# Ipsedo/MARLClassification

Hardware: AMD Instinct MI355X
Metric: agent-env-steps/sec (higher is better)
Workload: dtype f32; 1 GPU; RESISC45 256x256x3, 16 agents, 16 steps, f=12, README dims (configs[2]); full train iteration: rollout + A2C loss + BPTT backward + Adam; batch_per_gpu=256, global_batch=256, parallelism=dp1, rng=library (Philox4x32-10), launch=eager

## Files before the change

marlclassification_amd/csrc/common.h:

```cpp
#pragma once

#include <hip/hip_runtime.h>
#include <stdint.h>
#include <stdio.h>

#include "../../include/marl_hip.h"
#include "split.h"

namespace marl {

constexpr int kWave = 64;

inline int p4(int x) { return (x + 3) & ~3; }
inline int64_t cdiv(int64_t a, int64_t b) { return (a + b - 1) / b; }

void set_error(const char* fmt, ...);

int tune_get(const char* key, int dflt);
int tune_set(const char* key, int value);

__device__ __forceinline__ float rcp_fast(float x) { return __builtin_amdgcn_rcpf(x); }
__device__ __forceinline__ float sigmoid_acc(float x) { return rcp_fast(1.0f + __expf(-x)); }
__device__ __forceinline__ float tanh_fast(float x) { return 1.0f - 2.0f * rcp_fast(1.0f + __expf(2.0f * x)); }
__device__ __forceinline__ float silu_fast(float y) { return y * sigmoid_acc(y); }
__device__ __forceinline__ float silu_grad_fast(float y) {
    const float s = sigmoid_acc(y);
    return s * (1.0f + y * (1.0f - s));
}

__device__ __forceinline__ float wave_sum(float v) {
    int x = __float_as_int(v);
#define MARL_DPP_ADD(ctrl, rmask)                         \
    x = __float_as_int(__int_as_float(x) +                \
                       __int_as_float(__builtin_amdgcn_update_dpp(0, x, ctrl, rmask, 0xf, false)))
    MARL_DPP_ADD(0x111, 0xf);
    MARL_DPP_ADD(0x112, 0xf);
    MARL_DPP_ADD(0x114, 0xf);
    MARL_DPP_ADD(0x118, 0xf);
    MARL_DPP_ADD(0x142, 0xa);
    MARL_DPP_ADD(0x143, 0xc);
#undef MARL_DPP_ADD
    return __int_as_float(__builtin_amdgcn_readlane(x, 63));
}

#define MARL_HIP_CHECK(expr)                                                        \
    do {                                                                            \
        hipError_t e_ = (expr);                                                     \
        if (e_ != hipSuccess) {                                                     \
            marl::set_error("%s failed: %s (%s:%d)", #expr, hipGetErrorString(e_),  \
                            __FILE__, __LINE__);                                    \
            return MARL_EHIP;                                                       \
        }                                                                           \
    } while (0)

#define MARL_LAUNCH_CHECK() MARL_HIP_CHECK(hipGetLastError())

#define MARL_TRY(expr)             \
    do {                           \
        int rc_ = (expr);          \
        if (rc_ != MARL_OK) return rc_; \
    } while (0)

struct GemmSeg {
    const float* a;
    const float* b;
    int lda, ldb, k;
    const void* b3;
    int kt3;
};

struct GemmB {
    const float* b;
    int ld, k;
    const void* b3;
    int kt3;
    GemmB from_row(int row0) const {
        return GemmB{b + (size_t)row0 * ld, ld, k,
                     b3 ? static_cast<const char*>(b3) + (size_t)row0 * kt3 * 192 : nullptr, kt3};
    }
};
inline GemmB gemm_b(const float* b, int ld, int k) { return GemmB{b, ld, k, nullptr, 0}; }

struct GemmProb {
    GemmSeg seg[2];
    int nseg;
    int m, n;
    float* c;
    int ldc;
    const float* bias;
    int accumulate;
    const float* c_prev;
    float* h_next;
    float* c_next;
    float* gates;
    int ld_state, ld_gates;
};

constexpr int kMaxGemmBatch = 4;
struct GemmBatch {
    GemmProb p[kMaxGemmBatch];
    int count;
    int gx, gy;
    int xcd_map;
    int single_buf;
#ifdef MARL_KERNEL_TS
    long long* ts;
#endif
};

__device__ __forceinline__ void xcd_tile(unsigned gx, unsigned gy, unsigned gz, unsigned& bx,
                                         unsigned& by, unsigned& bz) {
    const unsigned T = gx * gy * gz, L = blockIdx.x;
    const unsigned per = T >> 3, rem = T & 7, xcd = L & 7, slot = L >> 3;
    const unsigned q = (xcd < rem ? xcd * (per + 1) : rem * (per + 1) + (xcd - rem) * per) + slot;
    bz = q / (gx * gy);
    const unsigned r = q - bz * gx * gy;
    bx = r / gy;
    by = r - bx * gy;
}
int xcd_map_enabled();

GemmProb gemm_prob(const float* a, int lda, const GemmB& b, float* c, int ldc, int m, int n,
                   const float* bias = nullptr, int accumulate = 0);
void gemm_add_seg(GemmProb& p, const float* a, int lda, const GemmB& b);

int launch_gemm_nt(const GemmBatch& batch, hipStream_t st);
int launch_gemm_lstm(const GemmBatch& batch, hipStream_t st);

int split_mode();
size_t split_image_floats(int rows, int k);
struct SplitDesc {
    const float* src;
    void* dst;
    int rows, k, ld, kt;
};
constexpr int kMaxSplitDesc = 64;
struct SplitBatch {
    SplitDesc d[kMaxSplitDesc];
    int count;
};
int launch_split_weights(const SplitBatch& b, hipStream_t st);
int launch_gemm_nt_split(const GemmBatch& batch, int max_m, int max_n, int64_t blocks128, hipStream_t st);
int launch_gemm_lstm_split(const GemmBatch& batch, int max_m, int max_n, hipStream_t st);
int launch_gemm_tn_split(const float* a, int lda, const float* b, int ldb, float* out, int ldo,
                         int64_t stride, int ni, int nj, int64_t rows, int64_t rows_per_split,
                         float* csum, dim3 grid, int gx, int gy, int gz, hipStream_t st);

struct G3Seg {
    const char* a3;
    const char* b3;
    int a_row0, b_row0;
    int steps;
};
struct G3Prob {
    G3Seg seg[2];
    int nseg;
    int m, n;
    float* c;
    int ldc;
    const float* bias;
    int accumulate;
    const float* c_prev;
    float* h_next;
    float* c_next;
    float* gates;
    int ld_state, ld_gates;
    char* h3;
    int h3_row0, h3_steps;
};
constexpr int kMaxG3 = 4;
struct G3Batch {
    G3Prob p[kMaxG3];
    int count;
    int gx, gy, xcd_map;
    int safe;
#ifdef MARL_G3_ABLATE
    long long* clk;
#endif
};
G3Prob g3_prob(const void* a3, int a_row0, const void* b3, int b_row0, int k, float* c, int ldc, int m, int n,
               const float* bias = nullptr, int accumulate = 0);
void g3_add_seg(G3Prob& p, const void* a3, int a_row0, const void* b3, int b_row0, int k);
int launch_gemm_nt3(const G3Batch& batch, hipStream_t st, int variant = 0);
int launch_gemm_lstm3(const G3Batch& batch, hipStream_t st, int variant = 0);
int g3_lstm_plan(const G3Batch& batch);
struct G3TnArgs {
    const char* a3;
    const char* b3;
    int a_steps, b_steps;
    int a_row0, b_row0;
    float* out;
    int ldo;
    int64_t out_split_stride;
    int ni, nj;
    int64_t rows, rows_per_split;
    float* csum;
    int gx, gy, gz, safe;
    int j_first;
#ifdef MARL_G3_ABLATE
    int abl;
#endif
};
struct G3TnPlan {
    int variant, splits;
    int64_t rows_per_split;
};
G3TnPlan g3_tn_plan(int ni, int nj, int64_t rows);
constexpr int kMaxTnCell = 4;
struct G3TnCell {
    G3TnArgs t[kMaxTnCell];
    int nt, n256;
    int gx, gz;
    int teams;
};
bool g3_tn_cell_ok(int ni, int nj_ih, int nj_hh, int64_t rows);
G3TnPlan g3_tn_cell_plan(int ni, int nj_ih, int nj_hh, int64_t rows);
size_t g3_tn_cell_scratch_bytes(int ni, int nj_ih, int nj_hh, int64_t rows);
int launch_gemm_tn3_cell(G3TnArgs ih, G3TnArgs hh, const G3TnPlan& plan, hipStream_t st);
size_t g3_tn_scratch_bytes(int ni, int nj, int64_t rows);
int launch_gemm_tn3(G3TnArgs a, const G3TnPlan& plan, hipStream_t st);

struct ImgDesc {
    const float* src;
    void* dst;
    int64_t rows;
    int k, ld;
};
constexpr int kMaxImgDesc = 64;
struct ImgBatch {
    ImgDesc d[kMaxImgDesc];
    int count;
};
int launch_images(const ImgBatch& b, hipStream_t st);

constexpr int kProfClasses = 6;
void prof_before(int cls, hipStream_t st);
void prof_after(int cls, hipStream_t st);
int profile_begin(int cls, int max_launches);
int profile_end(double* total_ms, int* launches);

struct RedQueue;
size_t gemm_tn_scratch_bytes(int ni, int nj, int64_t rows);
struct TnQueue;
int launch_gemm_tn(const float* a, int lda, const float* b, int ldb, float* c, int ldc, int ni,
                   int nj, int64_t rows, float* scratch, size_t scratch_bytes, hipStream_t st,
                   float* colsum_out = nullptr, RedQueue* q = nullptr, TnQueue* tq = nullptr);

struct TnBatchProb {
    const float* a;
    const float* b;
    float* out;
    float* csum;
    int64_t stride, rows, rows_per_split;
    int lda, ldb, ldo, ni, nj, gx, gy, first_block;
};
constexpr int kMaxTnBatch = 12;
struct TnBatch {
    TnBatchProb p[kMaxTnBatch];
    int count;
};
struct TnQueue {
    struct Item {
        const float* a;
        const float* b;
        float* c;
        float* colsum;
        int lda, ldb, ldc, ni, nj;
        int64_t rows;
    };
    Item it[kMaxTnBatch];
    int n = 0;
};
bool gemm_tn_is_small(int ni, int nj, int64_t rows);
int launch_tn_queue(TnQueue& tq, RedQueue* q, hipStream_t st);

struct RedDesc {
    const float* part;
    int64_t stride;
    int count, n;
    float* out0;
    int split, nj, ldc;
    float* out1;
    int accumulate;
    int folds, per;
};
constexpr int kMaxRed = 40;
struct RedBatch {
    RedDesc d[kMaxRed];
    int first_block[kMaxRed + 1];
    int count;
};
struct RedQueue {
    RedBatch stage1, stage2;
    float* scratch = nullptr;
    size_t cap = 0, off = 0;
    hipStream_t st = nullptr;
    int rc = MARL_OK;
    void reset(float* s, size_t floats, hipStream_t stream);
    float* take(size_t floats, bool may_flush = true);
    void push(const float* part, int64_t stride, int count, int n, float* out0, int split, int nj,
              int ldc, float* out1, int accumulate);
    int launch_pending();
    int flush();
};
int launch_red_batch(const RedBatch& b, hipStream_t st);

int launch_ln_silu_fwd(const float* z, int ldz, const float* gamma, const float* beta, float* out,
                       int ldo, float* stats, int64_t m, int n, hipStream_t st,
                       const float* wdot = nullptr, const float* bdot = nullptr,
                       float* dot_out = nullptr);
int ln_bwd_blocks(int64_t m, int n);
int launch_ln_silu_bwd_rank(const float* g, int ldg, int kin, const float* bt, int ldbt,
                            const float* z, int ldz, const float* stats, const float* gamma,
                            const float* beta, float* dz, int lddz, float* part, int64_t m, int n,
                            hipStream_t st);
int launch_ln_silu_bwd(const float* da, int ldda, const float* z, int ldz, const float* stats,
                       const float* gamma, const float* beta, float* dz, int lddz, float* part,
                       int64_t m, int n, hipStream_t st);
int launch_reduce_affine(float* part, int64_t nparts, int n, float* dgamma, float* dbeta,
                         int accumulate, hipStream_t st, RedQueue* q = nullptr);

int gn_fwd_im2col_supported(int P, int C);
int launch_gn_silu_fwd(const float* z, const float* gamma, const float* beta, float* out,
                       int64_t ldo, int out_chw, float* stats, int64_t rows, int P, int C, int G,
                       hipStream_t st, float* cols = nullptr, int ldk = 0, int hin = 0);
int gn_bwd_blocks(int64_t rows, int C);
int launch_gn_silu_bwd(const float* da, int64_t ldda, int da_chw, const float* z,
                       const float* stats, const float* gamma, const float* beta, float* dz,
                       float* part, int64_t rows, int P, int C, int G, hipStream_t st);

int launch_agg_msg(const float* m, float* out, int ld, int na, int nb, int n, hipStream_t st);
int launch_mix_msg(const float* m, float* out, int ld, int na, int nb, int n, const float* mix, int transpose,
                   hipStream_t st);
int mix_msg_max_agents();
struct CommGate {
    const int32_t* pos;
    int radius, metric, normalize;
};
__device__ __forceinline__ bool comm_in_range(int2 p, int2 q, int radius, int metric) {
    const int dy = p.x > q.x ? p.x - q.x : q.x - p.x, dx = p.y > q.y ? p.y - q.y : q.y - p.y;
    if (metric) return (int64_t)dy * dy + (int64_t)dx * dx <= (int64_t)radius * radius;
    return (dy > dx ? dy : dx) <= radius;
}
template <int MAXA>
__device__ __forceinline__ float comm_gate_weight(const float* __restrict__ base, const CommGate& G, int na, int nb,
                                                  int b, int a, int a2) {
    const int2* __restrict__ pos = reinterpret_cast<const int2*>(G.pos);
    const int2 pa = pos[(size_t)a * nb + b];
    if (!G.normalize) {
        const int2 q = pos[(size_t)a2 * nb + b];
        const float bv = base[a * na + a2];
        return comm_in_range(pa, q, G.radius, G.metric) ? bv : 0.f;
    }
    constexpr int CH = MAXA < 8 ? MAXA : 8;
    float S = 0.f, s = 0.f, u = 0.f;
#pragma unroll
    for (int j0 = 0; j0 < MAXA; j0 += CH) {
        int2 q[CH];
        float bv[CH];
#pragma unroll
        for (int j = 0; j < CH; ++j) {
            const int jj = j0 + j < na ? j0 + j : na - 1;
            q[j] = pos[(size_t)jj * nb + b];
            bv[j] = base[a * na + jj];
        }
#pragma unroll
        for (int j = 0; j < CH; ++j) {
            if (j0 + j < na) {
                const float uj = comm_in_range(pa, q[j], G.radius, G.metric) ? bv[j] : 0.f;
                S += bv[j];
                s += uj;
                if (j0 + j == a2) u = uj;
            }
        }
    }
    return s > 0.f ? u * (S / s) : 0.f;
}
int launch_mix_msg_gated(const float* m, float* out, int ld, int na, int nb, int n, const float* mix,
                         const CommGate& gate, int transpose, hipStream_t st);
int comm_grad_blocks(int64_t pairs, int* per_out);
int comm_grad_supported(int na, int n, int n2, int ldw);
int launch_comm_grad(const float* dz, int lddz, const float* msg, int ldmsg, const float* w, int ldw, int na, int nb,
                     int steps, int n2, int n, float* part, float* out, hipStream_t st);

int launch_pos_embed_fwd(const int32_t* pos, const float* npos_in, int h, int w, const float* W, const float* b,
                         const float* gamma, const float* beta, float* npos4, float* z, int ldz,
                         float* stats, float* out, int ldo, int64_t rows, int nd, hipStream_t st);

int launch_lstm_cell_bwd(const float* dh, int lddh, float* dc, int lddc, float* gates, int ldg,
                         const float* c_prev, const float* c_new, int ldc, int64_t rows, int n,
                         hipStream_t st);
struct LstmBwdBatch;
int launch_lstm_cell_bwd_batch(LstmBwdBatch& b, int count, hipStream_t st);
int launch_lstm_cell_bwd2(const float* dh0, int lddh0, float* dc0, int lddc0, float* gates0,
                          int ldg0, const float* cp0, const float* cn0, int ldc0, int n0,
                          const float* dh1, int lddh1, float* dc1, int lddc1, float* gates1,
                          int ldg1, const float* cp1, const float* cn1, int ldc1, int n1,
                          int64_t rows, hipStream_t st);

struct SampleArgs {
    const float* a_pol;
    int ld_a, nla;
    const float* w1;
    int ldw;
    const float* b1;
    const float* noise;
    uint64_t rng_seed, rng_ctr;
    const uint64_t* rng_off_dev;
    int rng_on;
    const int64_t* forced;
    const int32_t* pos_in;
    int32_t* pos_out;
    int64_t* step_pos;
    int64_t* step_actions;
    float* step_logp;
    float* probs;
    int32_t* actions_i32;
    int R, nA, H, W, f;
    int32_t table[MARL_MAX_ACTIONS][2];
    const float* pe_W;
    const float* pe_b;
    const float* pe_gamma;
    const float* pe_beta;
    float* pe_npos;
    float* pe_z;
    float* pe_stats;
    float* pe_out;
    int pe_ldz, pe_ldo, pe_nd;
    char* pe_img;
    int pe_row0, pe_steps, pe_col0;
    float ex_inv_tau, ex_keep, ex_floor;
    int ex_greedy;
};
int launch_sample(const SampleArgs& a, hipStream_t st, bool explore = false);

int launch_draw_episode(uint64_t seed, uint64_t offset, const uint64_t* offset_dev, int64_t* pos0,
                        int R, int H, int W, int f, float* h0, float* c0, int n_b, float* hc0,
                        float* cc0, int n_a, float* noise, int64_t n_noise, hipStream_t st);

struct PermDesc {
    const float* src;
    float* dst;
    int rows, cols;
    int dst_ld;
    int rd, rs1, rs2;
    int cd, cs1, cs2;
    int frag;
    const float* src2;
};
constexpr int kMaxPerm = 56;
struct PermBatch {
    PermDesc d[kMaxPerm];
    int count;
};
int launch_permute(const PermBatch& b, hipStream_t st);

__host__ __device__ inline int panel_frag_groups(int K) { return (K + 15) >> 4; }
__host__ __device__ inline size_t panel_frag_floats(int n, int K) {
    return ((size_t)((n + 31) >> 5) * panel_frag_groups(K) + 3) * 512;
}
__host__ __device__ inline size_t panel_frag_index(int r, int k, int groups) {
    return ((((size_t)(r >> 5) * groups + (k >> 4)) * 2 + ((r >> 4) & 1)) * 64 + ((k >> 2) & 3) * 16 + (r & 15)) * 4 +
           (k & 3);
}

struct Counters {
    uint64_t rng_offset;
    uint64_t step;
    float lr_over_bc1;
    float inv_sqrt_bc2;
    float pad[2];
};
static_assert(sizeof(Counters) == MARL_COUNTERS_BYTES, "counter block layout");
int launch_counters_set(Counters* c, uint64_t rng_offset, int64_t step, float lr, float beta1,
                        float beta2, int tick, hipStream_t st);

int launch_adam(float* p, const float* g, float* m, float* v, int64_t n, float lr_over_bc1,
                float inv_sqrt_bc2, float beta1, float beta2, float eps, float grad_scale,
                hipStream_t st, const Counters* cnt = nullptr);

int launch_fill(float* p, int64_t n, float v, hipStream_t st);
int launch_add2d(const float* a, int64_t lda, const float* b, int64_t ldb, float* out, int64_t ldo,
                 int64_t rows, int cols, hipStream_t st);
int launch_copy2d(const float* src, int64_t lds, float* dst, int64_t ldd, int64_t rows, int cols,
                  hipStream_t st);
int launch_i64_to_i32(const int64_t* src, int32_t* dst, int64_t n, hipStream_t st);
int launch_policy_dlogits(const float* dlogp, const float* probs, const int32_t* actions,
                          float* out, int ld, int64_t rows, int nA, hipStream_t st);
int launch_policy_dlogits_probs(const float* dlogp, const float* dprobs, const float* probs,
                                const int32_t* actions, float* out, int ld, int64_t rows, int nA,
                                hipStream_t st);
int launch_policy_dlogits_explore(const float* dlogp, const float* dprobs, const float* probs,
                                  const int32_t* actions, float* out, int ld, int64_t rows, int nA,
                                  float inv_tau, float keep, float floor, hipStream_t st);
int launch_acc2d(float* dst, int64_t ldd, const float* src, int64_t lds, int64_t rows, int cols,
                 hipStream_t st);
int launch_rowdot(const float* a, int lda, const float* w, const float* b, float* out,
                  int64_t rows, int n, hipStream_t st);

struct PanelLayer {
    const float* wfrag;
    int wgroups;
    const float* bias;
    const float* gamma;
    const float* beta;
    int n;
    float* z;
    int ldz;
    float* stats;
    float* a;
    int lda;
    char* a3;
    int a3_row0, a3_steps, a3_col0;
};
constexpr int kPanelMaxLayers = 4;
struct PanelFwdProb {
    const float* x;
    int ldx, k0;
    int agg_na, agg_nb;
    float* xbar;
    int m, nlayers;
    PanelLayer layer[kPanelMaxLayers];
    int by_batch, g_na, g_nb, agg_at, ld_xbar;
    const float* mix;
    CommGate gate;
};
struct PanelFwdBatch {
    PanelFwdProb p[2];
    int count;
    int off_panel1, off_red, off_part, off_prm;
    int off_mix;
    int has_sample, panel_blocks;
    int epi_prob;
    int ln_narrow_max;
    SampleArgs sample;
#ifdef MARL_KERNEL_TS
    long long* ts;
#endif
};
int panel_chain_supported(int na, int n_msg, int threads);
int panel_supported(int k0, int n0, int n1);
int panel_sample_supported(int n_actions);
int launch_panel_fwd(PanelFwdBatch& b, hipStream_t st, bool explore = false);

struct LstmBwdArgs {
    const float* dh;
    float* dc;
    float* gates;
    const float* c_prev;
    const float* c_new;
    int lddh, lddc, ldg, ldc, n;
    char* g3;
    int g3_row0, g3_steps;
    int skip_f32;
};
struct LstmBwdBatch {
    LstmBwdArgs a[2];
    int64_t rows;
    int vec4;
};
inline bool lstm_bwd_vec4_ok(const LstmBwdArgs& a) {
    return (a.n & 3) == 0 && (a.lddh & 3) == 0 && (a.lddc & 3) == 0 && (a.ldg & 3) == 0 && (a.ldc & 3) == 0;
}
__device__ __forceinline__ void lstm_cell_bwd_at(const LstmBwdArgs& A, int64_t r, int u, float dhv);
__device__ __forceinline__ void lstm_cell_bwd_elem(const LstmBwdArgs& A, int64_t rows, int64_t idx) {
    const int n = A.n;
    if (idx >= rows * n) return;
    const int64_t r = idx / n;
    const int u = (int)(idx % n);
    lstm_cell_bwd_at(A, r, u, A.dh[r * A.lddh + u]);
}
__device__ __forceinline__ void lstm_cell_bwd_at(const LstmBwdArgs& A, int64_t r, int u, float dhv) {
    const int n = A.n;
    float* g = A.gates + r * A.ldg + u;
    const float gi = g[0], gf = g[n], gg = g[2 * n], go = g[3 * n];
    const float tc = tanh_fast(A.c_new[r * A.ldc + u]);
    const float dcv = dhv * go * (1.0f - tc * tc) + A.dc[r * A.lddc + u];
    g[0] = dcv * gg * gi * (1.0f - gi);
    g[n] = dcv * A.c_prev[r * A.ldc + u] * gf * (1.0f - gf);
    g[2 * n] = dcv * gi * (1.0f - gg * gg);
    g[3 * n] = dhv * tc * go * (1.0f - go);
    A.dc[r * A.lddc + u] = dcv * gf;
}

__device__ __forceinline__ void lstm_cell_bwd_at4(const LstmBwdArgs& A, int64_t r, int u, const float (&dhv)[4]) {
    const int n = A.n;
    float* g = A.gates + r * A.ldg + u;
    const float4 gi4 = *reinterpret_cast<const float4*>(g), gf4 = *reinterpret_cast<const float4*>(g + n),
                 gg4 = *reinterpret_cast<const float4*>(g + 2 * n), go4 = *reinterpret_cast<const float4*>(g + 3 * n);
    const float4 cn4 = *reinterpret_cast<const float4*>(A.c_new + r * A.ldc + u),
                 cp4 = *reinterpret_cast<const float4*>(A.c_prev + r * A.ldc + u),
                 dc4 = *reinterpret_cast<const float4*>(A.dc + r * A.lddc + u);
    const float gi[4] = {gi4.x, gi4.y, gi4.z, gi4.w}, gf[4] = {gf4.x, gf4.y, gf4.z, gf4.w};
    const float gg[4] = {gg4.x, gg4.y, gg4.z, gg4.w}, go[4] = {go4.x, go4.y, go4.z, go4.w};
    const float cn[4] = {cn4.x, cn4.y, cn4.z, cn4.w}, cp[4] = {cp4.x, cp4.y, cp4.z, cp4.w};
    const float dcin[4] = {dc4.x, dc4.y, dc4.z, dc4.w};
    float o[5][4];
#pragma unroll
    for (int q = 0; q < 4; ++q) {
        const float tc = tanh_fast(cn[q]);
        const float dcv = dhv[q] * go[q] * (1.0f - tc * tc) + dcin[q];
        o[0][q] = dcv * gg[q] * gi[q] * (1.0f - gi[q]);
        o[1][q] = dcv * cp[q] * gf[q] * (1.0f - gf[q]);
        o[2][q] = dcv * gi[q] * (1.0f - gg[q] * gg[q]);
        o[3][q] = dhv[q] * tc * go[q] * (1.0f - go[q]);
        o[4][q] = dcv * gf[q];
    }
    if (!(A.g3 && A.skip_f32)) {
// ... 54 lines not shown
    int has_cell, panel_blocks;
    LstmBwdArgs cell;
    int64_t cell_rows;
    int cell_vec4;
    int cellb_img_done, cell_img_done;
    CommGate gate;
#ifdef MARL_KERNEL_TS
    long long* ts;
#endif
};
int panel_bwd_blocks(int m);
int panel_chain_blocks(int na, int nb);
int panel_chain_by_batch(int na);
int launch_panel_bwd(PanelBwdProb& p, hipStream_t st);

#ifdef MARL_KERNEL_TS
constexpr int kTsWaves = 16, kTsSlots = 48, kTsRoles = 2;
#define MARL_TS_DECL(ptr) long long* ts_ = (ptr); int tsi_ = 0
#define MARL_TS()                                                                              \
    if (ts_ && (threadIdx.x & 63) == 0 && blockIdx.x == 37 && blockIdx.y < kTsRoles && tsi_ < kTsSlots) \
    ts_[((int)blockIdx.y * kTsWaves + (threadIdx.x >> 6)) * kTsSlots + tsi_++] = wall_clock64()
int ts_begin(long long** dev, int call);
void ts_report(const char* tag, long long* dev, int waves, int role = 0);
#else
#define MARL_TS_DECL(ptr)
#define MARL_TS()
#endif

struct FDiv {
    uint32_t d, m;
};
inline FDiv make_fdiv(int d) { return FDiv{(uint32_t)d, (uint32_t)(((1ull << 32) / (uint64_t)d) + 1)}; }
__device__ __forceinline__ int fdiv(int n, FDiv f) {
    return f.d == 1 ? n : (int)__umulhi((uint32_t)n, f.m);
}

struct CnnFwdLayer {
    const float *w, *bias, *gamma, *beta;
    float* cols;
    float* z;
    float* gst;
    int cin, cout, G, hin, hout, P, K, ldk;
    const float* wfrag;
};
struct CnnFwdArgs {
    const void* img;
    const float* obs;
    const int32_t* pos;
    int img_u8;
    int64_t rows;
    int nb, c_img, H, W, f, L;
    CnnFwdLayer layer[MARL_MAX_CNN_LAYERS];
    float* u;
    int ldu;
    char* u3;
    int u3_row0, u3_steps;
    int rb;
    int off_b0, off_b1, off_stat;
    FDiv dP[MARL_MAX_CNN_LAYERS], dhout[MARL_MAX_CNN_LAYERS], dcin[MARL_MAX_CNN_LAYERS],
        dcpg[MARL_MAX_CNN_LAYERS], dG[MARL_MAX_CNN_LAYERS], dNT[MARL_MAX_CNN_LAYERS],
        dc4o[MARL_MAX_CNN_LAYERS];
    FDiv dpe, dff, df, dE;
#ifdef MARL_KERNEL_TS
    long long* ts;
#endif
};
int cnn_fwd_supported(const CnnFwdArgs& a);
int cnn_fwd_writes_image(const CnnFwdArgs& a);
int launch_cnn_fwd(CnnFwdArgs& a, hipStream_t st);
struct CnnFwdPlan {
    int which, rb, blocks;
};
CnnFwdPlan cnn_fwd_launch_plan(const CnnFwdArgs& a);

struct CnnDgradArgs {
    const float* dz;
    const float* wt;
    const float* zin;
    const float* gst;
    const float *gamma, *beta;
    float* dzin;
    float* part;
    int64_t rows;
    int ldwt, cin, cout, hin, hout, P, Pin, G;
    int rb, MT, NT, off_zin, off_da, off_perm, off_stat, off_gsum;
    int tbeg[17];
    FDiv dc4o, dc4i, dPin, dcpg, dG;
    const void* img;
    const int32_t* pos;
    float* w0_part;
    float* w0_bpart;
    int w0;
    int img_u8, nb, c_img, H, W, cin0, f0, K0;
    int off_pix, pix_per, cs0;
    FDiv dpe0, dff0, df0, dhin0;
#ifdef MARL_KERNEL_TS
    long long* ts;
#endif
};
int cnn_dgrad_supported(const CnnDgradArgs& a);
int cnn_dgrad_blocks(const CnnDgradArgs& a);
int cnn_dgrad_blocks_max(const CnnDgradArgs& a);
int cnn_dgrad_launch_rb(const CnnDgradArgs& a);
struct CnnDgradPlanInfo {
    int rb, MT, NT, blocks;
};
CnnDgradPlanInfo cnn_dgrad_launch_plan(const CnnDgradArgs& a);
int launch_cnn_dgrad(CnnDgradArgs& a, hipStream_t st);
int cnn_dgrad_w0_ok(const CnnDgradArgs& a, int cin0, int f0);

struct CnnDimgArgs {
    const float* dz0;
    const float* wt0;
    const int32_t* pos;
    float* d_img;
    int ns, na, nb, c_img, H, W;
    int ldwt, cin, cout, f, hout, P;
    int th;
};
int cnn_dimg_supported(const CnnDimgArgs& a);
int launch_cnn_dimg(CnnDimgArgs& a, hipStream_t st);

struct CnnWgradArgs {
    const float* dz;
    const void* img;
    const int32_t* pos;
    const float* zin;
    const float* gst;
    const float *gamma, *beta;
    float* part_w;
    float* part_b;
    int64_t rows;
    int first, img_u8, nb, c_img, H, W;
    int cin, cout, hin, hout, P, G, K;
    int rb, nchunks, blocks;
    int hp, cs, zs, in_per;
    int off_dz, off_tab, lds_floats;
    int in_plane;
    int nct, nkt, nkt_slab, slabs;
    int tgc, tgk, ms;
    int sct, skt;
    int pd, pi;
    FDiv dP, dhout, dPin, dhin, dcin, dc4o, dc4i, dpe, dff, df;
};
int cnn_wgrad_supported(const CnnWgradArgs& a);
int cnn_wgrad_blocks(const CnnWgradArgs& a);
int launch_cnn_wgrad(CnnWgradArgs& a, hipStream_t st);
struct CnnWgradPlanInfo {
    int form, rb, chunks, blocks;
    int sct, skt, tgc, tgk, ms, slabs, pd, pi;
};
CnnWgradPlanInfo cnn_wgrad_launch_plan(const CnnWgradArgs& a);
int launch_slab_reduce(const float* part, int64_t stride, int splits, float* c, int ldc, int ni,
                       int nj, const float* bpart, float* bias, hipStream_t st);

int launch_gather_im2col(const void* img, int img_u8, const int32_t* pos, float* cols, int ldk,
                         int na, int nb, int c_img, int cin, int H, int W, int f, hipStream_t st);
int launch_obs_im2col(const float* obs, float* cols, int ldk, int64_t rows, int c_img, int cin,
                      int f, hipStream_t st);
int launch_patch_gather(const float* img, const int64_t* pos, float* obs, int na, int nb, int c,
                        int H, int W, int f, hipStream_t st);
int launch_im2col(const float* a, float* cols, int ldk, int64_t rows, int hin, int cin,
                  hipStream_t st);
int launch_col2im(const float* dcols, int ldk, float* da, int64_t rows, int hin, int cin,
                  hipStream_t st);

struct LossCommon {
    const float* preds;
    const float* values;
    const int64_t* y;
    float* scratch;
    int ns, na, nb, nc;
    bool cls = false;
    const float* cls_w = nullptr;
    const float* cls_sw = nullptr;
    float cls_eps = 0.f;
    bool cls_wrew = false;
};
struct LossGradArgs : LossCommon {
    const float* logp;
    float* g_preds;
    int ld_gp;
    float* g_logp;
    float* g_values;
    float* scalars;
    const float* probs = nullptr;
    float* g_probs = nullptr;
    int n_act = 0;
    float entropy_coef = 0.f;
};

struct LossArgs : LossGradArgs {
    double* adv_stats;
    float gamma;
    int phase;
};
size_t loss_scratch_floats(int ns, int na, int nb);
int launch_loss(const LossArgs& a, hipStream_t st);

struct AdvArgs : LossCommon {
    float* advn;
    float* ret;
    double* adv_stats;
    float gamma, lam;
    int phase;
};
int launch_advantages(const AdvArgs& a, hipStream_t st);

struct PpoArgs : LossGradArgs {
    const float* old_logp;
    const float* advn;
    const float* ret;
    float clip_eps;
};
int launch_ppo_loss(const PpoArgs& a, hipStream_t st);

int launch_grad_clip(float* g, int64_t n, float max_norm, float grad_scale, float* norm_out, double* part,
                     hipStream_t st);

}
```

marlclassification_amd/csrc/episode.hip:

```cpp
#include <math.h>
#include <stdlib.h>
#include <string.h>

#include "../../include/marl_hip_rowops.h"
#include "../../include/marl_hip_cnnops.h"
#include "../../include/marl_hip_explore.h"
#include "../../include/marl_hip_classloss.h"
#include "common.h"

namespace marl {

struct Dims {
    int na, nb, ns;
    int64_t R, NR;
    int H, W, c_img, f;
    int L;
    int ch[MARL_MAX_CNN_LAYERS + 1];
    int grp[MARL_MAX_CNN_LAYERS];
    int hw[MARL_MAX_CNN_LAYERS + 1];
    int P[MARL_MAX_CNN_LAYERS];
    int K[MARL_MAX_CNN_LAYERS];
    int ldk[MARL_MAX_CNN_LAYERS];
    int nf, nin;
    int n_b, n_a, n_m, nm2, n_mo, n_d, nA, nC, nlb, nla;
// ... 445 lines not shown
            red += ((v + 63) & ~(size_t)63) + 64 * 2 * (size_t)n + 64;
        };
        auto upd_tn = [&](int ni, int nj, int64_t rows) {
            const size_t v = gemm_tn_scratch_bytes(ni, nj, rows);
            tns = v > tns ? v : tns;
            red += v / sizeof(float) + 64 * ((size_t)ni * nj + ni) + 192;
        };
        const int64_t nr = d.NR, r = d.R;
        upd_part(ln_bwd_blocks(nr, d.nlb), d.nlb);
        upd_part(ln_bwd_blocks(nr, d.nla), d.nla);
        upd_part(ln_bwd_blocks(nr, d.n_d), d.n_d);
        upd_part(ln_bwd_blocks(r, d.nm2), d.nm2);
        upd_part(ln_bwd_blocks(r, d.n_mo), d.n_mo);
        upd_part(ln_bwd_blocks(r, d.n_m), d.n_m);
        for (int l = 0; l < d.L; ++l) upd_part(gn_bwd_blocks(nr, d.ch[l + 1]), d.ch[l + 1]);
        for (int l = 1; l < d.L; ++l)
            if (e.dgrad_ok[l]) upd_part(cnn_dgrad_blocks_max(cnn_dgrad_shape(d, l)), d.ch[l]);
        upd_tn(d.nC, d.nlb, nr);
        upd_tn(d.nlb, d.n_b, nr);
        upd_tn(1, d.nla, nr);
        upd_tn(d.nla, d.n_a, nr);
        upd_tn(d.nA, d.nla, nr);
        upd_tn(d.n_mo, d.nm2, nr);
        upd_tn(d.nm2, d.n_m, nr);
        upd_tn(d.n_m, d.nm2, nr);
        upd_tn(d.nm2, d.n_b, nr);
        upd_tn(4 * d.n_b, d.nin, nr);
        upd_tn(4 * d.n_b, d.n_b, nr);
        upd_tn(4 * d.n_a, d.nin, nr);
        upd_tn(4 * d.n_a, d.n_a, nr);
        if (e.g3) {
            const int tn3[4][2] = {{4 * d.n_b, d.nin}, {4 * d.n_b, d.n_b}, {4 * d.n_a, d.nin}, {4 * d.n_a, d.n_a}};
            for (const auto& q : tn3) {
                const size_t v = g3_tn_scratch_bytes(q[0], q[1], nr);
                tns = v > tns ? v : tns;
            }
            const int cell[2][3] = {{4 * d.n_b, d.nin, d.n_b}, {4 * d.n_a, d.nin, d.n_a}};
            for (const auto& q : cell)
                if (g3_tn_cell_ok(q[0], q[1], q[2], nr)) {
                    const size_t v = g3_tn_cell_scratch_bytes(q[0], q[1], q[2], nr);
                    tns = v > tns ? v : tns;
                }
        }
        upd_tn(d.n_d, 2, nr);
        if (d.L > 1 && e.dgrad_ok[1]) {
            const CnnDgradArgs g1 = cnn_dgrad_shape(d, 1);
            if (g1.w0) {
                int64_t nb_ = cnn_dgrad_blocks_max(g1);
                if (nb_ > 2048) nb_ = 2048;
                const size_t v = (size_t)nb_ * ((size_t)d.ch[1] * d.K[0] + d.ch[1]) * sizeof(float);
                tns = v > tns ? v : tns;
                red += v / sizeof(float) + 64 * ((size_t)d.ch[1] * (d.K[0] + 1)) + 192;
            }
        }
        for (int l = 0; l < d.L; ++l) {
            if (e.wgrad_ok[l]) {
                const size_t v = (size_t)cnn_wgrad_blocks(cnn_wgrad_shape(d, l)) *
                                 ((size_t)d.ch[l + 1] * d.K[l] + d.ch[l + 1]) * sizeof(float);
                tns = v > tns ? v : tns;
                red += v / sizeof(float) + 64 * ((size_t)d.ch[l + 1] * (d.K[l] + 1)) + 192;
            } else {
                upd_tn(d.ch[l + 1], d.K[l], nr * d.P[l]);
            }
        }
        e.part_floats = part;
        e.tns_bytes = tns;
        e.PART = b.take(part);
        e.TNS = b.take(tns / sizeof(float) + 16);
        {
            const int pn[4] = {d.n_mo, d.nm2, d.n_m, d.nm2};
            for (int n : pn) red += 64 * 2 * (size_t)n + 64;
        }
        e.red_floats = red + 4096;
        e.RED = b.take(e.red_floats);
    }
    e.loss_floats = loss_scratch_floats(d.ns, d.na, d.nb);
    e.LOSS = b.take(e.loss_floats);
    e.total = b.off;
}

struct Explore {
    bool on;
    float inv_tau, keep, eps;
    int greedy;
};
struct ClassLoss {
    bool on;
    const float* w;
    int nc;
    float eps;
    const float* sw;
    int ns;
    bool wrew;
};
struct Installed {
    const float* comm = nullptr;
    int comm_na = 0;
    CommGate range = {nullptr, -1, 0, 1};
    Explore explore = {false, 1.f, 1.f, 0.f, 0};
    ClassLoss class_loss = {false, nullptr, 0, 0.f, nullptr, 0, false};
    hipEvent_t heads_event = nullptr;
};
static Installed g_installed;

enum SampleSite { SAMPLE_OWN = 0, SAMPLE_EPILOGUE, SAMPLE_RIDE };
struct Plan {
    bool panels;
    bool panels_bwd;
    bool chain;
    bool panel_sample;
    bool g3_lstm;
    bool g3_tn, g3_tn_pipe;
    bool u3_by_producers;
    int skip_f32;
    int lstm_plan;
    SampleSite sample;
    int comm_form;
    int explore_form;
    int comm, comm_range, explore, class_loss;
};

struct Ctx {
    Dims d;
    WLayout w;
    ELayout e;
    float* W;
    float* E;
    hipStream_t st;
    int train;
    RedQueue* rq = nullptr;
    TnQueue* tq = nullptr;
    bool defer_slabs = false;
    size_t defer_small = 0;
    bool defer_this(size_t slab_bytes) const { return defer_slabs || (defer_small && slab_bytes <= defer_small); }
    Installed opt;
    Plan plan;
    int u3_row(int t) const { return (int)(e.u3_stride_rows * (size_t)t); }

    const char* wp3k(int i) const { return reinterpret_cast<const char*>(W + w.wp3k[i]); }
    const char* wt3k(int i) const { return reinterpret_cast<const char*>(W + w.wt3k[i]); }
    char* img(size_t off) const { return reinterpret_cast<char*>(E + off); }
    const float* wp(int i) const { return W + w.wp[i]; }
    const float* wt(int i) const { return W + w.wt[i]; }
    GemmB wpB(int i) const {
        const ParamMeta m = param_meta(d, i);
        return GemmB{wp(i), w.ldp[i], m.k, m.kind == PK_MATRIX ? W + w.wp3[i] : nullptr, (m.k + 31) / 32};
    }
    GemmB wtB(int i) const {
        const ParamMeta m = param_meta(d, i);
        return GemmB{wt(i), w.ldt[i], m.n, m.kind == PK_MATRIX ? W + w.wt3[i] : nullptr, (m.n + 31) / 32};
    }
    const float* wpf(int i) const { return w.wpf[i] ? W + w.wpf[i] : nullptr; }
    const float* wtf(int i) const { return w.wtf[i] ? W + w.wtf[i] : nullptr; }
    float* gp(int i) const { return W + w.gp[i]; }
    float* at(size_t off) const { return E + off; }
    float* at(const SBuf& s, int t) const { return E + s.at(train ? t : 0); }
    float* Hs(int t) const { return E + e.H + (size_t)t * d.R * d.ld_nb; }
    float* Cs(int t) const { return E + e.C + (size_t)t * d.R * d.ld_nb; }
    float* HCs(int t) const { return E + e.HC + (size_t)t * d.R * d.ld_na; }
    float* CCs(int t) const { return E + e.CC + (size_t)t * d.R * d.ld_na; }
    float* MSGs(int t) const { return E + e.MSG + (size_t)t * d.R * d.ld_nm; }
    int32_t* POSs(int t) const { return reinterpret_cast<int32_t*>(E + e.POS) + (size_t)t * d.R * 2; }
    float* PROBSs(int t) const { return E + e.PROBS + (size_t)t * d.R * d.nA; }
    int32_t* ACTs(int t) const { return reinterpret_cast<int32_t*>(E + e.ACT) + (size_t)t * d.R; }
    float* DHs(int t) const { return E + e.DH + (size_t)t * d.R * d.ld_nb; }
    float* DHCs(int t) const { return E + e.DHC + (size_t)t * d.R * d.ld_na; }
};

static Plan make_plan(const Dims& d, const WLayout& w, const ELayout& e, const Installed& opt) {
    auto env_on = [](const char* v) { return !(v && v[0] == '0'); };
    static const bool env_panels = env_on(getenv("MARL_PANELS")), env_sample = env_on(getenv("MARL_PANEL_SAMPLE"));
    Plan p{};
    p.panels = env_panels && panel_model_ok(d);
    p.panels_bwd = p.panels && d.n_mo <= 384 && d.nm2 <= 384 && d.n_m <= 384;
    p.chain = p.panels_bwd && panel_chain_supported(d.na, d.n_m, 256) && tune_get("panel_chain", 1) != 0 &&
              (!opt.comm || d.n_b <= 384);
    p.panel_sample = p.chain && env_sample && panel_sample_supported(d.nA);
    p.sample = p.chain ? (p.panel_sample ? SAMPLE_EPILOGUE : SAMPLE_OWN)
                       : (p.panels && !opt.explore.on ? SAMPLE_RIDE : SAMPLE_OWN);
    p.comm_form = opt.comm ? (p.chain ? 5 : p.panels ? 3 : 4) : p.chain ? 0 : p.panels ? 1 : 2;
    p.explore_form = !opt.explore.on ? 0 : p.panel_sample ? 1 : 2;
    p.comm = opt.comm != nullptr;
    p.comm_range = opt.range.radius >= 0 ? opt.range.radius : -1;
    p.explore = opt.explore.on;
    p.class_loss = opt.class_loss.on;

    const int k_lstm = tune_get("g3_lstm", 1), k_tn = tune_get("g3_tn", 1);
    p.g3_lstm = e.g3 && k_lstm != 0;
    if (p.g3_lstm) {
        G3Batch b{};
        b.count = 2;
        b.p[0].m = b.p[1].m = (int)d.R;
        b.p[0].n = d.n_b;
        b.p[1].n = d.n_a;
        p.lstm_plan = tune_get("g3_lstm_variant", 0);
        if (!p.lstm_plan) p.lstm_plan = g3_lstm_plan(b);
    }
    p.g3_tn = p.g3_lstm && k_tn != 0 &&
              (k_tn == 2 || (d.nin <= 640 && d.n_b <= 512 && d.n_a <= 512 &&
                             (d.NR >= 32768 || (g3_tn_cell_ok(4 * d.n_b, d.nin, d.n_b, d.NR) &&
                                                g3_tn_cell_ok(4 * d.n_a, d.nin, d.n_a, d.NR)))));
    p.g3_tn_pipe = p.g3_tn && tune_get("g3_tn_pipe", 1) != 0;
    p.skip_f32 = p.panels_bwd && p.g3_tn;
    static float here;
    CnnFwdArgs probe = cnn_fwd_shape(d);
    for (int l = 0; l < d.L; ++l) probe.layer[l].wfrag = w.wf[4 * l] ? &here : nullptr;
    p.u3_by_producers = p.g3_lstm && e.fused_fwd && cnn_fwd_writes_image(probe) && p.panels &&
                        ((d.nf | d.n_mo | d.n_d) & 3) == 0 &&
                        d.nin % 16 == 0;
    return p;
}

static int make_ctx(const marl_config* cfg, const void* wws, size_t wbytes, void* ews, size_t ebytes,
                    int train, void* stream, Ctx& c) {
    MARL_TRY(make_dims(cfg, c.d));
    c.opt = g_installed;
    if (c.opt.comm && c.opt.comm_na != c.d.na) {
        set_error("communication matrix is %d x %d but the configuration has %d agents", c.opt.comm_na,
                  c.opt.comm_na, c.d.na);
        return MARL_EINVAL;
    }
    if (c.opt.range.radius >= 0 && !c.opt.comm) {
        set_error("a communication range is installed without its base matrix (marl_comm_matrix)");
        return MARL_EINVAL;
    }
    make_wlayout(c.d, c.w);
    make_elayout(c.d, train, c.e);
    if (wbytes < c.w.total * sizeof(float) || ebytes < c.e.total * sizeof(float)) {
        set_error("workspace too small for the current configuration / tuning knobs: weights %zu of %zu "
                  "bytes, episode %zu of %zu bytes (ask marl_workspace_sizes again)", wbytes,
                  c.w.total * sizeof(float), ebytes, c.e.total * sizeof(float));
        return MARL_ESIZE;
    }
    c.W = const_cast<float*>(static_cast<const float*>(wws));
    c.E = static_cast<float*>(ews);
    c.st = static_cast<hipStream_t>(stream);
    c.train = train;
    if (!c.W || !c.E) {
        set_error("null workspace");
        return MARL_EINVAL;
    }
    if ((reinterpret_cast<uintptr_t>(c.W) & 255) || (reinterpret_cast<uintptr_t>(c.E) & 255)) {
        set_error("workspaces must be 256-byte aligned");
        return MARL_EINVAL;
    }
    c.plan = make_plan(c.d, c.w, c.e, c.opt);
    return MARL_OK;
}

static int gemm1(const Ctx& c, const GemmProb& p) {
    GemmBatch b{};
    b.p[0] = p;
    b.count = 1;
    return launch_gemm_nt(b, c.st);
}
static int gemm2(const Ctx& c, const GemmProb& p0, const GemmProb& p1) {
    GemmBatch b{};
    b.p[0] = p0;
    b.p[1] = p1;
    b.count = 2;
    return launch_gemm_nt(b, c.st);
}

struct StepIn {
    const float* obs = nullptr;
    const float* npos = nullptr;
    const void* img = nullptr;
    int img_u8 = 0;
};

struct CnnFwdIo {
    const void* img = nullptr;
    const float* obs = nullptr;
    const int32_t* pos = nullptr;
    int img_u8 = 0;
    int64_t rows = 0;
    float* cols[MARL_MAX_CNN_LAYERS] = {};
    float* z[MARL_MAX_CNN_LAYERS] = {};
    float* gst[MARL_MAX_CNN_LAYERS] = {};
    float* u = nullptr;
    int ldu = 0;
    char* u3 = nullptr;
    int u3_row0 = 0, u3_steps = 0;
};
static CnnFwdArgs cnn_fwd_args(const Dims& d, const WLayout& w, const float* W, const CnnFwdIo& io) {
    CnnFwdArgs a{};
    a.img = io.img;
    a.obs = io.obs;
    a.pos = io.pos;
    a.img_u8 = io.img_u8;
    a.rows = io.rows;
    a.nb = d.nb;
    a.c_img = d.c_img;
    a.H = d.H;
    a.W = d.W;
    a.f = d.f;
    a.L = d.L;
    for (int l = 0; l < d.L; ++l)
        a.layer[l] = CnnFwdLayer{W + w.wp[4 * l], W + w.wp[4 * l + 1], W + w.wp[4 * l + 2], W + w.wp[4 * l + 3],
                                 io.cols[l], io.z[l], io.gst[l],
                                 d.ch[l], d.ch[l + 1], d.grp[l], d.hw[l], d.hw[l + 1], d.P[l],
                                 d.K[l], d.ldk[l], w.wf[4 * l] ? W + w.wf[4 * l] : nullptr};
    a.u = io.u;
    a.ldu = io.ldu;
    a.u3 = io.u3;
    a.u3_row0 = io.u3_row0;
    a.u3_steps = io.u3_steps;
// ... 316 lines not shown
    const bool vdot = d.nla <= 384;
    MARL_TRY(launch_ln_silu_fwd(c.at(c.e.ZC1), d.ld_nla, c.wp(MARL_P_CRI_LNW), c.wp(MARL_P_CRI_LNB),
                                c.at(c.e.AC1), d.ld_nla, c.at(c.e.STC1), rows, d.nla, st,
                                vdot ? c.wp(MARL_P_CRI_W1) : nullptr, c.wp(MARL_P_CRI_B1), values));
    MARL_TRY(launch_ln_silu_fwd(c.at(c.e.ZQ1), d.ld_nlb, c.wp(MARL_P_PRE_LNW), c.wp(MARL_P_PRE_LNB),
                                c.at(c.e.AQ1), d.ld_nlb, c.at(c.e.STQ1), rows, d.nlb, st));
    if (!vdot)
        MARL_TRY(launch_rowdot(c.at(c.e.AC1), d.ld_nla, c.wp(MARL_P_CRI_W1), c.wp(MARL_P_CRI_B1),
                               values, rows, d.nla, st));
    MARL_TRY(gemm1(c, gemm_prob(c.at(c.e.AQ1), d.ld_nlb, c.wpB(MARL_P_PRE_W1),
                                preds, d.nC, (int)rows, d.nC, c.wp(MARL_P_PRE_B1))));
    return MARL_OK;
}

static void explore_sample_args(const Explore& ex, SampleArgs& a) {
    if (!ex.on) return;
    a.ex_inv_tau = ex.inv_tau;
    a.ex_keep = ex.keep;
    a.ex_floor = ex.eps / (float)a.nA;
    a.ex_greedy = ex.greedy;
    if (ex.greedy) {
        a.noise = nullptr;
        a.rng_on = 0;
    }
}

struct SampleIo {
    const float* noise = nullptr;
    const int64_t* forced = nullptr;
    uint64_t rng_seed = 0, rng_offset = 0;
    const void* counters = nullptr;
    int64_t *step_pos = nullptr, *step_actions = nullptr;
    float* step_logp = nullptr;
    bool embed_next = false;
};
static void fill_sample_args(const Ctx& c, const marl_config* cfg, int t, const SampleIo& io, SampleArgs& a) {
    const Dims& d = c.d;
    memset(&a, 0, sizeof(a));
    if (io.step_logp) {
        a.noise = io.noise ? io.noise + (size_t)t * d.R * d.nA : nullptr;
        a.rng_on = !io.noise && !io.forced;
        a.rng_seed = io.rng_seed ^ 0x9E3779B97F4A7C15ull;
        a.rng_ctr = (io.rng_offset << 16) + (uint64_t)t;
        a.rng_off_dev = io.counters ? &static_cast<const Counters*>(io.counters)->rng_offset : nullptr;
        a.forced = io.forced ? io.forced + (size_t)t * d.R : nullptr;
        a.step_pos = io.step_pos ? io.step_pos + (size_t)t * d.R * 2 : nullptr;
        a.step_actions = io.step_actions ? io.step_actions + (size_t)t * d.R : nullptr;
        a.step_logp = io.step_logp + (size_t)t * d.R;
    }
    if (io.embed_next && t + 1 < d.ns) {
        a.pe_W = c.wp(MARL_P_POS_W);
        a.pe_b = c.wp(MARL_P_POS_B);
        a.pe_gamma = c.wp(MARL_P_POS_LNW);
        a.pe_beta = c.wp(MARL_P_POS_LNB);
        a.pe_npos = c.at(c.e.NPOS, t + 1);
        a.pe_z = c.at(c.e.ZPOS, t + 1);
        a.pe_stats = c.at(c.e.STPOS, t + 1);
        a.pe_out = c.at(c.e.U, t + 1) + d.nf + d.n_mo;
        a.pe_ldz = d.ld_nd;
        a.pe_ldo = d.ld_nin;
        a.pe_nd = d.n_d;
        if (c.plan.u3_by_producers) {
            a.pe_img = c.img(c.e.U3);
            a.pe_row0 = c.u3_row(t + 1);
            a.pe_steps = img_steps(d.nin);
            a.pe_col0 = d.nf + d.n_mo;
        }
    }
    a.a_pol = c.at(c.e.AP1, t);
    a.ld_a = d.ld_nla;
    a.nla = d.nla;
    a.w1 = c.wp(MARL_P_POL_W1);
    a.ldw = d.ld_nla;
    a.b1 = c.wp(MARL_P_POL_B1);
    a.pos_in = c.POSs(t);
    a.pos_out = c.POSs(t + 1);
    a.probs = c.PROBSs(t);
    a.actions_i32 = c.ACTs(t);
    a.R = (int)d.R;
    a.nA = d.nA;
    a.H = d.H;
    a.W = d.W;
    a.f = d.f;
    for (int j = 0; j < d.nA; ++j) {
        a.table[j][0] = cfg->actions[j][0];
        a.table[j][1] = cfg->actions[j][1];
    }
    explore_sample_args(c.opt.explore, a);
}

static int fwd_open(const Ctx& c, int t, const StepIn& in, bool decode) {
    MARL_TRY(step_cnn(c, t, in));
    if (decode) MARL_TRY(step_decode(c, t));
    return step_pos_lstm(c, t, in, t > 0);
}
static int fwd_step_chain(const Ctx& c, int t, const StepIn& in, const SampleArgs& a) {
    MARL_TRY(fwd_open(c, t, in, t == 0));
    MARL_TRY(step_chain(c, t, a));
    return c.plan.sample == SAMPLE_EPILOGUE ? MARL_OK : launch_sample(a, c.st, c.opt.explore.on);
}
static int fwd_step_panels(const Ctx& c, int t, const StepIn& in, const SampleArgs& a) {
    const bool ride = c.plan.sample == SAMPLE_RIDE && t + 1 < c.d.ns;
    MARL_TRY(fwd_open(c, t, in, t == 0));
    MARL_TRY(step_encode_policy(c, t));
    if (t + 1 < c.d.ns) MARL_TRY(step_decode(c, t + 1, ride ? &a : nullptr));
    return ride ? MARL_OK : launch_sample(a, c.st, c.opt.explore.on);
}
static int fwd_step_rows(const Ctx& c, int t, const StepIn& in, const SampleArgs& a) {
    MARL_TRY(fwd_open(c, t, in, true));
    MARL_TRY(step_encode_policy(c, t));
    if (t + 1 < c.d.ns) MARL_TRY(step_decode(c, t + 1));
    return launch_sample(a, c.st, c.opt.explore.on);
}

struct PermQueue {
    PermBatch b{};
    hipStream_t st;
    int rc = MARL_OK;
    explicit PermQueue(hipStream_t s) : st(s) { b.count = 0; }
    void push(const PermDesc& p) {
        if (rc != MARL_OK) return;
        b.d[b.count++] = p;
        if (b.count == kMaxPerm) flush();
    }
    void flush() {
        if (rc == MARL_OK && b.count > 0) rc = launch_permute(b, st);
        b.count = 0;
    }
};

static PermDesc perm(const float* src, float* dst, int rows, int cols, int dst_ld, int rd, int rs1,
                     int rs2, int cd, int cs1, int cs2, const float* src2 = nullptr) {
    PermDesc p;
    p.src = src;
    p.dst = dst;
    p.rows = rows;
    p.cols = cols;
    p.dst_ld = dst_ld;
    p.rd = rd;
    p.rs1 = rs1;
    p.rs2 = rs2;
    p.cd = cd;
    p.cs1 = cs1;
    p.cs2 = cs2;
    p.frag = 0;
    p.src2 = src2;
    return p;
}

static PermDesc copy_desc(const float* src, int64_t lds, float* dst, int64_t ldd, int64_t rows, int cols) {
    return perm(src, dst, (int)rows, cols, (int)ldd, 1, (int)lds, 0, 1, 1, 0);
}

static int load_state(const Ctx& c, const float* h, const float* cc_, const float* hc,
                      const float* cca, const float* msg) {
    const Dims& d = c.d;
    PermQueue q(c.st);
    q.push(copy_desc(h, d.n_b, c.Hs(0), d.ld_nb, d.R, d.n_b));
    q.push(copy_desc(cc_, d.n_b, c.Cs(0), d.ld_nb, d.R, d.n_b));
    q.push(copy_desc(hc, d.n_a, c.HCs(0), d.ld_na, d.R, d.n_a));
    q.push(copy_desc(cca, d.n_a, c.CCs(0), d.ld_na, d.R, d.n_a));
    q.push(copy_desc(msg, d.n_m, c.MSGs(0), d.ld_nm, d.R, msg ? d.n_m : d.ld_nm));
    q.flush();
    MARL_TRY(q.rc);
    if (c.e.g3) {
        ImgBatch ib{};
        ib.d[0] = ImgDesc{h, c.img(c.e.H3), d.R, d.n_b, d.n_b};
        ib.d[1] = ImgDesc{hc, c.img(c.e.HC3), d.R, d.n_a, d.n_a};
        ib.count = 2;
        MARL_TRY(launch_images(ib, c.st));
    }
    return MARL_OK;
}


static int pack_weights(const Dims& d, const WLayout& w, const float* const* params, float* W,
                        hipStream_t st) {
    PermQueue q(st);
    for (int i = 0; i < MARL_NPARAMS; ++i) {
        const ParamMeta m = param_meta(d, i);
        if (m.kind == PK_NONE) continue;
        const float* src = params[i];
        if (!src) {
            set_error("parameter %d is null", i);
            return MARL_EINVAL;
        }
        if (m.kind == PK_MATRIX) {
            q.push(perm(src, W + w.wp[i], m.n, m.k, w.ldp[i], 1, m.k, 0, 1, 1, 0));
            q.push(perm(src, W + w.wt[i], m.k, m.n, w.ldt[i], 1, 1, 0, 1, m.k, 0));
        } else if (m.kind == PK_CONV) {
            const int ci = m.k / 9;
            q.push(perm(src, W + w.wp[i], m.n, m.k, w.ldp[i], 1, m.k, 0, ci, 1, 9));
            q.push(perm(src, W + w.wt[i], m.k, m.n, w.ldt[i], ci, 1, 9, 1, m.k, 0));
        } else {
            q.push(perm(src, W + w.wp[i], 1, m.n, m.n, 1, 0, 0, 1, 1, 0));
        }
    }
    q.push(perm(params[MARL_P_LB_BIH], W + w.bsum_b, 1, 4 * d.n_b, 4 * d.n_b, 1, 0, 0, 1, 1, 0,
                params[MARL_P_LB_BHH]));
    q.push(perm(params[MARL_P_LA_BIH], W + w.bsum_a, 1, 4 * d.n_a, 4 * d.n_a, 1, 0, 0, 1, 1, 0,
                params[MARL_P_LA_BHH]));
    q.flush();
    MARL_TRY(q.rc);
    for (int i = 0; i < MARL_NPARAMS; ++i) {
        const ParamMeta m = param_meta(d, i);
        if (!w.wf[i]) continue;
        const int steps = m.k / 16;
        q.push(perm(W + w.wp[i], W + w.wf[i], (m.n / 16) * steps * 4, 64, 64, steps * 4, 16 * w.ldp[i], 4, 4,
                    w.ldp[i], 1));
    }
    for (int i = 0; i < MARL_NPARAMS; ++i) {
        const ParamMeta m = param_meta(d, i);
        if (w.wpf[i]) {
            PermDesc p = perm(W + w.wp[i], W + w.wpf[i], m.n, m.k, 0, 1, w.ldp[i], 0, 1, 1, 0);
            p.frag = w.gpf[i];
            q.push(p);
        }
        if (w.wtf[i]) {
            PermDesc p = perm(W + w.wt[i], W + w.wtf[i], m.k, m.n, 0, 1, w.ldt[i], 0, 1, 1, 0);
            p.frag = w.gtf[i];
            q.push(p);
        }
    }
    q.flush();
    MARL_TRY(q.rc);
    SplitBatch sb{};
    sb.count = 0;
    for (int i = 0; i < MARL_NPARAMS; ++i) {
        const ParamMeta m = param_meta(d, i);
        if (m.kind != PK_MATRIX) continue;
        sb.d[sb.count++] = SplitDesc{W + w.wp[i], W + w.wp3[i], m.n, m.k, w.ldp[i], (m.k + 31) / 32};
        sb.d[sb.count++] = SplitDesc{W + w.wt[i], W + w.wt3[i], m.k, m.n, w.ldt[i], (m.n + 31) / 32};
    }
    MARL_TRY(launch_split_weights(sb, st));
    ImgBatch ib{};
    ib.count = 0;
    for (int i = 0; i < MARL_NPARAMS; ++i) {
        const ParamMeta m = param_meta(d, i);
        if (m.kind != PK_MATRIX || !w.wp3k[i]) continue;
        if (ib.count + 2 > kMaxImgDesc) {
            MARL_TRY(launch_images(ib, st));
            ib.count = 0;
        }
        ib.d[ib.count++] = ImgDesc{W + w.wp[i], W + w.wp3k[i], m.n, m.k, w.ldp[i]};
        ib.d[ib.count++] = ImgDesc{W + w.wt[i], W + w.wt3k[i], m.k, m.n, w.ldt[i]};
    }
    return launch_images(ib, st);
}

static int unpack_grads(const Ctx& c, float* const* grads, int which = 0) {
    PermQueue q(c.st);
    for (int i = 0; i < MARL_NPARAMS; ++i) {
        const bool head = i >= MARL_P_POL_W0 && i <= MARL_P_PRE_B1;
        if ((which == 1 && !head) || (which == 2 && head)) continue;
        const ParamMeta m = param_meta(c.d, i);
        if (m.kind == PK_MATRIX) {
            q.push(perm(c.gp(i), grads[i], m.n, m.k, m.k, 1, c.w.ldp[i], 0, 1, 1, 0));
        } else if (m.kind == PK_CONV) {
            const int ci = m.k / 9;
            q.push(perm(c.gp(i), grads[i], m.n, m.k, m.k, 1, c.w.ldp[i], 0, 9, 1, ci));
        }
    }
    if (which != 1) {
        q.push(perm(grads[MARL_P_LB_BIH], grads[MARL_P_LB_BHH], 1, 4 * c.d.n_b, 4 * c.d.n_b, 1, 0, 0, 1, 1, 0));
        q.push(perm(grads[MARL_P_LA_BIH], grads[MARL_P_LA_BHH], 1, 4 * c.d.n_a, 4 * c.d.n_a, 1, 0, 0, 1, 1, 0));
    }
    q.flush();
    return q.rc;
}

static int tn(const Ctx& c, const float* a, int lda, const float* b, int ldb, int pidx, int ni,
              int nj, int64_t rows, float* bias = nullptr) {
    RedQueue* q = c.defer_this(gemm_tn_scratch_bytes(ni, nj, rows)) ? c.rq : nullptr;
    return launch_gemm_tn(a, lda, b, ldb, c.gp(pidx), c.w.ldp[pidx], ni, nj, rows, c.at(c.e.TNS),
                          c.e.tns_bytes, c.st, bias, q, q ? c.tq : nullptr);
}
static int tn3(const Ctx& c, const char* a3, int ni, const char* b3, int nj, int pidx, int64_t rows, float* bias) {
    const G3TnPlan plan = g3_tn_plan(ni, nj, rows);
    if (g3_tn_scratch_bytes(ni, nj, rows) > c.e.tns_bytes) {
        set_error("tn3: scratch too small");
        return MARL_ESIZE;
    }
    float* scratch = c.at(c.e.TNS);
    G3TnArgs a{};
    a.a3 = a3;
    a.b3 = b3;
    a.a_steps = img_steps(ni);
    a.b_steps = img_steps(nj);
    a.out = scratch;
    a.ldo = nj;
    a.out_split_stride = (int64_t)ni * nj;
    a.ni = ni;
    a.nj = nj;
    a.rows = rows;
    a.csum = bias ? scratch + (size_t)plan.splits * ni * nj : nullptr;
    MARL_TRY(launch_gemm_tn3(a, plan, c.st));
    return launch_slab_reduce(scratch, (int64_t)ni * nj, plan.splits, c.gp(pidx), c.w.ldp[pidx], ni, nj, a.csum, bias, c.st);
}
static int tn3_cell(const Ctx& c, const char* g3, int ni, const char* u3, int nin, int p_ih, const char* h3, int nh,
                    int p_hh, int64_t rows, float* bias) {
    const G3TnPlan plan = g3_tn_cell_plan(ni, nin, nh, rows);
    if (g3_tn_cell_scratch_bytes(ni, nin, nh, rows) > c.e.tns_bytes) {
        set_error("tn3_cell: scratch too small");
        return MARL_ESIZE;
    }
    float* s_ih = c.at(c.e.TNS);
    float* s_hh = s_ih + (size_t)plan.splits * ni * nin;
    float* s_cs = s_hh + (size_t)plan.splits * ni * nh;
    G3TnArgs ih{}, hh{};
    ih.a3 = hh.a3 = g3;
    ih.a_steps = hh.a_steps = img_steps(ni);
    ih.ni = hh.ni = ni;
    ih.rows = hh.rows = rows;
    ih.b3 = u3;
    ih.b_steps = img_steps(nin);
    ih.nj = ih.ldo = nin;
    ih.out = s_ih;
    ih.out_split_stride = (int64_t)ni * nin;
    ih.csum = bias ? s_cs : nullptr;
    hh.b3 = h3;
    hh.b_steps = img_steps(nh);
    hh.nj = hh.ldo = nh;
    hh.out = s_hh;
    hh.out_split_stride = (int64_t)ni * nh;
    MARL_TRY(launch_gemm_tn3_cell(ih, hh, plan, c.st));
    MARL_TRY(launch_slab_reduce(s_ih, (int64_t)ni * nin, plan.splits, c.gp(p_ih), c.w.ldp[p_ih], ni, nin, nullptr, nullptr, c.st));
    return launch_slab_reduce(s_hh, (int64_t)ni * nh, plan.splits, c.gp(p_hh), c.w.ldp[p_hh], ni, nh, ih.csum, bias, c.st);
}
static float* part_scratch(const Ctx& c, int64_t blocks, int n, int acc, RedQueue*& q) {
    q = acc ? nullptr : c.rq;
    if (!q) return c.at(c.e.PART);
    float* p = q->take((size_t)blocks * 2 * n);
    if (q->rc != MARL_OK) q = nullptr;
    return q ? p : c.at(c.e.PART);
}
static int ln_bwd(const Ctx& c, float* da, int ldda, const float* z, int ldz, const float* stats,
                  int pw, int pb, int64_t rows, int n, float* const* grads, int acc,
                  float* dz = nullptr, int lddz = 0) {
    if (!dz) {
        dz = da;
        lddz = ldda;
    }
    RedQueue* q;
    float* part = part_scratch(c, ln_bwd_blocks(rows, n), n, acc, q);
    MARL_TRY(launch_ln_silu_bwd(da, ldda, z, ldz, stats, c.wp(pw), c.wp(pb), dz, lddz, part, rows, n,
                                c.st));
    return launch_reduce_affine(part, ln_bwd_blocks(rows, n), n, grads[pw], grads[pb], acc, c.st, q);
}

static int ln_bwd_rank(const Ctx& c, const float* g, int ldg, int kin, int w1, const float* z, int ldz,
                       const float* stats, int pw, int pb, int64_t rows, int n, float* const* grads,
                       float* dz, int lddz) {
    RedQueue* q;
    float* part = part_scratch(c, ln_bwd_blocks(rows, n), n, 0, q);
    MARL_TRY(launch_ln_silu_bwd_rank(g, ldg, kin, c.wt(w1), p4(kin), z, ldz, stats, c.wp(pw),
                                     c.wp(pb), dz, lddz, part, rows, n, c.st));
    return launch_reduce_affine(part, ln_bwd_blocks(rows, n), n, grads[pw], grads[pb], 0, c.st, q);
}

static int gate_image_fallback(const Ctx& c, const PanelBwdProb& pd, int t) {
    const Dims& d = c.d;
    ImgBatch ib{};
    ib.count = 0;
    if (pd.has_cellb && pd.cellb.g3 && !pd.cellb_img_done)
        ib.d[ib.count++] = ImgDesc{c.at(c.e.GB, t), c.img(c.e.GB3) + img_off((int64_t)t * d.R, 0, img_steps(4 * d.n_b)),
                                   d.R, 4 * d.n_b, d.ld_gb};
    if (pd.has_cell && pd.cell.g3 && !pd.cell_img_done)
        ib.d[ib.count++] = ImgDesc{c.at(c.e.GA, t), c.img(c.e.GA3) + img_off((int64_t)t * d.R, 0, img_steps(4 * d.n_a)),
                                   d.R, 4 * d.n_a, d.ld_ga};
    return launch_images(ib, c.st);
}

struct StepBwd {
    const float* obs = nullptr;
    const float* g_probs = nullptr;
    const float *g_msg = nullptr, *g_h = nullptr, *g_c = nullptr, *g_hc = nullptr, *g_cc = nullptr;
    float *d_msg = nullptr, *d_h = nullptr, *d_c = nullptr, *d_hc = nullptr, *d_cc = nullptr;
};


static LstmBwdArgs cell_bwd_args(const Ctx& c, int which, int t) {
    const Dims& d = c.d;
    const int n = which ? d.n_a : d.n_b, ld = which ? d.ld_na : d.ld_nb;
    return LstmBwdArgs{which ? c.DHCs(t + 1) : c.DHs(t + 1), c.at(which ? c.e.DCC : c.e.DC),
                       c.at(which ? c.e.GA : c.e.GB, t), which ? c.CCs(t) : c.Cs(t),
                       which ? c.CCs(t + 1) : c.Cs(t + 1), ld, ld, which ? d.ld_ga : d.ld_gb, ld, n,
                       c.e.g3 ? c.img(which ? c.e.GA3 : c.e.GB3) : nullptr, (int)((int64_t)t * d.R), img_steps(4 * n),
                       c.plan.skip_f32};
}

static void fill_dec_bwd_layers(const Ctx& c, int t, size_t pblk, float* ddbar, float* dad1, PanelBwdLayer* layer) {
    const Dims& d = c.d;
    layer[0] = PanelBwdLayer{c.at(c.e.ZD2, t), d.ld_nmo, c.at(c.e.STD2, t), c.wp(MARL_P_DEC_LN1W),
                             c.wp(MARL_P_DEC_LN1B), d.n_mo, ddbar, d.ld_dbl,
                             c.at(c.e.PLN[0]) + (size_t)t * pblk * d.n_mo, c.wtf(MARL_P_DEC_W1),
                             c.w.gtf[MARL_P_DEC_W1], d.nm2};
    layer[1] = PanelBwdLayer{c.at(c.e.ZD1, t), d.ld_nm2, c.at(c.e.STD1, t), c.wp(MARL_P_DEC_LN0W),
                             c.wp(MARL_P_DEC_LN0B), d.nm2, dad1, d.ld_nm2,
                             c.at(c.e.PLN[1]) + (size_t)t * pblk * d.nm2, c.wtf(MARL_P_DEC_W0),
                             c.w.gtf[MARL_P_DEC_W0], d.n_m};
}
static void fill_enc_bwd_layers(const Ctx& c, int t, size_t pblk, PanelBwdLayer* layer) {
    const Dims& d = c.d;
    layer[0] = PanelBwdLayer{c.at(c.e.ZE2, t), d.ld_nm, c.at(c.e.STE2, t), c.wp(MARL_P_ENC_LN1W),
                             c.wp(MARL_P_ENC_LN1B), d.n_m, c.at(c.e.DZE2) + (size_t)t * d.R * d.ld_nm, d.ld_nm,
                             c.at(c.e.PLN[2]) + (size_t)t * pblk * d.n_m, c.wtf(MARL_P_ENC_W1),
                             c.w.gtf[MARL_P_ENC_W1], d.nm2};
    layer[1] = PanelBwdLayer{c.at(c.e.ZE1, t), d.ld_nm2, c.at(c.e.STE1, t), c.wp(MARL_P_ENC_LN0W),
                             c.wp(MARL_P_ENC_LN0B), d.nm2, c.at(c.e.DAE1) + (size_t)t * d.R * d.ld_nm2, d.ld_nm2,
                             c.at(c.e.PLN[3]) + (size_t)t * pblk * d.nm2, c.wtf(MARL_P_ENC_W0),
                             c.w.gtf[MARL_P_ENC_W0], d.n_b};
}

static float* slab_scratch(const Ctx& c, size_t floats) {
    if (c.rq && c.defer_this(floats * sizeof(float))) {
        float* p = c.rq->take(floats);
        if (c.rq->rc == MARL_OK) return p;
    }
    return c.at(c.e.TNS);
}
static int slab_reduce(const Ctx& c, float* part_w, float* part_b, int blocks, int co, int k, int pidx, float* bias) {
    if (c.rq && part_w != c.at(c.e.TNS)) {
        c.rq->push(part_w, (int64_t)co * k, blocks, co * k, c.gp(pidx), co * k, k, c.w.ldp[pidx], nullptr, 0);
        c.rq->push(part_b, co, blocks, co, bias, co, co, co, nullptr, 0);
        return MARL_OK;
    }
    return launch_slab_reduce(part_w, (int64_t)co * k, blocks, c.gp(pidx), c.w.ldp[pidx], co, k, part_b, bias, c.st);
}

struct BwdState {
    Ctx c;
    RedQueue rq;
    TnQueue tq;
    float* const* grads;
    const StepBwd* sb;
    bool enc_last = false;
    bool heads_early = false;
    int pln_blocks = 0;
    bool action_done = false;
    bool belief_done = false;
};

static int bwd_heads(BwdState& s, const float* g_preds, const float* g_logp, const float* g_values,
                     const float* g_probs) {
    const Ctx& c = s.c;
    const Dims& d = c.d;
    const StepBwd* sb = s.sb;
    float* const* grads = s.grads;
    hipStream_t st = c.st;
    const int64_t NR = d.NR;
    const int ns = d.ns;
    {
        PermQueue q(st);
        q.push(copy_desc(g_preds, d.nC, c.at(c.e.GPRED), d.ld_nC, NR, g_preds ? d.nC : d.ld_nC));
        q.push(copy_desc(g_values, 1, c.at(c.e.DVAL), 4, NR, g_values ? 1 : 4));
        q.push(copy_desc(nullptr, 0, c.DHs(0), d.ld_nb, d.R, d.ld_nb));
        q.push(copy_desc(nullptr, 0, c.DHCs(0), d.ld_na, d.R, d.ld_na));
        q.push(copy_desc(nullptr, 0, c.at(c.e.DC), d.ld_nb, d.R, d.ld_nb));
        q.push(copy_desc(nullptr, 0, c.at(c.e.DCC), d.ld_na, d.R, d.ld_na));
        q.flush();
        MARL_TRY(q.rc);
    }
    if (sb) {
        MARL_TRY(launch_acc2d(c.at(c.e.DC), d.ld_nb, sb->g_c, d.n_b, d.R, d.n_b, st));
        MARL_TRY(launch_acc2d(c.at(c.e.DCC), d.ld_na, sb->g_cc, d.n_a, d.R, d.n_a, st));
        MARL_TRY(launch_fill(reinterpret_cast<float*>(c.POSs(0)), d.R * 2, 0.f, st));
    }
    MARL_TRY(gemm1(c, gemm_prob(c.at(c.e.GPRED), d.ld_nC, c.wtB(MARL_P_PRE_W1),
                                c.at(c.e.DAQ1), d.ld_nlb, (int)NR, d.nlb)));
    MARL_TRY(tn(c, c.at(c.e.GPRED), d.ld_nC, c.at(c.e.AQ1), d.ld_nlb, MARL_P_PRE_W1, d.nC, d.nlb, NR, grads[MARL_P_PRE_B1]));
    MARL_TRY(ln_bwd(c, c.at(c.e.DAQ1), d.ld_nlb, c.at(c.e.ZQ1), d.ld_nlb, c.at(c.e.STQ1),
                    MARL_P_PRE_LNW, MARL_P_PRE_LNB, NR, d.nlb, grads, 0));
    MARL_TRY(tn(c, c.at(c.e.DAQ1), d.ld_nlb, c.Hs(1), d.ld_nb, MARL_P_PRE_W0, d.nlb, d.n_b, NR, grads[MARL_P_PRE_B0]));
    MARL_TRY(tn(c, c.at(c.e.DVAL), 4, c.at(c.e.AC1), d.ld_nla, MARL_P_CRI_W1, 1, d.nla, NR, grads[MARL_P_CRI_B1]));
    if (d.nla <= 384) {
        MARL_TRY(ln_bwd_rank(c, c.at(c.e.DVAL), 4, 1, MARL_P_CRI_W1, c.at(c.e.ZC1), d.ld_nla,
                             c.at(c.e.STC1), MARL_P_CRI_LNW, MARL_P_CRI_LNB, NR, d.nla, grads,
                             c.at(c.e.DAC1), d.ld_nla));
    } else {
        MARL_TRY(gemm1(c, gemm_prob(c.at(c.e.DVAL), 4, c.wtB(MARL_P_CRI_W1), c.at(c.e.DAC1),
                                    d.ld_nla, (int)NR, d.nla)));
        MARL_TRY(ln_bwd(c, c.at(c.e.DAC1), d.ld_nla, c.at(c.e.ZC1), d.ld_nla, c.at(c.e.STC1),
                        MARL_P_CRI_LNW, MARL_P_CRI_LNB, NR, d.nla, grads, 0));
    }
    MARL_TRY(tn(c, c.at(c.e.DAC1), d.ld_nla, c.HCs(1), d.ld_na, MARL_P_CRI_W0, d.nla, d.n_a, NR, grads[MARL_P_CRI_B0]));
    if (sb && sb->g_probs) g_probs = sb->g_probs;
    const Explore& ex = c.opt.explore;
    if (ex.on && (ex.inv_tau != 1.f || ex.eps != 0.f))
        MARL_TRY(launch_policy_dlogits_explore(g_logp, g_probs, c.PROBSs(0), c.ACTs(0), c.at(c.e.DLOG), d.ld_nA, NR,
                                               d.nA, ex.inv_tau, ex.keep, ex.eps / (float)d.nA, st));
    else if (g_probs)
        MARL_TRY(launch_policy_dlogits_probs(g_logp, g_probs, c.PROBSs(0), c.ACTs(0), c.at(c.e.DLOG),
                                             d.ld_nA, NR, d.nA, st));
    else
        MARL_TRY(launch_policy_dlogits(g_logp, c.PROBSs(0), c.ACTs(0), c.at(c.e.DLOG), d.ld_nA, NR,
                                       d.nA, st));
    MARL_TRY(tn(c, c.at(c.e.DLOG), d.ld_nA, c.at(c.e.AP1, 0), d.ld_nla, MARL_P_POL_W1, d.nA, d.nla, NR, grads[MARL_P_POL_B1]));
    if (d.nA <= 4 && d.nla <= 384) {
        MARL_TRY(ln_bwd_rank(c, c.at(c.e.DLOG), d.ld_nA, d.nA, MARL_P_POL_W1, c.at(c.e.ZP1, 0),
                             d.ld_nla, c.at(c.e.STP1, 0), MARL_P_POL_LNW, MARL_P_POL_LNB, NR, d.nla,
                             grads, c.at(c.e.DAP1), d.ld_nla));
    } else {
        MARL_TRY(gemm1(c, gemm_prob(c.at(c.e.DLOG), d.ld_nA, c.wtB(MARL_P_POL_W1),
                                    c.at(c.e.DAP1), d.ld_nla, (int)NR, d.nla)));
        MARL_TRY(ln_bwd(c, c.at(c.e.DAP1), d.ld_nla, c.at(c.e.ZP1, 0), d.ld_nla, c.at(c.e.STP1, 0),
                        MARL_P_POL_LNW, MARL_P_POL_LNB, NR, d.nla, grads, 0));
    }
    MARL_TRY(tn(c, c.at(c.e.DAP1), d.ld_nla, c.HCs(1), d.ld_na, MARL_P_POL_W0, d.nla, d.n_a, NR, grads[MARL_P_POL_B0]));
    {
        GemmProb ph = gemm_prob(c.at(c.e.DAQ1), d.ld_nlb, c.wtB(MARL_P_PRE_W0), c.DHs(1), d.ld_nb, (int)NR, d.n_b);
        GemmProb pa = gemm_prob(c.at(c.e.DAP1), d.ld_nla, c.wtB(MARL_P_POL_W0), c.DHCs(1), d.ld_na, (int)NR, d.n_a);
        gemm_add_seg(pa, c.at(c.e.DAC1), d.ld_nla, c.wtB(MARL_P_CRI_W0));
        MARL_TRY(gemm2(c, ph, pa));
    }
    if (sb) {
        MARL_TRY(launch_acc2d(c.DHs(ns), d.ld_nb, sb->g_h, d.n_b, d.R, d.n_b, st));
        MARL_TRY(launch_acc2d(c.DHCs(ns), d.ld_na, sb->g_hc, d.n_a, d.R, d.n_a, st));
    }

    s.heads_early = c.opt.heads_event != nullptr && !sb;
    if (s.heads_early) {
        if (c.tq) MARL_TRY(launch_tn_queue(s.tq, c.rq, st));
        MARL_TRY(s.rq.flush());
        MARL_TRY(unpack_grads(c, grads, 1));
        MARL_HIP_CHECK(hipEventRecord(c.opt.heads_event, st));
    }
    return MARL_OK;
}


static int enc_bwd_rows(const BwdState& s, int t, int acc, float* dh) {
    const Ctx& c = s.c;
    const Dims& d = c.d;
    const int R = (int)d.R;
    float* dze2 = c.at(c.e.DZE2) + (size_t)t * d.R * d.ld_nm;
    float* dae1 = c.at(c.e.DAE1) + (size_t)t * d.R * d.ld_nm2;
    MARL_TRY(ln_bwd(c, dze2, d.ld_nm, c.at(c.e.ZE2, t), d.ld_nm, c.at(c.e.STE2, t), MARL_P_ENC_LN1W,
                    MARL_P_ENC_LN1B, d.R, d.n_m, s.grads, acc));
    MARL_TRY(gemm1(c, gemm_prob(dze2, d.ld_nm, c.wtB(MARL_P_ENC_W1), dae1, d.ld_nm2, R, d.nm2)));
    MARL_TRY(ln_bwd(c, dae1, d.ld_nm2, c.at(c.e.ZE1, t), d.ld_nm2, c.at(c.e.STE1, t), MARL_P_ENC_LN0W,
                    MARL_P_ENC_LN0B, d.R, d.nm2, s.grads, acc));
    return gemm1(c, gemm_prob(dae1, d.ld_nm2, c.wtB(MARL_P_ENC_W0), dh, d.ld_nb, R, d.n_b, nullptr, 1));
}

static int bwd_recurrent(const BwdState& s, int t, float* ddbar, float* ddbar2) {
    const Ctx& c = s.c;
    const Dims& d = c.d;
    const int R = (int)d.R;
    const struct { int which, w, row0; float* out; int ldo, n, acc; } prod[4] = {
        {0, MARL_P_LB_WHH, 0, c.DHs(t), d.ld_nb, d.n_b, 1},
        {1, MARL_P_LA_WHH, 0, c.DHCs(t), d.ld_na, d.n_a, 1},
        {0, MARL_P_LB_WIH, d.nf, ddbar, d.ld_dbl, d.n_mo + d.n_d, 0},
        {1, MARL_P_LA_WIH, d.nf, ddbar2, d.ld_dbl, d.n_mo + d.n_d, 0}};
    const int count = c.plan.panels_bwd ? 4 : 2;
    if (c.plan.panels_bwd && c.e.g3) {
        G3Batch g{};
        for (int i = 0; i < count; ++i) {
            const auto& q = prod[i];
            g.p[i] = g3_prob(c.img(q.which ? c.e.GA3 : c.e.GB3), (int)((int64_t)t * d.R), c.wt3k(q.w), q.row0,
                             4 * (q.which ? d.n_a : d.n_b), q.out, q.ldo, R, q.n, nullptr, q.acc);
        }
        g.count = count;
        return launch_gemm_nt3(g, c.st);
    }
    GemmBatch gb{};
    for (int i = 0; i < count; ++i) {
        const auto& q = prod[i];
        gb.p[i] = gemm_prob(c.at(q.which ? c.e.GA : c.e.GB, t), q.which ? d.ld_ga : d.ld_gb,
                            c.wtB(q.w).from_row(q.row0), q.out, q.ldo, R, q.n, nullptr, q.acc);
    }
    gb.count = count;
    if (!c.plan.panels_bwd) {
        GemmProb& p = gb.p[gb.count++];
        p = gemm_prob(c.at(c.e.GB, t), d.ld_gb, c.wtB(MARL_P_LB_WIH).from_row(d.nf), ddbar, d.ld_dbl, R, d.n_mo);
        gemm_add_seg(p, c.at(c.e.GA, t), d.ld_ga, c.wtB(MARL_P_LA_WIH).from_row(d.nf));
    }
    return launch_gemm_nt(gb, c.st);
}

static void fill_dec_bwd_prob(BwdState& s, int t, float* ddbar, float* ddbar2, PanelBwdProb& pd) {
// ... 24 lines not shown
    fill_dec_bwd_prob(s, t, ddbar, ddbar2, pd);
    pd.by_batch = panel_chain_by_batch(d.na);
    pd.g_na = d.na;
    pd.g_nb = d.nb;
    if (t > 0) {
        pd.nlayers = 4;
        pd.agg_at = 2;
        pd.mix = c.opt.comm;
        if (c.opt.comm) pd.gate = comm_gate(c, t);
        fill_enc_bwd_layers(c, t - 1, (size_t)s.pln_blocks * 2, pd.layer + 2);
        pd.dx = c.DHs(t);
        pd.lddx = d.ld_nb;
        pd.accumulate = 1;
        pd.has_cellb = 1;
        pd.cellb = cell_bwd_args(c, 0, t - 1);
        s.belief_done = true;
    }
    MARL_TRY(launch_panel_bwd(pd, c.st));
    return gate_image_fallback(c, pd, t - 1);
}

static int bwd_step_panels(BwdState& s, int t, float* ddbar, float* ddbar2) {
    const Ctx& c = s.c;
    const Dims& d = c.d;
    PanelBwdProb pd{};
    fill_dec_bwd_prob(s, t, ddbar, ddbar2, pd);
    MARL_TRY(launch_panel_bwd(pd, c.st));
    MARL_TRY(gate_image_fallback(c, pd, t - 1));
    if (t == 0) return MARL_OK;
    PanelBwdProb pe{};
    pe.da = c.at(c.e.DMBAR);
    pe.ldda = d.ld_nm;
    pe.agg_na = d.na;
    pe.agg_nb = d.nb;
    if (c.opt.comm) {
        MARL_TRY(mix_msg(c, t, c.at(c.e.DMBAR), c.at(c.e.DMBAR), d.ld_nm, 1));
        pe.agg_na = pe.agg_nb = 0;
    }
    pe.m = (int)d.R;
    pe.nlayers = 2;
    fill_enc_bwd_layers(c, t - 1, (size_t)s.pln_blocks * 2, pe.layer);
    pe.dx = c.DHs(t);
    pe.lddx = d.ld_nb;
    pe.accumulate = 1;
    return launch_panel_bwd(pe, c.st);
}

static int bwd_step_rows(const BwdState& s, int t, float* ddbar) {
    const Ctx& c = s.c;
    const Dims& d = c.d;
    const int R = (int)d.R;
    const int first = (t == d.ns - 1);
    float* dad1 = c.at(c.e.DAD1) + (size_t)t * d.R * d.ld_nm2;
    MARL_TRY(ln_bwd(c, ddbar, d.ld_dbl, c.at(c.e.ZD2, t), d.ld_nmo, c.at(c.e.STD2, t),
                    MARL_P_DEC_LN1W, MARL_P_DEC_LN1B, d.R, d.n_mo, s.grads, !first));
    MARL_TRY(gemm1(c, gemm_prob(ddbar, d.ld_dbl, c.wtB(MARL_P_DEC_W1), dad1, d.ld_nm2, R, d.nm2)));
    MARL_TRY(ln_bwd(c, dad1, d.ld_nm2, c.at(c.e.ZD1, t), d.ld_nm2, c.at(c.e.STD1, t),
                    MARL_P_DEC_LN0W, MARL_P_DEC_LN0B, d.R, d.nm2, s.grads, !first));
    if (t > 0 || (s.sb && s.sb->d_msg))
        MARL_TRY(gemm1(c, gemm_prob(dad1, d.ld_nm2, c.wtB(MARL_P_DEC_W0), c.at(c.e.DMBAR), d.ld_nm, R, d.n_m)));
    if (t == 0) return MARL_OK;
    float* dze2 = c.at(c.e.DZE2) + (size_t)(t - 1) * d.R * d.ld_nm;
    if (c.opt.comm)
        MARL_TRY(mix_msg(c, t, c.at(c.e.DMBAR), dze2, d.n_m, 1));
    else
        MARL_TRY(launch_agg_msg(c.at(c.e.DMBAR), dze2, d.ld_nm, d.na, d.nb, d.n_m, c.st));
    return enc_bwd_rows(s, t - 1, !first, c.DHs(t));
}

static int bwd_loop(BwdState& s) {
    Ctx& c = s.c;
    const Dims& d = c.d;
    const StepBwd* sb = s.sb;
    float* const* grads = s.grads;
    hipStream_t st = c.st;
    const int ns = d.ns;
    const size_t s_nmo = (size_t)d.R * d.ld_dbl;
    if (!c.plan.panels_bwd) {
        MARL_TRY(launch_tn_queue(s.tq, c.rq, st));
        c.rq = nullptr;
        c.tq = nullptr;
    }
    if (s.enc_last) {
        MARL_TRY(launch_copy2d(sb->g_msg, d.n_m, c.at(c.e.DZE2) + (size_t)(ns - 1) * d.R * d.ld_nm, d.ld_nm, d.R,
                               d.n_m, st));
        MARL_TRY(enc_bwd_rows(s, ns - 1, 0, c.DHs(ns)));
    }
    s.pln_blocks = c.plan.chain ? panel_chain_blocks(d.na, d.nb) : panel_bwd_blocks((int)d.R);
    for (int t = ns - 1; t >= 0; --t) {
        {
            LstmBwdBatch lb{};
            int nc = 0;
            if (!s.belief_done) lb.a[nc++] = cell_bwd_args(c, 0, t);
            if (!s.action_done) lb.a[nc++] = cell_bwd_args(c, 1, t);
            lb.rows = d.R;
            if (nc) MARL_TRY(launch_lstm_cell_bwd_batch(lb, nc, st));
        }
        s.action_done = s.belief_done = false;
        float* ddbar = c.at(c.e.DDBAR) + (size_t)t * s_nmo;
        float* ddbar2 = c.at(c.e.DDBAR2) + (size_t)t * s_nmo;
        MARL_TRY(bwd_recurrent(s, t, ddbar, ddbar2));
        if (c.plan.chain)
            MARL_TRY(bwd_step_chain(s, t, ddbar, ddbar2));
        else if (c.plan.panels_bwd)
            MARL_TRY(bwd_step_panels(s, t, ddbar, ddbar2));
        else
            MARL_TRY(bwd_step_rows(s, t, ddbar));
    }
    if (sb) {
        if (sb->d_msg) {
            if (c.opt.comm)
                MARL_TRY(launch_mix_msg(c.at(c.e.DMBAR), c.at(c.e.DMBAR), d.ld_nm, d.na, d.nb, d.n_m, c.opt.comm, 1, st));
            else
                MARL_TRY(launch_agg_msg(c.at(c.e.DMBAR), c.at(c.e.DMBAR), d.ld_nm, d.na, d.nb, d.n_m, st));
            MARL_TRY(launch_copy2d(c.at(c.e.DMBAR), d.ld_nm, sb->d_msg, d.n_m, d.R, d.n_m, st));
        }
        if (sb->d_h) MARL_TRY(launch_copy2d(c.DHs(0), d.ld_nb, sb->d_h, d.n_b, d.R, d.n_b, st));
        if (sb->d_c) MARL_TRY(launch_copy2d(c.at(c.e.DC), d.ld_nb, sb->d_c, d.n_b, d.R, d.n_b, st));
        if (sb->d_hc) MARL_TRY(launch_copy2d(c.DHCs(0), d.ld_na, sb->d_hc, d.n_a, d.R, d.n_a, st));
        if (sb->d_cc) MARL_TRY(launch_copy2d(c.at(c.e.DCC), d.ld_na, sb->d_cc, d.n_a, d.R, d.n_a, st));
    }
    if (c.plan.panels_bwd) {
        const int64_t nblk = s.pln_blocks;
        MARL_TRY(launch_reduce_affine(c.at(c.e.PLN[0]), nblk * ns, d.n_mo, grads[MARL_P_DEC_LN1W],
                                      grads[MARL_P_DEC_LN1B], 0, st, c.rq));
        MARL_TRY(launch_reduce_affine(c.at(c.e.PLN[1]), nblk * ns, d.nm2, grads[MARL_P_DEC_LN0W],
                                      grads[MARL_P_DEC_LN0B], 0, st, c.rq));
        if (ns > 1) {
            MARL_TRY(launch_reduce_affine(c.at(c.e.PLN[2]), nblk * (ns - 1), d.n_m,
                                          grads[MARL_P_ENC_LN1W], grads[MARL_P_ENC_LN1B], 0, st, c.rq));
            MARL_TRY(launch_reduce_affine(c.at(c.e.PLN[3]), nblk * (ns - 1), d.nm2,
                                          grads[MARL_P_ENC_LN0W], grads[MARL_P_ENC_LN0B], 0, st, c.rq));
        }
    }
    return MARL_OK;
}

static int bwd_chain_wgrads(const BwdState& s) {
    const Ctx& c = s.c;
    const Dims& d = c.d;
    float* const* grads = s.grads;
    const int64_t NR = d.NR;
    const int ns = d.ns;
    MARL_TRY(tn(c, c.at(c.e.DDBAR), d.ld_dbl, c.at(c.e.AD1, 0), d.ld_nm2, MARL_P_DEC_W1, d.n_mo, d.nm2, NR, grads[MARL_P_DEC_B1]));
    MARL_TRY(tn(c, c.at(c.e.DAD1), d.ld_nm2, c.at(c.e.MBAR, 0), d.ld_nm, MARL_P_DEC_W0, d.nm2, d.n_m, NR, grads[MARL_P_DEC_B0]));
    if (ns > 1 || s.enc_last) {
        const int64_t er = (int64_t)(s.enc_last ? ns : ns - 1) * d.R;
        MARL_TRY(tn(c, c.at(c.e.DZE2), d.ld_nm, c.at(c.e.AE1, 0), d.ld_nm2, MARL_P_ENC_W1, d.n_m, d.nm2, er, grads[MARL_P_ENC_B1]));
        MARL_TRY(tn(c, c.at(c.e.DAE1), d.ld_nm2, c.Hs(1), d.ld_nb, MARL_P_ENC_W0, d.nm2, d.n_b, er, grads[MARL_P_ENC_B0]));
    } else {
        const int enc[] = {MARL_P_ENC_B0, MARL_P_ENC_LN0W, MARL_P_ENC_LN0B, MARL_P_ENC_B1,
                           MARL_P_ENC_LN1W, MARL_P_ENC_LN1B};
        for (int i : enc) MARL_TRY(launch_fill(grads[i], param_meta(d, i).n, 0.f, c.st));
        MARL_TRY(launch_fill(c.gp(MARL_P_ENC_W0), (int64_t)d.nm2 * c.w.ldp[MARL_P_ENC_W0], 0.f, c.st));
        MARL_TRY(launch_fill(c.gp(MARL_P_ENC_W1), (int64_t)d.n_m * c.w.ldp[MARL_P_ENC_W1], 0.f, c.st));
    }
    for (int which = 0; which < 2; ++which) {
        const int n = which ? d.n_a : d.n_b;
        const int p_ih = which ? MARL_P_LA_WIH : MARL_P_LB_WIH, p_hh = which ? MARL_P_LA_WHH : MARL_P_LB_WHH;
        float* bias = grads[which ? MARL_P_LA_BIH : MARL_P_LB_BIH];
        if (c.plan.g3_tn) {
            const char* g3 = c.img(which ? c.e.GA3 : c.e.GB3);
            const char* h3 = c.img(which ? c.e.HC3 : c.e.H3);
            if (g3_tn_cell_ok(4 * n, d.nin, n, NR)) {
                MARL_TRY(tn3_cell(c, g3, 4 * n, c.img(c.e.U3), d.nin, p_ih, h3, n, p_hh, NR, bias));
            } else {
                MARL_TRY(tn3(c, g3, 4 * n, c.img(c.e.U3), d.nin, p_ih, NR, nullptr));
                MARL_TRY(tn3(c, g3, 4 * n, h3, n, p_hh, NR, bias));
            }
        } else {
            const float* g = c.at(which ? c.e.GA : c.e.GB, 0);
            const int ldg = which ? d.ld_ga : d.ld_gb;
            MARL_TRY(tn(c, g, ldg, c.at(c.e.U, 0), d.ld_nin, p_ih, 4 * n, d.nin, NR));
            MARL_TRY(tn(c, g, ldg, which ? c.HCs(0) : c.Hs(0), which ? d.ld_na : d.ld_nb, p_hh, 4 * n, n, NR, bias));
        }
    }
    return MARL_OK;
}


static int bwd_conv_wgrad(const BwdState& s, int l, const float* dz, const void* img, int img_u8) {
    const Ctx& c = s.c;
    const Dims& d = c.d;
    const int co = d.ch[l + 1];
    CnnWgradArgs w = cnn_wgrad_shape(d, l);
    w.dz = dz;
    w.img = img;
    w.img_u8 = img_u8;
    w.pos = c.POSs(0);
    if (l > 0) {
        w.zin = c.at(c.e.Z[l - 1], 0);
        w.gst = c.at(c.e.GST[l - 1], 0);
        w.gamma = c.wp(4 * (l - 1) + 2);
        w.beta = c.wp(4 * (l - 1) + 3);
    } else if (s.sb) {
        w.img = s.sb->obs;
        w.img_u8 = 0;
        w.nb = (int)d.R;
        w.H = w.W = d.f;
    } else if (!img) {
        set_error("episode_backward: the image batch of the forward call is needed");
        return MARL_EINVAL;
    }
    w.part_w = slab_scratch(c, (size_t)cnn_wgrad_blocks(w) * ((size_t)co * d.K[l] + co));
    MARL_TRY(launch_cnn_wgrad(w, c.st));
    return slab_reduce(c, w.part_w, w.part_b, w.blocks, co, d.K[l], 4 * l, s.grads[4 * l + 1]);
}

static int bwd_cnn_layers(const BwdState& s, const void* img, int img_u8, const float* d_img) {
    const Ctx& c = s.c;
    const Dims& d = c.d;
    float* const* grads = s.grads;
    hipStream_t st = c.st;
    const int64_t NR = d.NR;
    const float* da = c.at(c.e.DU);
    int64_t ldda = d.ld_nin;
    int chw = 1;
    bool have_dz = false;
    bool w0_done = false;
    for (int l = d.L - 1; l >= 0; --l) {
        const int co = d.ch[l + 1];
        const int64_t rows = NR * d.P[l];
        float* dz = c.at(c.e.DZ[l]);
        if (!have_dz) {
            RedQueue* q;
            float* part = part_scratch(c, gn_bwd_blocks(NR, co), co, 0, q);
            MARL_TRY(launch_gn_silu_bwd(da, ldda, chw, c.at(c.e.Z[l], 0), c.at(c.e.GST[l], 0),
                                        c.wp(4 * l + 2), c.wp(4 * l + 3), dz, part, NR, d.P[l], co,
                                        d.grp[l], st));
            MARL_TRY(launch_reduce_affine(part, gn_bwd_blocks(NR, co), co, grads[4 * l + 2],
                                          grads[4 * l + 3], 0, st, q));
        }
        have_dz = false;
        if (l == 0 && w0_done) {
        } else if (c.e.wgrad_ok[l]) {
            MARL_TRY(bwd_conv_wgrad(s, l, dz, img, img_u8));
        } else {
            MARL_TRY(tn(c, dz, co, c.at(c.e.COLS[l], 0), d.ldk[l], 4 * l, co, d.K[l], rows, grads[4 * l + 1]));
        }
        if (l == 0) break;
        CnnDgradArgs g = cnn_dgrad_shape(d, l);
        g.dz = dz;
        g.wt = c.wt(4 * l);
        g.ldwt = p4(co);
        g.zin = c.at(c.e.Z[l - 1], 0);
        g.gst = c.at(c.e.GST[l - 1], 0);
        g.gamma = c.wp(4 * (l - 1) + 2);
        g.beta = c.wp(4 * (l - 1) + 3);
        g.dzin = c.at(c.e.DZ[l - 1]);
        if (g.w0 && !img) g.w0 = 0;
        if (d_img) g.w0 = 0;
        if (c.e.dgrad_ok[l] && (size_t)cnn_dgrad_blocks(g) * 2 * d.ch[l] <= c.e.part_floats) {
            RedQueue* q;
            const int nblk = cnn_dgrad_blocks(g);
            g.part = part_scratch(c, nblk, d.ch[l], 0, q);
            const int co0 = d.ch[l], k0 = d.K[0];
            if (g.w0) {
                g.w0_part = slab_scratch(c, (size_t)nblk * ((size_t)co0 * k0 + co0));
                g.w0_bpart = g.w0_part + (size_t)nblk * co0 * k0;
                g.img = img;
                g.img_u8 = img_u8;
                g.pos = c.POSs(0);
                g.dzin = nullptr;
            }
            MARL_TRY(launch_cnn_dgrad(g, st));
            MARL_TRY(launch_reduce_affine(g.part, nblk, d.ch[l], grads[4 * (l - 1) + 2], grads[4 * (l - 1) + 3], 0,
                                          st, q));
            if (g.w0) {
                MARL_TRY(slab_reduce(c, g.w0_part, g.w0_bpart, nblk, co0, k0, 0, grads[1]));
                w0_done = true;
            }
            have_dz = true;
            continue;
        }
        MARL_TRY(gemm1(c, gemm_prob(dz, co, c.wtB(4 * l), c.at(c.e.DCOLS[l]), d.ldk[l], (int)rows, d.K[l])));
        MARL_TRY(launch_col2im(c.at(c.e.DCOLS[l]), d.ldk[l], c.at(c.e.DA[l - 1]), NR,
                               d.hw[l], d.ch[l], st));
        da = c.at(c.e.DA[l - 1]);
        ldda = (int64_t)d.P[l - 1] * d.ch[l];
        chw = 0;
    }
    return MARL_OK;
}

static int bwd_inputs(const BwdState& s, const void* img, int img_u8, float* d_img) {
    const Ctx& c = s.c;
    const Dims& d = c.d;
    float* const* grads = s.grads;
    hipStream_t st = c.st;
    const int64_t NR = d.NR;
    if (c.e.g3 && c.plan.panels_bwd) {
        G3Batch g{};
        g.p[0] = g3_prob(c.img(c.e.GB3), 0, c.wt3k(MARL_P_LB_WIH), 0, 4 * d.n_b, c.at(c.e.DU), d.ld_nin, (int)NR,
                         d.nf);
        g3_add_seg(g.p[0], c.img(c.e.GA3), 0, c.wt3k(MARL_P_LA_WIH), 0, 4 * d.n_a);
        g.count = 1;
        MARL_TRY(launch_gemm_nt3(g, st));
    } else {
        GemmProb p = gemm_prob(c.at(c.e.GB, 0), d.ld_gb, c.wtB(MARL_P_LB_WIH),
                               c.at(c.e.DU), d.ld_nin, (int)NR, c.plan.panels_bwd ? d.nf : d.nin);
        gemm_add_seg(p, c.at(c.e.GA, 0), d.ld_ga, c.wtB(MARL_P_LA_WIH));
        MARL_TRY(gemm1(c, p));
    }
    if (c.plan.panels_bwd)
        MARL_TRY(launch_add2d(c.at(c.e.DDBAR) + d.n_mo, d.ld_dbl, c.at(c.e.DDBAR2) + d.n_mo, d.ld_dbl,
                              c.at(c.e.DU) + d.nf + d.n_mo, d.ld_nin, NR, d.n_d, st));
    MARL_TRY(ln_bwd(c, c.at(c.e.DU) + d.nf + d.n_mo, d.ld_nin, c.at(c.e.ZPOS, 0), d.ld_nd,
                    c.at(c.e.STPOS, 0), MARL_P_POS_LNW, MARL_P_POS_LNB, NR, d.n_d, grads, 0,
                    c.at(c.e.DZPOS), d.ld_nd));
    MARL_TRY(tn(c, c.at(c.e.DZPOS), d.ld_nd, c.at(c.e.NPOS, 0), 4, MARL_P_POS_W, d.n_d, 2, NR, grads[MARL_P_POS_B]));
    MARL_TRY(bwd_cnn_layers(s, img, img_u8, d_img));
    if (d_img) {
        CnnDimgArgs a = cnn_dimg_shape(d);
        a.dz0 = c.at(c.e.DZ[0]);
        a.wt0 = c.wt(0);
        a.ldwt = c.w.ldt[0];
        a.pos = c.POSs(0);
        a.d_img = d_img;
        MARL_TRY(launch_cnn_dimg(a, st));
    }
    return MARL_OK;
}

static int episode_backward(const Ctx& c0, const void* img, int img_u8, const float* g_preds,
                            const float* g_logp, const float* g_values, float* const* grads,
                            const StepBwd* sb = nullptr, float* d_img = nullptr,
                            const float* g_probs = nullptr) {
    BwdState s;
    s.c = c0;
    s.grads = grads;
    s.sb = sb;
    s.enc_last = sb && sb->g_msg;
    Ctx& c = s.c;
    s.rq.reset(c.at(c.e.RED), c.e.red_floats, c.st);
    const int defer = tune_get("red_defer", 3);
    if (defer) c.rq = &s.rq;
    if (defer) c.tq = &s.tq;
    c.defer_slabs = defer == 2;
    c.defer_small = defer == 3 ? (size_t)8192 * 1024 : 0;
    for (int i = 0; i < MARL_NPARAMS; ++i)
        if (param_meta(c.d, i).kind != PK_NONE && !grads[i]) {
            set_error("gradient buffer %d is null", i);
            return MARL_EINVAL;
        }
    MARL_TRY(bwd_heads(s, g_preds, g_logp, g_values, g_probs));
    MARL_TRY(bwd_loop(s));
    MARL_TRY(bwd_chain_wgrads(s));
    MARL_TRY(bwd_inputs(s, img, img_u8, d_img));
    if (c.tq) MARL_TRY(launch_tn_queue(s.tq, c.rq, c.st));
    MARL_TRY(s.rq.flush());
    return unpack_grads(c, grads, s.heads_early ? 2 : 0);
}

}

using namespace marl;

extern "C" {

int marl_abi_version(void) { return MARL_ABI_VERSION; }

int64_t marl_param_numel(const marl_config* cfg, int index) {
    Dims d;
    if (make_dims(cfg, d) != MARL_OK || index < 0 || index >= MARL_NPARAMS) return -1;
    const ParamMeta m = param_meta(d, index);
    if (m.kind == PK_NONE) return 0;
    return m.kind == PK_VEC ? m.n : (int64_t)m.n * m.k;
}

int marl_workspace_sizes(const marl_config* cfg, int train, size_t* wbytes, size_t* ebytes) {
    Dims d;
    MARL_TRY(make_dims(cfg, d));
    WLayout w;
    make_wlayout(d, w);
    ELayout e;
    make_elayout(d, train, e);
    if (wbytes) *wbytes = w.total * sizeof(float);
    if (ebytes) *ebytes = e.total * sizeof(float);
    return MARL_OK;
}

int marl_pack_weights(const marl_config* cfg, const float* const* params_host, void* weights_ws,
                      size_t weights_ws_bytes, void* stream) {
    Dims d;
    MARL_TRY(make_dims(cfg, d));
    if (!params_host || !weights_ws) {
        set_error("null argument");
        return MARL_EINVAL;
    }
    WLayout w;
    make_wlayout(d, w);
    if (weights_ws_bytes < w.total * sizeof(float)) {
        set_error("pack_weights: weights workspace too small (%zu of %zu bytes)", weights_ws_bytes,
                  w.total * sizeof(float));
        return MARL_ESIZE;
    }
    return pack_weights(d, w, params_host, static_cast<float*>(weights_ws),
                        static_cast<hipStream_t>(stream));
}

int marl_patch_gather(const float* img, const int64_t* pos, float* obs, int nb_agents, int batch,
                      int c, int h, int w, int f, void* stream) {
    if (!img || !pos || !obs || nb_agents < 1 || batch < 1 || c < 1 || f < 1 || h < f || w < f) {
        set_error("patch_gather: bad argument");
        return MARL_EINVAL;
    }
    return launch_patch_gather(img, pos, obs, nb_agents, batch, c, h, w, f,
                               static_cast<hipStream_t>(stream));
}

}

namespace marl {
__global__ void transition_kernel(const int64_t* __restrict__ pos_in,
                                  const int64_t* __restrict__ actions,
                                  int64_t* __restrict__ pos_out, SampleArgs tbl, int rows, int nA,
                                  int H, int W, int f) {
    const int r = blockIdx.x * blockDim.x + threadIdx.x;
    if (r >= rows) return;
    int a = (int)actions[r];
    a = a < 0 ? 0 : (a >= nA ? nA - 1 : a);
    const int64_t p0 = pos_in[r * 2], p1 = pos_in[r * 2 + 1];
    const int64_t q0 = p0 + tbl.table[a][0], q1 = p1 + tbl.table[a][1];
    const bool ok = q0 >= 0 && q0 + f < H && q1 >= 0 && q1 + f < W;
    pos_out[r * 2] = ok ? q0 : p0;
    pos_out[r * 2 + 1] = ok ? q1 : p1;
}
}

extern "C" {

int marl_transition(const int64_t* pos_in, const int64_t* actions, int64_t* pos_out,
                    const int32_t* table_host, int nb_action, int rows, int h, int w, int f,
                    void* stream) {
    if (!pos_in || !actions || !pos_out || !table_host || nb_action < 1 ||
        nb_action > MARL_MAX_ACTIONS || rows < 1) {
        set_error("transition: bad argument");
        return MARL_EINVAL;
    }
    SampleArgs tbl;
    memset(&tbl, 0, sizeof(tbl));
    for (int j = 0; j < nb_action; ++j) {
        tbl.table[j][0] = table_host[2 * j];
        tbl.table[j][1] = table_host[2 * j + 1];
    }
    hipLaunchKernelGGL(transition_kernel, dim3((unsigned)cdiv(rows, 256)), dim3(256), 0,
                       static_cast<hipStream_t>(stream), pos_in, actions, pos_out, tbl, rows,
                       nb_action, h, w, f);
    MARL_LAUNCH_CHECK();
    return MARL_OK;
}

static int episode_forward_all(const marl_config* cfg, const void* weights_ws, size_t weights_ws_bytes,
                               void* episode_ws, size_t episode_ws_bytes, const void* img, const int64_t* pos0,
                               const float* h0, const float* c0, const float* hc0, const float* cc0,
                               const float* noise, const int64_t* forced_actions, uint64_t rng_seed,
                               uint64_t rng_offset, const void* counters, float* step_preds, float* step_logp,
                               float* step_values, int64_t* step_pos, int64_t* step_actions, float* step_probs,
                               int train, void* stream) {
    Ctx c;
    MARL_TRY(make_ctx(cfg, weights_ws, weights_ws_bytes, episode_ws, episode_ws_bytes, train, stream, c));
    if (!img || !pos0 || !h0 || !c0 || !hc0 || !cc0 || !step_preds || !step_logp || !step_values) {
        set_error("episode_forward: null argument");
        return MARL_EINVAL;
    }
    if (c.d.ns >= 65536) {
        set_error("episode_forward: more than 65535 steps");
        return MARL_ELIMIT;
    }
    const Dims& d = c.d;
    MARL_TRY(launch_i64_to_i32(pos0, c.POSs(0), d.R * 2, c.st));
    MARL_TRY(load_state(c, h0, c0, hc0, cc0, nullptr));
    StepIn in;
    in.img = img;
    in.img_u8 = cfg->img_u8 != 0;
    const SampleIo io{noise, forced_actions, rng_seed, rng_offset, counters, step_pos, step_actions, step_logp, true};
    for (int t = 0; t < d.ns; ++t) {
        SampleArgs a;
        fill_sample_args(c, cfg, t, io, a);
        if (c.plan.chain)
            MARL_TRY(fwd_step_chain(c, t, in, a));
        else if (c.plan.panels)
            MARL_TRY(fwd_step_panels(c, t, in, a));
        else
            MARL_TRY(fwd_step_rows(c, t, in, a));
    }
    MARL_TRY(heads_batched(c, 0, d.NR, step_values, step_preds));
    if (step_probs) MARL_TRY(launch_copy2d(c.PROBSs(0), d.nA, step_probs, d.nA, d.NR, d.nA, c.st));
    return MARL_OK;
}

int marl_episode_forward(const marl_config* cfg, const void* weights_ws, size_t weights_ws_bytes,
                         void* episode_ws, size_t episode_ws_bytes, const void* img, const int64_t* pos0, const float* h0, const float* c0,
                         const float* hc0, const float* cc0, const float* noise,
                         const int64_t* forced_actions, uint64_t rng_seed, uint64_t rng_offset,
                         const void* counters, float* step_preds, float* step_logp,
                         float* step_values, int64_t* step_pos, int64_t* step_actions, int train,
                         void* stream) {
    return episode_forward_all(cfg, weights_ws, weights_ws_bytes, episode_ws, episode_ws_bytes, img, pos0, h0, c0,
                               hc0, cc0, noise, forced_actions, rng_seed, rng_offset, counters, step_preds,
                               step_logp, step_values, step_pos, step_actions, nullptr, train, stream);
}

int marl_episode_forward_probs(const marl_config* cfg, const void* weights_ws, size_t weights_ws_bytes,
                               void* episode_ws, size_t episode_ws_bytes, const void* img, const int64_t* pos0,
                               const float* h0, const float* c0, const float* hc0, const float* cc0,
                               const float* noise, const int64_t* forced_actions, uint64_t rng_seed,
                               uint64_t rng_offset, const void* counters, float* step_preds, float* step_logp,
                               float* step_values, int64_t* step_pos, int64_t* step_actions, float* step_probs,
                               int train, void* stream) {
    if (!step_probs) {
        set_error("episode_forward_probs: null step_probs");
        return MARL_EINVAL;
    }
    return episode_forward_all(cfg, weights_ws, weights_ws_bytes, episode_ws, episode_ws_bytes, img, pos0, h0, c0,
                               hc0, cc0, noise, forced_actions, rng_seed, rng_offset, counters, step_preds,
                               step_logp, step_values, step_pos, step_actions, step_probs, train, stream);
}

static int episode_backward_entry(const char* who, bool need_dimg, const marl_config* cfg, void* weights_ws,
                                  size_t weights_ws_bytes, void* episode_ws, size_t episode_ws_bytes, const void* img,
                                  const float* g_preds, const float* g_logp, const float* g_values,
                                  float* const* grads_host, float* d_img, const float* g_probs, void* stream) {
    Ctx c;
    MARL_TRY(make_ctx(cfg, weights_ws, weights_ws_bytes, episode_ws, episode_ws_bytes, 1, stream, c));
    if (!grads_host) {
        set_error("%s: null gradient table", who);
        return MARL_EINVAL;
    }
    if (d_img || need_dimg) {
        if (cfg->img_u8 != 0) {
            set_error("%s: an integer (uint8) image batch has no gradient", who);
            return MARL_EINVAL;
        }
        if (!d_img || !img) {
            set_error("%s: null %s", who, d_img ? "img" : "d_img");
            return MARL_EINVAL;
        }
        if (!cnn_dimg_supported(cnn_dimg_shape(c.d))) {
            set_error("%s: shape outside the image-gradient kernel's range", who);
            return MARL_ELIMIT;
        }
    }
    return episode_backward(c, img, d_img ? 0 : cfg->img_u8 != 0, g_preds, g_logp, g_values, grads_host, nullptr,
                            d_img, g_probs);
}

int marl_episode_backward(const marl_config* cfg, void* weights_ws, size_t weights_ws_bytes,
                          void* episode_ws, size_t episode_ws_bytes, const void* img, const float* g_preds, const float* g_logp,
                          const float* g_values, float* const* grads_host, void* stream) {
    return episode_backward_entry("episode_backward", false, cfg, weights_ws, weights_ws_bytes, episode_ws,
                                  episode_ws_bytes, img, g_preds, g_logp, g_values, grads_host, nullptr, nullptr,
                                  stream);
}

int marl_episode_backward_img(const marl_config* cfg, void* weights_ws, size_t weights_ws_bytes,
                              void* episode_ws, size_t episode_ws_bytes, const void* img, const float* g_preds,
                              const float* g_logp, const float* g_values, float* const* grads_host, float* d_img,
                              void* stream) {
    return episode_backward_entry("episode_backward_img", true, cfg, weights_ws, weights_ws_bytes, episode_ws,
                                  episode_ws_bytes, img, g_preds, g_logp, g_values, grads_host, d_img, nullptr,
                                  stream);
}

int marl_episode_backward_probs(const marl_config* cfg, void* weights_ws, size_t weights_ws_bytes,
                                void* episode_ws, size_t episode_ws_bytes, const void* img, const float* g_preds,
                                const float* g_logp, const float* g_values, float* const* grads_host, float* d_img,
                                const float* g_probs, void* stream) {
    return episode_backward_entry("episode_backward_probs", false, cfg, weights_ws, weights_ws_bytes, episode_ws,
                                  episode_ws_bytes, img, g_preds, g_logp, g_values, grads_host, d_img, g_probs,
                                  stream);
}

int marl_backward_heads_event(void* hip_event) {
    g_installed.heads_event = static_cast<hipEvent_t>(hip_event);
    return MARL_OK;
}

int marl_comm_matrix(const float* m_dev, int nb_agents) {
    if (!m_dev) {
        g_installed.comm = nullptr;
        g_installed.comm_na = 0;
        return MARL_OK;
    }
    if (nb_agents < 1) {
        set_error("comm_matrix: %d agents", nb_agents);
        return MARL_EINVAL;
    }
    if (nb_agents > mix_msg_max_agents()) {
        set_error("comm_matrix: %d agents, the mixing kernel serves at most %d", nb_agents, mix_msg_max_agents());
        return MARL_ELIMIT;
    }
    g_installed.comm = m_dev;
    g_installed.comm_na = nb_agents;
    return MARL_OK;
}

int marl_comm_range(int radius, int metric, int normalize) {
    if (radius < 0) {
        g_installed.range = CommGate{nullptr, -1, 0, 1};
        return MARL_OK;
    }
    if (metric != MARL_COMM_CHEBYSHEV && metric != MARL_COMM_EUCLIDEAN) {
        set_error("comm_range: unknown metric %d", metric);
        return MARL_EINVAL;
    }
    g_installed.range = CommGate{nullptr, radius, metric, normalize != 0};
    return MARL_OK;
}

int marl_policy_explore(float temperature, float eps, int greedy) {
    if (!std::isfinite(temperature) || !(temperature > 0.f)) {
        set_error("policy_explore: temperature %g, need a finite value > 0", (double)temperature);
        return MARL_EINVAL;
    }
    if (!(eps >= 0.f && eps <= 0.5f)) {
        set_error("policy_explore: eps %g outside [0, 0.5]", (double)eps);
        return MARL_EINVAL;
    }
    const bool on = temperature != 1.f || eps != 0.f || greedy != 0;
    g_installed.explore = Explore{on, 1.0f / temperature, 1.0f - eps, eps, greedy != 0};
    return MARL_OK;
}

int marl_class_loss(const float* class_weights_dev, int nb_class, float label_smoothing,
// ... 171 lines not shown
    a.ns = d.ns;
    a.na = d.na;
    a.nb = d.nb;
    a.nc = d.nC;
    a.cls = k.on;
    if (k.on) {
        a.cls_w = k.w;
        a.cls_sw = k.sw;
        a.cls_eps = k.eps;
        a.cls_wrew = k.wrew;
    }
    return MARL_OK;
}

static void fill_loss_grads(LossGradArgs& a, const marl_config* cfg, const float* step_logp, const float* step_probs,
                            float entropy_coef, float* g_preds, float* g_logp, float* g_values, float* g_probs,
                            float* scalars_out) {
    a.logp = step_logp;
    a.g_preds = g_preds;
    a.ld_gp = a.nc;
    a.g_logp = g_logp;
    a.g_values = g_values;
    a.scalars = scalars_out;
    a.probs = step_probs;
    a.g_probs = g_probs;
    a.n_act = cfg->nb_action;
    a.entropy_coef = entropy_coef;
}

static int a2c_loss_all(const marl_config* cfg, void* episode_ws, size_t episode_ws_bytes, bool bad, const char* who,
                        const float* step_preds, const float* step_logp, const float* step_values, const int64_t* y,
                        float gamma, const float* step_probs, float entropy_coef, float* g_preds, float* g_logp,
                        float* g_values, float* g_probs, float* scalars_out, double* adv_stats, int phase,
                        void* stream) {
    LossArgs a;
    MARL_TRY(loss_entry(cfg, episode_ws, episode_ws_bytes,
                        bad || !episode_ws || !step_preds || !step_logp || !step_values || !y || !scalars_out ||
                            !adv_stats || phase < 0 || phase > 2,
                        who, step_preds, step_values, y, a));
    fill_loss_grads(a, cfg, step_logp, step_probs, entropy_coef, g_preds, g_logp, g_values, g_probs, scalars_out);
    a.adv_stats = adv_stats;
    a.gamma = gamma;
    a.phase = phase;
    return launch_loss(a, static_cast<hipStream_t>(stream));
}

int marl_a2c_loss_fwd_bwd(const marl_config* cfg, void* episode_ws, size_t episode_ws_bytes,
                          const float* step_preds,
                          const float* step_logp, const float* step_values, const int64_t* y,
                          float gamma, float* g_preds, float* g_logp, float* g_values,
                          float* scalars_out, double* adv_stats, int phase, void* stream) {
    return a2c_loss_all(cfg, episode_ws, episode_ws_bytes, false, "a2c_loss", step_preds, step_logp, step_values, y,
                        gamma, nullptr, 0.f, g_preds, g_logp, g_values, nullptr, scalars_out, adv_stats, phase,
                        stream);
}

int marl_a2c_loss_entropy_fwd_bwd(const marl_config* cfg, void* episode_ws, size_t episode_ws_bytes,
                                  const float* step_preds, const float* step_logp, const float* step_values,
                                  const int64_t* y, float gamma, const float* step_probs, float entropy_coef,
                                  float* g_preds, float* g_logp, float* g_values, float* g_probs,
                                  float* scalars_out, double* adv_stats, int phase, void* stream) {
    return a2c_loss_all(cfg, episode_ws, episode_ws_bytes, !step_probs || !g_probs || !(entropy_coef >= 0.f),
                        "a2c_loss_entropy", step_preds, step_logp, step_values, y, gamma, step_probs, entropy_coef,
                        g_preds, g_logp, g_values, g_probs, scalars_out, adv_stats, phase, stream);
}

int marl_advantages(const marl_config* cfg, void* episode_ws, size_t episode_ws_bytes, const float* step_preds,
                    const float* step_values, const int64_t* y, float gamma, float lam, float* advn, float* ret,
                    double* adv_stats, int phase, void* stream) {
    AdvArgs a;
    MARL_TRY(loss_entry(cfg, episode_ws, episode_ws_bytes,
                        !episode_ws || !step_preds || !step_values || !y || !advn || !ret || !adv_stats ||
                            phase < 0 || phase > 2 || !(lam >= 0.f && lam <= 1.f),
                        "advantages", step_preds, step_values, y, a));
    a.advn = advn;
    a.ret = ret;
    a.adv_stats = adv_stats;
    a.gamma = gamma;
    a.lam = lam;
    a.phase = phase;
    return launch_advantages(a, static_cast<hipStream_t>(stream));
}

int marl_ppo_loss_fwd_bwd(const marl_config* cfg, void* episode_ws, size_t episode_ws_bytes,
                          const float* step_preds, const float* step_logp, const float* step_values,
                          const int64_t* y, const float* old_logp, const float* advn, const float* ret,
                          float clip_eps, const float* step_probs, float entropy_coef, float* g_preds, float* g_logp,
                          float* g_values, float* g_probs, float* scalars_out, void* stream) {
    PpoArgs a;
    MARL_TRY(loss_entry(cfg, episode_ws, episode_ws_bytes,
                        !episode_ws || !step_preds || !step_logp || !step_values || !y || !old_logp || !advn ||
                            !ret || !scalars_out || !(clip_eps > 0.f) ||
                            (step_probs == nullptr) != (g_probs == nullptr) ||
                            (step_probs && !(entropy_coef >= 0.f)),
                        "ppo_loss", step_preds, step_values, y, a));
    fill_loss_grads(a, cfg, step_logp, step_probs, entropy_coef, g_preds, g_logp, g_values, g_probs, scalars_out);
    a.old_logp = old_logp;
    a.advn = advn;
    a.ret = ret;
    a.clip_eps = clip_eps;
    return launch_ppo_loss(a, static_cast<hipStream_t>(stream));
}

int marl_grad_clip(float* grads, int64_t n, float max_norm, float grad_scale, float* norm_out, void* scratch,
                   size_t scratch_bytes, void* stream) {
    if (!grads || n < 0 || !(max_norm > 0.f) || !(grad_scale > 0.f) || !norm_out || !scratch ||
        (reinterpret_cast<uintptr_t>(scratch) & 7) != 0) {
        set_error("grad_clip: bad argument");
        return MARL_EINVAL;
    }
    if (scratch_bytes < MARL_GRAD_CLIP_SCRATCH_BYTES) {
        set_error("grad_clip: scratch too small (%zu of %d bytes)", scratch_bytes, MARL_GRAD_CLIP_SCRATCH_BYTES);
        return MARL_ESIZE;
    }
    return launch_grad_clip(grads, n, max_norm, grad_scale, norm_out, static_cast<double*>(scratch),
                            static_cast<hipStream_t>(stream));
}

int marl_adam_step(float* params, const float* grads, float* exp_avg, float* exp_avg_sq, int64_t n,
                   int64_t step, float lr, float beta1, float beta2, float eps, float grad_scale,
                   const void* counters, void* stream) {
    if (!params || !grads || !exp_avg || !exp_avg_sq || n < 0 || step < 1) {
        set_error("adam: bad argument");
        return MARL_EINVAL;
    }
    const double bc1 = 1.0 - pow((double)beta1, (double)step);
    const double bc2 = 1.0 - pow((double)beta2, (double)step);
    return launch_adam(params, grads, exp_avg, exp_avg_sq, n, (float)((double)lr / bc1),
                       (float)(1.0 / sqrt(bc2)), beta1, beta2, eps, grad_scale,
                       static_cast<hipStream_t>(stream), static_cast<const Counters*>(counters));
}

}

static int step_forward(const marl_config* cfg, const void* weights_ws, size_t weights_ws_bytes, void* episode_ws,
                        size_t episode_ws_bytes, const float* obs, const float* msg, const float* norm_pos,
                        const float* h, const float* cc_, const float* hc, const float* cca, float* probs,
                        float* values, float* preds, float* new_msg, float* h_out, float* c_out, float* hc_out,
                        float* cc_out, const float* noise, uint64_t rng_seed, uint64_t rng_offset,
                        int64_t* actions_out, float* logp_out, int train, void* stream) {
    if (g_installed.range.radius >= 0) {
        set_error("step_forward: a communication range is installed - a single step has no integer positions of "
                  "the emission step; run the fused episode");
        return MARL_EINVAL;
    }
    Ctx c;
    MARL_TRY(make_ctx(cfg, weights_ws, weights_ws_bytes, episode_ws, episode_ws_bytes, train, stream, c));
    if (!obs || !msg || !norm_pos || !h || !cc_ || !hc || !cca || !probs || !values || !preds ||
        !new_msg || !h_out || !c_out || !hc_out || !cc_out) {
        set_error("step_forward: null argument");
        return MARL_EINVAL;
    }
    const Dims& d = c.d;
    MARL_TRY(load_state(c, h, cc_, hc, cca, msg));
    StepIn in;
    in.obs = obs;
    in.npos = norm_pos;
    MARL_TRY(step_core(c, 0, in));
    SampleIo io;
    if (actions_out && logp_out)
        io = SampleIo{noise, nullptr, rng_seed, rng_offset, nullptr, nullptr, actions_out, logp_out, false};
    SampleArgs a;
    fill_sample_args(c, cfg, 0, io, a);
    a.probs = probs;
    MARL_TRY(launch_sample(a, c.st, c.opt.explore.on));
    MARL_TRY(heads_batched(c, 0, d.R, values, preds));
    MARL_TRY(launch_copy2d(c.MSGs(1), d.ld_nm, new_msg, d.n_m, d.R, d.n_m, c.st));
    MARL_TRY(launch_copy2d(c.Hs(1), d.ld_nb, h_out, d.n_b, d.R, d.n_b, c.st));
    MARL_TRY(launch_copy2d(c.Cs(1), d.ld_nb, c_out, d.n_b, d.R, d.n_b, c.st));
    MARL_TRY(launch_copy2d(c.HCs(1), d.ld_na, hc_out, d.n_a, d.R, d.n_a, c.st));
    MARL_TRY(launch_copy2d(c.CCs(1), d.ld_na, cc_out, d.n_a, d.R, d.n_a, c.st));
    if (train)
        MARL_TRY(launch_copy2d(probs, d.nA, c.PROBSs(0), d.nA, d.R, d.nA, c.st));
    return MARL_OK;
}

extern "C" {

int marl_step_forward(const marl_config* cfg, const void* weights_ws, size_t weights_ws_bytes,
                      void* episode_ws, size_t episode_ws_bytes, const float* obs, const float* msg, const float* norm_pos, const float* h,
                      const float* cc_, const float* hc, const float* cca, float* probs,
                      float* values, float* preds, float* new_msg, float* h_out, float* c_out,
                      float* hc_out, float* cc_out, const float* noise, uint64_t rng_seed,
                      uint64_t rng_offset, int64_t* actions_out, float* logp_out, void* stream) {
    return step_forward(cfg, weights_ws, weights_ws_bytes, episode_ws, episode_ws_bytes, obs, msg, norm_pos, h, cc_,
                        hc, cca, probs, values, preds, new_msg, h_out, c_out, hc_out, cc_out, noise, rng_seed,
                        rng_offset, actions_out, logp_out, 0, stream);
}

int marl_step_forward_train(const marl_config* cfg, const void* weights_ws, size_t weights_ws_bytes,
                            void* step_ws, size_t step_ws_bytes, const float* obs, const float* msg,
                            const float* norm_pos, const float* h, const float* c, const float* hc,
                            const float* cc, float* probs, float* values, float* preds, float* new_msg,
                            float* h_out, float* c_out, float* hc_out, float* cc_out, const float* noise,
                            uint64_t rng_seed, uint64_t rng_offset, int64_t* actions_out, float* logp_out,
                            void* stream) {
    if (!cfg) {
        set_error("step_forward_train: null configuration");
        return MARL_EINVAL;
    }
    marl_config one = *cfg;
    one.nb_steps = 1;
    return step_forward(&one, weights_ws, weights_ws_bytes, step_ws, step_ws_bytes, obs, msg, norm_pos, h, c, hc, cc,
                        probs, values, preds, new_msg, h_out, c_out, hc_out, cc_out, noise, rng_seed, rng_offset,
                        actions_out, logp_out, 1, stream);
}

int marl_step_backward(const marl_config* cfg, void* weights_ws, size_t weights_ws_bytes, void* step_ws,
                       size_t step_ws_bytes, const float* obs, const float* g_probs, const float* g_logp,
                       const float* g_values, const float* g_preds, const float* g_msg, const float* g_h,
                       const float* g_c, const float* g_hc, const float* g_cc, float* const* grads_host,
                       float* d_msg, float* d_h, float* d_c, float* d_hc, float* d_cc, void* stream) {
    if (!cfg) {
        set_error("step_backward: null configuration");
        return MARL_EINVAL;
    }
    if (g_installed.range.radius >= 0) {
        set_error("step_backward: a communication range is installed - a single step has no integer positions of "
                  "the emission step; run the fused episode");
        return MARL_EINVAL;
    }
    marl_config one = *cfg;
    one.nb_steps = 1;
    Ctx c;
    MARL_TRY(make_ctx(&one, weights_ws, weights_ws_bytes, step_ws, step_ws_bytes, 1, stream, c));
    if (!grads_host || !obs) {
        set_error("step_backward: null gradient table or observation");
        return MARL_EINVAL;
    }
    StepBwd sb;
    sb.obs = obs;
    sb.g_probs = g_probs;
    sb.g_msg = g_msg;
    sb.g_h = g_h;
    sb.g_c = g_c;
    sb.g_hc = g_hc;
    sb.g_cc = g_cc;
    sb.d_msg = d_msg;
    sb.d_h = d_h;
    sb.d_c = d_c;
    sb.d_hc = d_hc;
    sb.d_cc = d_cc;
    return episode_backward(c, nullptr, 0, g_preds, g_logp, g_values, grads_host, &sb);
}

int marl_debug_buffer(const marl_config* cfg, int train, const char* name, int t,
                      int64_t* offset_floats, int* ld) {
    Dims d;
    MARL_TRY(make_dims(cfg, d));
    ELayout e;
    make_elayout(d, train, e);
    if (!name || !offset_floats || !ld || t < 0 || t > d.ns) return MARL_EINVAL;
    const size_t R = (size_t)d.R;
    const int ts = train ? t : 0;
    auto set = [&](size_t off, int l) {
        *offset_floats = (int64_t)off;
        *ld = l;
        return MARL_OK;
    };
    if (!strncmp(name, "WP", 2) || !strncmp(name, "WT", 2)) {
        const int idx = atoi(name + 2);
        WLayout w;
        make_wlayout(d, w);
        if (name[2] == 'F') {
            const int fi = atoi(name + 3);
            const size_t off = fi >= 0 && fi < MARL_NPARAMS ? (name[1] == 'P' ? w.wpf[fi] : w.wtf[fi]) : 0;
            if (!off) {
                set_error("parameter %d has no fragment-order copy", fi);
                return MARL_EINVAL;
            }
            return set(off, name[1] == 'P' ? w.gpf[fi] : w.gtf[fi]);
        }
        if (idx < 0 || idx >= MARL_NPARAMS || param_meta(d, idx).kind == PK_NONE) {
            set_error("no parameter %d", idx);
            return MARL_EINVAL;
        }
        return name[1] == 'P' ? set(w.wp[idx], w.ldp[idx]) : set(w.wt[idx], w.ldt[idx]);
    }
    if (!strcmp(name, "U")) return set(e.U.at(ts), d.ld_nin);
    if (!strcmp(name, "H")) return set(e.H + (size_t)t * R * d.ld_nb, d.ld_nb);
    if (!strcmp(name, "C")) return set(e.C + (size_t)t * R * d.ld_nb, d.ld_nb);
    if (!strcmp(name, "HC")) return set(e.HC + (size_t)t * R * d.ld_na, d.ld_na);
    if (!strcmp(name, "CC")) return set(e.CC + (size_t)t * R * d.ld_na, d.ld_na);
    if (!strcmp(name, "MSG")) return set(e.MSG + (size_t)t * R * d.ld_nm, d.ld_nm);
    if (!strcmp(name, "PROBS")) return set(e.PROBS + (size_t)t * R * d.nA, d.nA);
    if (!strcmp(name, "COLS0")) {
        if (e.fused_fwd && (!train || e.wgrad_ok[0])) {
            set_error("COLS0 is not materialised for this shape (fused CNN kernels)");
            return MARL_EINVAL;
        }
        return set(e.COLS[0].at(e.COLS[0].stride ? ts : 0), d.ldk[0]);
    }
    if (!strcmp(name, "Z0")) return set(e.Z[0].at(ts), d.ch[1]);
    if (!strcmp(name, "GB")) return set(e.GB.at(ts), d.ld_gb);
    if (train) {
        if (!strcmp(name, "DU")) return set(e.DU + (size_t)t * R * d.ld_nin, d.ld_nin);
        if (!strcmp(name, "DH")) return set(e.DH + (size_t)t * R * d.ld_nb, d.ld_nb);
        if (!strcmp(name, "DHC")) return set(e.DHC + (size_t)t * R * d.ld_na, d.ld_na);
    }
    set_error("unknown debug buffer %s", name);
    return MARL_EINVAL;
}

int marl_plan_query(const marl_config* cfg, int train, const char* key, int* value) {
    Dims d;
    MARL_TRY(make_dims(cfg, d));
    if (!key || !value) return MARL_EINVAL;
// ... 431 lines not shown
```

marlclassification_amd/csrc/gemm.hip:

```cpp
#include <stdlib.h>

#include "common.h"

namespace marl {

typedef float f32x16 __attribute__((ext_vector_type(16)));

constexpr int BK = 32;



__device__ __forceinline__ void lds_barrier() {
    asm volatile("s_waitcnt lgkmcnt(0)\n\ts_barrier" ::: "memory");
}

template <int BM, int BN, int WM, int WN, bool LSTM, int GROUPS>
__global__ __launch_bounds__(256 * GROUPS) void gemm_nt_kernel(const GemmBatch batch) {
    constexpr int BK = 32;
    constexpr int LDS_K = BK + 4;
    constexpr int KC = BK / 4;
    constexpr int TM = BM / WM / 32;
    constexpr int TN = BN / WN / 32;
    constexpr int A_CH = BM * KC / 256;
    constexpr int B_CH = BN * KC / 256 / GROUPS;
// ... 360 lines not shown
    float mk0 = 1.f, mk1 = 1.f, mk2 = 1.f, mk3 = 1.f;
    bool masked = false;
    const bool do_csum = csum != nullptr && by == 0;
    float4 cs = make_float4(0.f, 0.f, 0.f, 0.f);
#define MARL_TN_LOAD1(idx_, clamp_)                                                    \
    if (A_CH > (idx_)) {                                                               \
        uint32_t da_ = 0u, db_ = 0u;                                                   \
        if (clamp_) {                                                                  \
            const int64_t gr_ = base_ + (tid + 256 * (idx_)) / (BM / 4);               \
            const int64_t back_ = gr_ < r_end ? 0 : gr_ - (r_end - 1);                 \
            da_ = (uint32_t)(-(back_ * lda * 4));                                      \
            db_ = (uint32_t)(-(back_ * ldb * 4));                                      \
            mk##idx_ = gr_ < r_end ? 1.f : 0.f;                                        \
        }                                                                              \
        ra##idx_ = *reinterpret_cast<const float4*>(abase + (aof##idx_ + da_));        \
        rb##idx_ = *reinterpret_cast<const float4*>(bbase + (bof##idx_ + db_));        \
    }
#define MARL_TN_LOAD(tile_)                                                            \
    {                                                                                  \
        const int64_t base_ = r_begin + (int64_t)(tile_) * BK;                         \
        masked = base_ + BK > r_end;                                                   \
        if (!masked) {                                                                 \
            MARL_TN_LOAD1(0, false) MARL_TN_LOAD1(1, false) MARL_TN_LOAD1(2, false) MARL_TN_LOAD1(3, false) \
        } else {                                                                       \
            MARL_TN_LOAD1(0, true) MARL_TN_LOAD1(1, true) MARL_TN_LOAD1(2, true) MARL_TN_LOAD1(3, true) \
        }                                                                              \
        abase += (size_t)BK * lda * 4;                                                 \
        bbase += (size_t)BK * ldb * 4;                                                 \
    }
#define MARL_TN_STORE(idx_)                                                            \
    if (A_CH > (idx_)) {                                                               \
        const int c_ = tid + 256 * (idx_);                                             \
        float4 v_ = ra##idx_;                                                          \
        if (masked) {                                                                  \
            v_.x *= mk##idx_;                                                          \
            v_.y *= mk##idx_;                                                          \
            v_.z *= mk##idx_;                                                          \
            v_.w *= mk##idx_;                                                          \
        }                                                                              \
        if (do_csum) {                                                                 \
            cs.x += v_.x;                                                              \
            cs.y += v_.y;                                                              \
            cs.z += v_.z;                                                              \
            cs.w += v_.w;                                                              \
        }                                                                              \
        *reinterpret_cast<float4*>(As_ + (c_ / (BM / 4)) * BM + (c_ % (BM / 4)) * 4) = v_; \
        *reinterpret_cast<float4*>(Bs_ + (c_ / (BN / 4)) * BN + (c_ % (BN / 4)) * 4) = rb##idx_; \
    }

    const int fcol = lane & 31;
    const int fk = lane >> 5;
    if (T > 0) MARL_TN_LOAD(0)
    for (int tile = 0; tile < T; ++tile) {
        const int buf = NBUF == 2 ? (tile & 1) : 0;
        if (NBUF == 1 && tile > 0) lds_barrier();
        {
            float* As_ = smem + buf * BK * (BM + BN);
            float* Bs_ = As_ + BK * BM;
            MARL_TN_STORE(0) MARL_TN_STORE(1) MARL_TN_STORE(2) MARL_TN_STORE(3)
        }
        lds_barrier();
        if (tile + 1 < T) MARL_TN_LOAD(tile + 1)
        const float* As = smem + buf * BK * (BM + BN) + wm * (BM / WM) + fcol;
        const float* Bs = smem + buf * BK * (BM + BN) + BK * BM + wn * (BN / WN) + fcol;
        if (prio) __builtin_amdgcn_s_setprio(1);
#pragma unroll
        for (int ks = 0; ks < BK / 2; ++ks) {
            float a[TM], b[TN];
#pragma unroll
            for (int i = 0; i < TM; ++i) a[i] = As[(ks * 2 + fk) * BM + i * 32];
#pragma unroll
            for (int j = 0; j < TN; ++j) b[j] = Bs[(ks * 2 + fk) * BN + j * 32];
#pragma unroll
            for (int i = 0; i < TM; ++i)
#pragma unroll
                for (int j = 0; j < TN; ++j)
                    acc[i][j] = __builtin_amdgcn_mfma_f32_32x32x2f32(a[i], b[j], acc[i][j], 0, 0, 0);
        }
        if (prio) __builtin_amdgcn_s_setprio(0);
    }
#undef MARL_TN_LOAD1
#undef MARL_TN_LOAD
#undef MARL_TN_STORE

    if (do_csum) {
        constexpr int CPR = BM / 4;
        constexpr int SH = 256 / CPR;
        __syncthreads();
        float4* sh4 = reinterpret_cast<float4*>(smem);
        sh4[(tid / CPR) * CPR + (tid % CPR)] = cs;
        __syncthreads();
        if (tid < CPR) {
            float4 t = sh4[tid];
#pragma unroll
            for (int q = 1; q < SH; ++q) {
                const float4 u = sh4[q * CPR + tid];
                t.x += u.x;
                t.y += u.y;
                t.z += u.z;
                t.w += u.w;
            }
            float* co = csum + (size_t)bz * NI;
            const int ic = i0 + tid * 4;
            if (ic < NI) co[ic] = t.x;
            if (ic + 1 < NI) co[ic + 1] = t.y;
            if (ic + 2 < NI) co[ic + 2] = t.z;
            if (ic + 3 < NI) co[ic + 3] = t.w;
        }
    }

    float* o = out + (size_t)bz * out_split_stride;
    const int row_h = 4 * (lane >> 5);
#pragma unroll
    for (int i = 0; i < TM; ++i)
#pragma unroll
        for (int j = 0; j < TN; ++j) {
            const int col = j0 + wn * (BN / WN) + j * 32 + fcol;
            if (col >= NJ) continue;
#pragma unroll
            for (int r = 0; r < 16; ++r) {
                const int row = i0 + wm * (BM / WM) + i * 32 + (r & 3) + 8 * (r >> 2) + row_h;
                if (row < NI) o[(size_t)row * ldo + col] = acc[i][j][r];
            }
        }
}

template <int BM, int BN, int WM, int WN, int BK, int NBUF = 2>
__global__ __launch_bounds__(256) void gemm_tn_kernel(const float* __restrict__ A, int lda,
                                                      const float* __restrict__ B, int ldb,
                                                      float* __restrict__ out, int ldo,
                                                      int64_t out_split_stride, int NI, int NJ,
                                                      int64_t rows, int64_t rows_per_split,
                                                      float* __restrict__ csum, int gx, int gy,
                                                      int gz, int prio) {
    unsigned bx = blockIdx.x, by = blockIdx.y, bz = blockIdx.z;
    if (gx > 0) xcd_tile(gx, gy, gz, bx, by, bz);
    gemm_tn_body<BM, BN, WM, WN, BK, NBUF>(A, lda, B, ldb, out, ldo, out_split_stride, NI, NJ, rows, rows_per_split,
                                           csum, prio, bx, by, bz);
}

__global__ __launch_bounds__(256) void gemm_tn_batch_kernel(const TnBatch T) {
    int pi = 0;
    while (pi + 1 < T.count && (int)blockIdx.x >= T.p[pi + 1].first_block) ++pi;
    const TnBatchProb& P = T.p[pi];
    const unsigned local = blockIdx.x - (unsigned)P.first_block;
    const unsigned per = (unsigned)(P.gx * P.gy);
    const unsigned bz = local / per, r = local - bz * per;
    gemm_tn_body<64, 64, 2, 2, 32, 2>(P.a, P.lda, P.b, P.ldb, P.out, P.ldo, P.stride, P.ni, P.nj, P.rows, P.rows_per_split,
                                      P.csum, 0, r / (unsigned)P.gy, r % (unsigned)P.gy, bz);
}

__global__ __launch_bounds__(1024) void slab_reduce_kernel(
    const float* __restrict__ part, int64_t stride, int splits, float* __restrict__ c, int ldc,
    int NI, int NJ, const float* __restrict__ bpart, float* __restrict__ bias, int main_blocks) {
    __shared__ float sh[16][64];
    const int el = threadIdx.x & 63, g = threadIdx.x >> 6;
    const bool is_bias = (int)blockIdx.x >= main_blocks;
    const int64_t n = is_bias ? NI : (int64_t)NI * NJ;
    const int64_t e = (int64_t)(is_bias ? blockIdx.x - main_blocks : blockIdx.x) * 64 + el;
    const float* src = is_bias ? bpart : part;
    const int64_t st = is_bias ? NI : stride;
    float s0 = 0.f, s1 = 0.f, s2 = 0.f, s3 = 0.f;
    if (e < n) {
        int z = g;
        for (; z + 48 < splits; z += 64) {
            s0 += src[(size_t)z * st + e];
            s1 += src[(size_t)(z + 16) * st + e];
            s2 += src[(size_t)(z + 32) * st + e];
            s3 += src[(size_t)(z + 48) * st + e];
        }
        for (; z < splits; z += 16) s0 += src[(size_t)z * st + e];
    }
    sh[g][el] = (s0 + s1) + (s2 + s3);
    __syncthreads();
    if (g == 0 && e < n) {
        float t = sh[0][el];
#pragma unroll
        for (int q = 1; q < 16; ++q) t += sh[q][el];
        if (is_bias) {
            bias[e] = t;
        } else {
            const int i = (int)(e / NJ), j = (int)(e - (int64_t)i * NJ);
            c[(size_t)i * ldc + j] = t;
        }
    }
}

__global__ __launch_bounds__(1024) void slab_reduce4_kernel(
    const float* __restrict__ part, int64_t stride, int splits, float* __restrict__ c, int ldc,
    int NI, int NJ, const float* __restrict__ bpart, float* __restrict__ bias, int main_blocks) {
    __shared__ float4 sh[16][64];
    const int el = threadIdx.x & 63, g = threadIdx.x >> 6;
    if ((int)blockIdx.x >= main_blocks) {
        float* shf = reinterpret_cast<float*>(&sh[0][0]);
        const int64_t e = (int64_t)(blockIdx.x - main_blocks) * 64 + el;
        float s0 = 0.f, s1 = 0.f, s2 = 0.f, s3 = 0.f;
        if (e < NI) {
            int z = g;
            for (; z + 48 < splits; z += 64) {
                s0 += bpart[(size_t)z * NI + e];
                s1 += bpart[(size_t)(z + 16) * NI + e];
                s2 += bpart[(size_t)(z + 32) * NI + e];
                s3 += bpart[(size_t)(z + 48) * NI + e];
            }
            for (; z < splits; z += 16) s0 += bpart[(size_t)z * NI + e];
        }
        shf[g * 64 + el] = (s0 + s1) + (s2 + s3);
        __syncthreads();
        if (g == 0 && e < NI) {
            float t = shf[el];
#pragma unroll
            for (int q = 1; q < 16; ++q) t += shf[q * 64 + el];
            bias[e] = t;
        }
        return;
    }
    const int64_t n = (int64_t)NI * NJ;
    const int64_t e = ((int64_t)blockIdx.x * 64 + el) * 4;
    float4 s0 = make_float4(0.f, 0.f, 0.f, 0.f), s1 = s0, s2 = s0, s3 = s0;
#define MARL_ADD4(d_, v_) \
    {                     \
        const float4 t_ = (v_); \
        d_.x += t_.x;     \
        d_.y += t_.y;     \
        d_.z += t_.z;     \
        d_.w += t_.w;     \
    }
    if (e < n) {
        int z = g;
        for (; z + 48 < splits; z += 64) {
            const float4 v0 = *reinterpret_cast<const float4*>(part + (size_t)z * stride + e);
            const float4 v1 = *reinterpret_cast<const float4*>(part + (size_t)(z + 16) * stride + e);
            const float4 v2 = *reinterpret_cast<const float4*>(part + (size_t)(z + 32) * stride + e);
            const float4 v3 = *reinterpret_cast<const float4*>(part + (size_t)(z + 48) * stride + e);
            MARL_ADD4(s0, v0) MARL_ADD4(s1, v1) MARL_ADD4(s2, v2) MARL_ADD4(s3, v3)
        }
        for (; z < splits; z += 16) MARL_ADD4(s0, *reinterpret_cast<const float4*>(part + (size_t)z * stride + e))
    }
#undef MARL_ADD4
    sh[g][el] = make_float4((s0.x + s1.x) + (s2.x + s3.x), (s0.y + s1.y) + (s2.y + s3.y),
                            (s0.z + s1.z) + (s2.z + s3.z), (s0.w + s1.w) + (s2.w + s3.w));
    __syncthreads();
    if (g == 0 && e < n) {
        float4 t = sh[0][el];
#pragma unroll
        for (int q = 1; q < 16; ++q) {
            const float4 u = sh[q][el];
            t.x += u.x;
            t.y += u.y;
            t.z += u.z;
            t.w += u.w;
        }
        const int i = (int)(e / NJ), j = (int)(e - (int64_t)i * NJ);
        *reinterpret_cast<float4*>(c + (size_t)i * ldc + j) = t;
    }
}

int launch_slab_reduce(const float* part, int64_t stride, int splits, float* c, int ldc, int ni,
                       int nj, const float* bpart, float* bias, hipStream_t st) {
    if ((nj & 3) == 0 && (stride & 3) == 0 && (ldc & 3) == 0 && ((reinterpret_cast<uintptr_t>(part) |
                                                                  reinterpret_cast<uintptr_t>(c)) & 15) == 0) {
        const int main_blocks = (int)cdiv((int64_t)ni * nj, 256);
        const int extra = (bpart && bias) ? (int)cdiv(ni, 64) : 0;
        hipLaunchKernelGGL(slab_reduce4_kernel, dim3((unsigned)(main_blocks + extra)), dim3(1024), 0, st, part,
                           stride, splits, c, ldc, ni, nj, bpart, bias, main_blocks);
        MARL_LAUNCH_CHECK();
        return MARL_OK;
    }
    const int main_blocks = (int)cdiv((int64_t)ni * nj, 64);
    const int extra = (bpart && bias) ? (int)cdiv(ni, 64) : 0;
    hipLaunchKernelGGL(slab_reduce_kernel, dim3((unsigned)(main_blocks + extra)), dim3(1024), 0, st,
                       part, stride, splits, c, ldc, ni, nj, bpart, bias, main_blocks);
    MARL_LAUNCH_CHECK();
    return MARL_OK;
}

__global__ __launch_bounds__(1024) void red_batch_kernel(const RedBatch B) {
    __shared__ float sh[16][64];
    __shared__ int sdesc;
    const int el = threadIdx.x & 63, g = threadIdx.x >> 6;
    if (threadIdx.x == 0) {
        int i = 0;
        while (i + 1 < B.count && (int)blockIdx.x >= B.first_block[i + 1]) ++i;
        sdesc = i;
    }
    __syncthreads();
    const RedDesc D = B.d[sdesc];
    const int nb = (D.n + 63) >> 6, local = (int)blockIdx.x - B.first_block[sdesc];
    const int f = local / nb, e = (local - f * nb) * 64 + el;
    const int z0 = f * D.per, zn = D.count - z0 < D.per ? D.count - z0 : D.per;
    float s0 = 0.f, s1 = 0.f, s2 = 0.f, s3 = 0.f;
    if (e < D.n) {
        const float* p = D.part + (size_t)z0 * D.stride + e;
        int z = g;
        for (; z + 112 < zn; z += 128) {
            float v[8];
#pragma unroll
            for (int u = 0; u < 8; ++u) v[u] = p[(size_t)(z + 16 * u) * D.stride];
            s0 += v[0] + v[4];
            s1 += v[1] + v[5];
            s2 += v[2] + v[6];
            s3 += v[3] + v[7];
        }
        for (; z < zn; z += 16) s0 += p[(size_t)z * D.stride];
    }
    sh[g][el] = (s0 + s1) + (s2 + s3);
    __syncthreads();
    if (g == 0 && e < D.n) {
        float t = sh[0][el];
#pragma unroll
        for (int q = 1; q < 16; ++q) t += sh[q][el];
        float* o;
        if (D.folds > 1) {
            o = D.out0 + (size_t)f * D.n + e;
        } else if (e < D.split) {
            const int i = e / D.nj, j = e - i * D.nj;
            o = D.out0 + (size_t)i * D.ldc + j;
        } else {
            o = D.out1 + (e - D.split);
        }
        if (D.accumulate) t += *o;
        *o = t;
    }
}

int launch_red_batch(const RedBatch& b, hipStream_t st) {
    if (b.count <= 0) return MARL_OK;
    hipLaunchKernelGGL(red_batch_kernel, dim3((unsigned)b.first_block[b.count]), dim3(1024), 0, st, b);
    MARL_LAUNCH_CHECK();
    return MARL_OK;
}

void RedQueue::reset(float* s, size_t floats, hipStream_t stream) {
    scratch = s;
    cap = floats;
    off = 0;
    st = stream;
    rc = MARL_OK;
    stage1.count = stage2.count = 0;
    stage1.first_block[0] = stage2.first_block[0] = 0;
}

float* RedQueue::take(size_t floats, bool may_flush) {
    floats = (floats + 63) & ~(size_t)63;
    if (off + floats > cap) {
        if (!may_flush) return nullptr;
        (void)flush();
        if (floats > cap) {
            rc = MARL_ESIZE;
            set_error("reduction scratch too small (%zu > %zu floats)", floats, cap);
            return scratch;
        }
    }
    float* p = scratch + off;
    off += floats;
    return p;
}

static void red_add(RedBatch& b, const RedDesc& d) {
    b.d[b.count] = d;
    b.first_block[b.count + 1] = b.first_block[b.count] + d.folds * (int)cdiv(d.n, 64);
    ++b.count;
}

void RedQueue::push(const float* part, int64_t stride, int count, int n, float* out0, int split, int nj,
                    int ldc, float* out1, int accumulate) {
    if (rc != MARL_OK || n <= 0 || count <= 0) return;
    int folds = count > 1024 ? 64 : (count > 256 ? 16 : 1);
    if (stage2.count + 1 > kMaxRed || stage1.count + (folds > 1) > kMaxRed) (void)launch_pending();
    RedDesc d{part, stride, count, n, out0, split, nj, ldc, out1, accumulate, 1, count};
    if (folds > 1) {
        const int per = (int)cdiv(count, folds);
        folds = (int)cdiv(count, per);
        float* tmp = take((size_t)folds * n, false);
        if (tmp) {
            red_add(stage1, RedDesc{part, stride, count, n, tmp, n, n, n, nullptr, 0, folds, per});
            d.part = tmp;
            d.stride = n;
            d.count = d.per = folds;
        }
    }
    red_add(stage2, d);
}

int RedQueue::launch_pending() {
    if (rc == MARL_OK && stage1.count) rc = launch_red_batch(stage1, st);
    if (rc == MARL_OK && stage2.count) rc = launch_red_batch(stage2, st);
    stage1.count = stage2.count = 0;
    return rc;
}

int RedQueue::flush() {
    (void)launch_pending();
    off = 0;
    return rc;
}

GemmProb gemm_prob(const float* a, int lda, const GemmB& b, float* c, int ldc, int m, int n,
                   const float* bias, int accumulate) {
    GemmProb p{};
    p.seg[0] = GemmSeg{a, b.b, lda, b.ld, b.k, b.b3, b.kt3};
    p.nseg = 1;
    p.m = m;
    p.n = n;
    p.c = c;
    p.ldc = ldc;
    p.bias = bias;
    p.accumulate = accumulate;
    return p;
}

void gemm_add_seg(GemmProb& p, const float* a, int lda, const GemmB& b) {
    p.seg[1] = GemmSeg{a, b.b, lda, b.ld, b.k, b.b3, b.kt3};
    p.nseg = 2;
}


template <int BM, int BN, int WM, int WN, bool LSTM, int GROUPS>
static int launch_nt_variant(dim3 grid, const GemmBatch& batch_in, hipStream_t st) {
    GemmBatch batch = batch_in;
    batch.gx = (int)grid.x;
    batch.gy = (int)grid.y;
    batch.xcd_map = xcd_map_enabled() || (batch.count == 1 && !LSTM && tune_get("nt_xcd", 1));
    if (batch.xcd_map) grid = dim3(grid.x * grid.y * grid.z);
    constexpr size_t lds2 = (size_t)2 * (GROUPS * BM + BN) * (32 + 4) * sizeof(float);
    batch.single_buf = GROUPS == 1 && !LSTM && BM == 128 && true;
    const size_t lds = batch.single_buf ? lds2 / 2 : lds2;
    auto kern = gemm_nt_kernel<BM, BN, WM, WN, LSTM, GROUPS>;
    if (lds2 > 64 * 1024) {
        static bool raised = false;
        if (!raised) {
            MARL_HIP_CHECK(hipFuncSetAttribute(reinterpret_cast<const void*>(kern),
                                               hipFuncAttributeMaxDynamicSharedMemorySize, (int)lds2));
            raised = true;
        }
    }
    hipLaunchKernelGGL(kern, grid, dim3(256 * GROUPS), lds, st, batch);
    return MARL_OK;
}

int xcd_map_enabled() { return 0; }

static int gemm_groups() { return 1; }

static int check_prob(const GemmProb& p) {
    for (int s = 0; s < p.nseg; ++s) {
        const GemmSeg& g = p.seg[s];
        if (!g.a || !g.b || g.k <= 0 || (g.lda & 3) || (g.ldb & 3) ||
            (reinterpret_cast<uintptr_t>(g.a) & 15) || (reinterpret_cast<uintptr_t>(g.b) & 15) ||
            g.lda < p4(g.k) || g.ldb < p4(g.k)) {
            set_error("gemm: bad operand (seg %d: a=%p lda=%d b=%p ldb=%d k=%d)", s, (const void*)g.a,
                      g.lda, (const void*)g.b, g.ldb, g.k);
            return MARL_EINVAL;
        }
        const int64_t brows = p.h_next ? 4 * (int64_t)p.n : (int64_t)p.n;
        if ((int64_t)p.m * g.lda >= (1ll << 30) || brows * g.ldb >= (1ll << 30)) {
            set_error("gemm: operand of seg %d spans more than 4 GiB", s);
            return MARL_ELIMIT;
        }
    }
    if (p.m <= 0 || p.n <= 0) {
        set_error("gemm: empty problem m=%d n=%d", p.m, p.n);
        return MARL_EINVAL;
    }
    return MARL_OK;
}

int launch_gemm_nt(const GemmBatch& batch, hipStream_t st) {
    if (batch.count < 1 || batch.count > kMaxGemmBatch) return MARL_EINVAL;
    int max_m = 0, max_n = 0;
    int64_t blocks128 = 0;
    for (int i = 0; i < batch.count; ++i) {
        MARL_TRY(check_prob(batch.p[i]));
        if (!batch.p[i].c) return MARL_EINVAL;
        max_m = batch.p[i].m > max_m ? batch.p[i].m : max_m;
        max_n = batch.p[i].n > max_n ? batch.p[i].n : max_n;
        blocks128 += cdiv(batch.p[i].m, 128) * cdiv(batch.p[i].n, 128);
    }
    static const bool log_shapes = getenv("MARL_GEMM_LOG") != nullptr;
    if (log_shapes)
        for (int i = 0; i < batch.count; ++i)
            fprintf(stderr, "[gemm_nt] %d/%d m=%d n=%d k=%d+%d acc=%d bias=%d lda=%d ldc=%d\n", i,
                    batch.count, batch.p[i].m, batch.p[i].n, batch.p[i].seg[0].k,
                    batch.p[i].nseg > 1 ? batch.p[i].seg[1].k : 0, batch.p[i].accumulate,
                    batch.p[i].bias != nullptr, batch.p[i].seg[0].lda, batch.p[i].ldc);
    prof_before(1, st);
    if (split_mode()) {
        MARL_TRY(launch_gemm_nt_split(batch, max_m, max_n, blocks128, st));
    } else if (blocks128 >= 256 && max_n >= 96) {
        const int g = gemm_groups();
        dim3 grid((unsigned)cdiv(max_m, 128 * g), (unsigned)cdiv(max_n, 128), (unsigned)batch.count);
        if (g == 2)
            MARL_TRY((launch_nt_variant<128, 128, 2, 2, false, 2>(grid, batch, st)));
        else
            MARL_TRY((launch_nt_variant<128, 128, 2, 2, false, 1>(grid, batch, st)));
    } else {
        const int g = gemm_groups();
        dim3 grid((unsigned)cdiv(max_m, 64 * g), (unsigned)cdiv(max_n, 64), (unsigned)batch.count);
        if (g == 2)
            MARL_TRY((launch_nt_variant<64, 64, 2, 2, false, 2>(grid, batch, st)));
        else
            MARL_TRY((launch_nt_variant<64, 64, 2, 2, false, 1>(grid, batch, st)));
    }
    prof_after(1, st);
    MARL_LAUNCH_CHECK();
    return MARL_OK;
}

static int g_prof_class = -1;
static int g_prof_cap = 0, g_prof_n = 0;
static hipEvent_t* g_prof_ev = nullptr;

void prof_before(int cls, hipStream_t st) {
    if (cls == g_prof_class && g_prof_n < g_prof_cap) (void)hipEventRecord(g_prof_ev[2 * g_prof_n], st);
}
void prof_after(int cls, hipStream_t st) {
    if (cls == g_prof_class && g_prof_n < g_prof_cap) {
        (void)hipEventRecord(g_prof_ev[2 * g_prof_n + 1], st);
        ++g_prof_n;
    }
}

int profile_begin(int cls, int max_launches) {
// ... 226 lines not shown
```

marlclassification_amd/csrc/rowops.hip:

```cpp
#include <stdarg.h>
#include <stdlib.h>

#include <ctype.h>
#include <stdlib.h>
#include <string.h>

#include "common.h"
#include "sample.h"

namespace marl {

static thread_local char g_err[512] = "";
void set_error(const char* fmt, ...) {
    va_list ap;
    va_start(ap, fmt);
    vsnprintf(g_err, sizeof(g_err), fmt, ap);
    va_end(ap);
}
const char* last_error() { return g_err; }

namespace {
struct Knob {
    char key[32];
    int value;
    bool set;
};
constexpr int kMaxKnobs = 128;
Knob g_knobs[kMaxKnobs];
int g_nknobs = 0;
Knob* knob(const char* key, bool create) {
    for (int i = 0; i < g_nknobs; ++i)
        if (!strcmp(g_knobs[i].key, key)) return &g_knobs[i];
    if (!create || g_nknobs >= kMaxKnobs || strlen(key) >= sizeof(g_knobs[0].key)) return nullptr;
    Knob* k = &g_knobs[g_nknobs++];
    strcpy(k->key, key);
    k->value = 0;
    k->set = false;
    return k;
}
}

static const char* const kKnownKnobs[] = {
    "g3", "g3_lstm", "g3_tn", "g3_min_units", "g3_safe", "mfma_split", "g3_lstm_variant", "g3_nt_variant",
    "g3_tn_variant", "g3_tn_cell", "g3_tn_pipe", "g3_tn_wgs", "nt_xcd", "tn_xcd", "panel_chain", "red_defer",
    "tn_split_waves", "wgrad3", "cnn_fwd2", "cnn_fwd3", "dgrad_wgs", "dgrad_min_chunks",
    "g3_clk", "g3_tn_abl",
};

int tune_set(const char* key, int value) {
    bool known = false;
    for (const char* name : kKnownKnobs) known = known || !strcmp(name, key);
    if (!known) {
        set_error("marl_tune: unknown knob %s", key);
        return MARL_EINVAL;
    }
    Knob* k = knob(key, true);
    if (!k) {
        set_error("marl_tune: knob table full or key too long (%s)", key);
        return MARL_EINVAL;
    }
    k->value = value;
    k->set = true;
    return MARL_OK;
}

int tune_get(const char* key, int dflt) {
    Knob* k = knob(key, true);
    if (k && k->set) return k->value;
    char env[48] = "MARL_";
    size_t n = strlen(env);
    for (const char* c = key; *c && n + 1 < sizeof(env); ++c) env[n++] = (char)toupper((unsigned char)*c);
    env[n] = 0;
    const char* e = getenv(env);
    const int v = e ? atoi(e) : dflt;
    if (k && e) {
        k->value = v;
        k->set = true;
    }
    return v;
}

__device__ __forceinline__ float wave_max(float v) {
#pragma unroll
    for (int o = 32; o > 0; o >>= 1) v = fmaxf(v, __shfl_xor(v, o));
    return v;
}
__device__ __forceinline__ float silu_f(float y) { return silu_fast(y); }
__device__ __forceinline__ float silu_grad(float y) { return silu_grad_fast(y); }

__global__ __launch_bounds__(256) void ln_silu_fwd_kernel(const float* __restrict__ z, int ldz,
                                                          const float* __restrict__ gamma,
                                                          const float* __restrict__ beta,
                                                          float* __restrict__ out, int ldo,
                                                          float* __restrict__ stats, int64_t m,
                                                          int n) {
    const int lane = threadIdx.x & 63;
    const int64_t row = (int64_t)blockIdx.x * 4 + (threadIdx.x >> 6);
    if (row >= m) return;
    const float* zr = z + row * ldz;
    float s = 0.f;
    for (int c = lane; c < n; c += 64) s += zr[c];
    const float mean = wave_sum(s) / (float)n;
    float q = 0.f;
    for (int c = lane; c < n; c += 64) {
        const float d = zr[c] - mean;
        q += d * d;
    }
    const float rstd = 1.0f / sqrtf(wave_sum(q) / (float)n + 1e-5f);
    float* orow = out + row * ldo;
    for (int c = lane; c < n; c += 64) {
        const float y = (zr[c] - mean) * rstd * gamma[c] + beta[c];
        orow[c] = silu_f(y);
    }
    if (stats && lane == 0) {
        stats[row * 2] = mean;
        stats[row * 2 + 1] = rstd;
    }
}

template <int U>
__global__ __launch_bounds__(256) void ln_silu_fwd_reg_kernel(const float* __restrict__ z, int ldz,
                                                              const float* __restrict__ gamma,
                                                              const float* __restrict__ beta,
                                                              float* __restrict__ out, int ldo,
                                                              float* __restrict__ stats, int64_t m,
                                                              int n, const float* __restrict__ wdot,
                                                              const float* __restrict__ bdot,
                                                              float* __restrict__ dot_out, int64_t half) {
    const int lane = threadIdx.x & 63;
    const int64_t row0 = (int64_t)blockIdx.x * 4 + (threadIdx.x >> 6);
    if (row0 >= half) return;
    const int64_t rows[2] = {row0, row0 + half};
    const bool ok1 = rows[1] < m;
    float v[2][U], gm[U], bt[U], wd[U];
#pragma unroll
    for (int u = 0; u < U; ++u) {
        const int c = lane + 64 * u;
        v[0][u] = c < n ? z[rows[0] * ldz + c] : 0.f;
        v[1][u] = (c < n && ok1) ? z[rows[1] * ldz + c] : 0.f;
        gm[u] = c < n ? gamma[c] : 0.f;
        bt[u] = c < n ? beta[c] : 0.f;
        wd[u] = (c < n && wdot) ? wdot[c] : 0.f;
    }
#pragma unroll
    for (int k = 0; k < 2; ++k) {
        if (k == 1 && !ok1) break;
        const int64_t row = rows[k];
        float s = 0.f;
#pragma unroll
        for (int u = 0; u < U; ++u) s += v[k][u];
        const float mean = wave_sum(s) / (float)n;
        float q = 0.f;
#pragma unroll
        for (int u = 0; u < U; ++u) {
            const float d = (lane + 64 * u < n) ? v[k][u] - mean : 0.f;
            v[k][u] = d;
            q += d * d;
        }
        const float rstd = 1.0f / sqrtf(wave_sum(q) / (float)n + 1e-5f);
        float* orow = out + row * ldo;
        float dot = 0.f;
#pragma unroll
        for (int u = 0; u < U; ++u) {
            const int c = lane + 64 * u;
            if (c < n) {
                const float a = silu_f(v[k][u] * rstd * gm[u] + bt[u]);
                orow[c] = a;
                dot += a * wd[u];
            }
        }
        if (stats && lane == 0) {
            stats[row * 2] = mean;
            stats[row * 2 + 1] = rstd;
        }
        if (wdot) {
            dot = wave_sum(dot);
            if (lane == 0) dot_out[row] = dot + bdot[0];
        }
    }
}

int launch_ln_silu_fwd(const float* z, int ldz, const float* gamma, const float* beta, float* out,
                       int ldo, float* stats, int64_t m, int n, hipStream_t st, const float* wdot,
                       const float* bdot, float* dot_out) {
    if (m <= 0) return MARL_OK;
    const int64_t half = (m + 1) / 2;
    dim3 grid((unsigned)cdiv(n <= 384 ? half : m, 4)), blk(256);
    if (wdot && n > 384) {
        set_error("fused row dot needs a LayerNorm width <= 384");
        return MARL_ELIMIT;
    }
    if (n <= 128)
        hipLaunchKernelGGL(ln_silu_fwd_reg_kernel<2>, grid, blk, 0, st, z, ldz, gamma, beta, out, ldo,
                           stats, m, n, wdot, bdot, dot_out, half);
    else if (n <= 384)
        hipLaunchKernelGGL(ln_silu_fwd_reg_kernel<6>, grid, blk, 0, st, z, ldz, gamma, beta, out, ldo,
                           stats, m, n, wdot, bdot, dot_out, half);
    else
        hipLaunchKernelGGL(ln_silu_fwd_kernel, grid, blk, 0, st, z, ldz, gamma, beta, out, ldo, stats,
                           m, n);
    MARL_LAUNCH_CHECK();
    return MARL_OK;
}

static int bwd_waves(int n) { return n <= 512 ? 16 : (n <= 1024 ? 8 : 4); }
static int bwd_rows_per_wave(int64_t m, int waves) {
    int64_t r = cdiv(m, (int64_t)waves * 256);
    if (r < 1) r = 1;
    if (r > 64) r = 64;
    return (int)r;
}
int ln_bwd_blocks(int64_t m, int n) {
    const int w = bwd_waves(n);
    return (int)cdiv(m, (int64_t)w * bwd_rows_per_wave(m, w));
}

__global__ __launch_bounds__(1024) void ln_silu_bwd_kernel(
// ... 1275 lines not shown
}

int launch_lstm_cell_bwd2(const float* dh0, int lddh0, float* dc0, int lddc0, float* gates0,
                          int ldg0, const float* cp0, const float* cn0, int ldc0, int n0,
                          const float* dh1, int lddh1, float* dc1, int lddc1, float* gates1,
                          int ldg1, const float* cp1, const float* cn1, int ldc1, int n1,
                          int64_t rows, hipStream_t st) {
    LstmBwdBatch b{};
    b.a[0] = LstmBwdArgs{dh0, dc0, gates0, cp0, cn0, lddh0, lddc0, ldg0, ldc0, n0, nullptr, 0, 0, 0};
    b.a[1] = LstmBwdArgs{dh1, dc1, gates1, cp1, cn1, lddh1, lddc1, ldg1, ldc1, n1, nullptr, 0, 0, 0};
    b.rows = rows;
    return launch_lstm_cell_bwd_batch(b, 2, st);
}

template <int MAXA, bool EXPLORE = false>
__global__ __launch_bounds__(256) void sample_kernel(const SampleArgs A) {
    const int lane = threadIdx.x & 63;
    const int r = blockIdx.x * 4 + (threadIdx.x >> 6);
    if (r >= A.R) return;
    float p[MAXA];
    SamplePre<MAXA> S;
    sample_prefetch<MAXA>(A, r, lane, S);
    sample_row_logits<MAXA>(A, r, p, lane);
    sample_finish<MAXA, EXPLORE>(A, r, p, lane, S);
}

int launch_sample(const SampleArgs& a, hipStream_t st, bool explore) {
    if (a.nA > MARL_MAX_ACTIONS) return MARL_ELIMIT;
    if (explore) {
        if (a.nA <= 4)
            hipLaunchKernelGGL((sample_kernel<4, true>), dim3((unsigned)cdiv(a.R, 4)), dim3(256), 0, st, a);
        else
            hipLaunchKernelGGL((sample_kernel<MARL_MAX_ACTIONS, true>), dim3((unsigned)cdiv(a.R, 4)), dim3(256), 0, st, a);
    } else if (a.nA <= 4)
        hipLaunchKernelGGL(sample_kernel<4>, dim3((unsigned)cdiv(a.R, 4)), dim3(256), 0, st, a);
    else
        hipLaunchKernelGGL(sample_kernel<MARL_MAX_ACTIONS>, dim3((unsigned)cdiv(a.R, 4)), dim3(256), 0, st, a);
    MARL_LAUNCH_CHECK();
    return MARL_OK;
}

__global__ __launch_bounds__(256) void draw_episode_kernel(
    uint64_t seed, uint64_t offset, const uint64_t* __restrict__ offset_dev,
    int64_t* __restrict__ pos0, int R, int H, int W, int f,
    float* __restrict__ h0, float* __restrict__ c0, int64_t nb_el, float* __restrict__ hc0,
    float* __restrict__ cc0, int64_t na_el, float* __restrict__ noise, int64_t n_noise,
    int64_t q_pos, int64_t q_b, int64_t q_a, int64_t q_n) {
    if (offset_dev) offset += *offset_dev;
    const int64_t q = (int64_t)blockIdx.x * blockDim.x + threadIdx.x;
    int64_t rel = q;
    if (rel < q_pos) {
        const Philox4 u = philox4x32_10(seed, offset, (uint32_t)rel, 0u);
        const uint32_t uv[4] = {u.x, u.y, u.z, u.w};
#pragma unroll
        for (int i = 0; i < 4; ++i) {
            const int64_t e = rel * 4 + i;
            if (e < (int64_t)R * 2) {
                const uint32_t span = (uint32_t)(((e & 1) ? W : H) - f);
                pos0[e] = (int64_t)(((uint64_t)uv[i] * span) >> 32);
            }
        }
        return;
    }
    rel -= q_pos;
    float* dst = nullptr;
    int64_t n = 0;
    uint32_t stream = 1;
    bool normal = true;
    if (rel < q_b) {
        dst = h0, n = nb_el, stream = 1;
    } else if ((rel -= q_b) < q_b) {
        dst = c0, n = nb_el, stream = 2;
    } else if ((rel -= q_b) < q_a) {
        dst = hc0, n = na_el, stream = 3;
    } else if ((rel -= q_a) < q_a) {
        dst = cc0, n = na_el, stream = 4;
    } else if ((rel -= q_a) < q_n) {
        dst = noise, n = n_noise, stream = 5, normal = false;
    } else {
        return;
    }
    const Philox4 u = philox4x32_10(seed, offset, (uint32_t)rel, stream | ((uint32_t)(rel >> 32) << 8));
    float v[4];
    if (normal) {
        const float r0 = sqrtf(-2.0f * logf(philox_u01(u.x))), r1 = sqrtf(-2.0f * logf(philox_u01(u.z)));
        const float a0 = 6.283185307179586f * philox_u01(u.y), a1 = 6.283185307179586f * philox_u01(u.w);
        v[0] = r0 * cosf(a0);
        v[1] = r0 * sinf(a0);
        v[2] = r1 * cosf(a1);
        v[3] = r1 * sinf(a1);
    } else {
        v[0] = -logf(philox_u01(u.x));
        v[1] = -logf(philox_u01(u.y));
        v[2] = -logf(philox_u01(u.z));
        v[3] = -logf(philox_u01(u.w));
    }
#pragma unroll
    for (int i = 0; i < 4; ++i)
        if (rel * 4 + i < n) dst[rel * 4 + i] = v[i];
}

int launch_draw_episode(uint64_t seed, uint64_t offset, const uint64_t* offset_dev, int64_t* pos0,
                        int R, int H, int W, int f, float* h0, float* c0, int n_b, float* hc0,
                        float* cc0, int n_a, float* noise, int64_t n_noise, hipStream_t st) {
    const int64_t nb_el = (int64_t)R * n_b, na_el = (int64_t)R * n_a;
    const int64_t q_pos = cdiv((int64_t)R * 2, 4), q_b = cdiv(nb_el, 4), q_a = cdiv(na_el, 4),
                  q_n = noise ? cdiv(n_noise, 4) : 0;
    const int64_t total = q_pos + 2 * q_b + 2 * q_a + q_n;
    hipLaunchKernelGGL(draw_episode_kernel, dim3((unsigned)cdiv(total, 256)), dim3(256), 0, st, seed,
                       offset, offset_dev, pos0, R, H, W, f, h0, c0, nb_el, hc0, cc0, na_el, noise, n_noise, q_pos,
                       q_b, q_a, q_n);
    MARL_LAUNCH_CHECK();
    return MARL_OK;
}

__global__ void permute_kernel(const PermBatch B) {
    const PermDesc& d = B.d[blockIdx.y];
    const int64_t tot = (int64_t)d.rows * d.cols;
    if (d.frag > 0) {
        for (int64_t idx = (int64_t)blockIdx.x * blockDim.x + threadIdx.x; idx < tot;
             idx += (int64_t)gridDim.x * blockDim.x) {
            const int r = (int)(idx / d.cols), c = (int)(idx % d.cols);
            d.dst[panel_frag_index(r, c, d.frag)] = d.src[(int64_t)r * d.rs1 + c];
        }
        return;
    }
    for (int64_t idx = (int64_t)blockIdx.x * blockDim.x + threadIdx.x; idx < tot;
         idx += (int64_t)gridDim.x * blockDim.x) {
        const int r = (int)(idx / d.cols), c = (int)(idx % d.cols);
        const int64_t so = (int64_t)(r / d.rd) * d.rs1 + (int64_t)(r % d.rd) * d.rs2 +
                           (int64_t)(c / d.cd) * d.cs1 + (int64_t)(c % d.cd) * d.cs2;
        float v = d.src ? d.src[so] : 0.f;
        if (d.src2) v += d.src2[so];
        d.dst[(int64_t)r * d.dst_ld + c] = v;
    }
}

int launch_permute(const PermBatch& b, hipStream_t st) {
    if (b.count <= 0) return MARL_OK;
    if (b.count > kMaxPerm) return MARL_EINVAL;
    int64_t mx = 0;
    for (int i = 0; i < b.count; ++i) {
        const int64_t t = (int64_t)b.d[i].rows * b.d[i].cols;
        mx = t > mx ? t : mx;
    }
    int64_t gx = cdiv(mx, 256);
    if (gx > 1024) gx = 1024;
    if (gx < 1) gx = 1;
    hipLaunchKernelGGL(permute_kernel, dim3((unsigned)gx, (unsigned)b.count), dim3(256), 0, st, b);
    MARL_LAUNCH_CHECK();
    return MARL_OK;
}

__global__ void adam_kernel(float* __restrict__ p, const float* __restrict__ g,
                            float* __restrict__ m, float* __restrict__ v, int64_t n,
                            float step_size, float inv_sqrt_bc2, float beta1, float beta2,
                            float eps, float grad_scale, const Counters* __restrict__ cnt) {
    if (cnt) {
        step_size = cnt->lr_over_bc1;
        inv_sqrt_bc2 = cnt->inv_sqrt_bc2;
    }
    for (int64_t i = (int64_t)blockIdx.x * blockDim.x + threadIdx.x; i < n;
         i += (int64_t)gridDim.x * blockDim.x) {
        const float gr = g[i] * grad_scale;
        const float mi = m[i] + (1.0f - beta1) * (gr - m[i]);
        const float vi = v[i] * beta2 + (1.0f - beta2) * (gr * gr);
        m[i] = mi;
        v[i] = vi;
        const float denom = sqrtf(vi) * inv_sqrt_bc2 + eps;
        p[i] = p[i] - step_size * (mi / denom);
    }
}

int launch_adam(float* p, const float* g, float* m, float* v, int64_t n, float lr_over_bc1,
                float inv_sqrt_bc2, float beta1, float beta2, float eps, float grad_scale,
                hipStream_t st, const Counters* cnt) {
    if (n <= 0) return MARL_OK;
    int64_t gx = cdiv(n, 256);
    if (gx > 4096) gx = 4096;
    hipLaunchKernelGGL(adam_kernel, dim3((unsigned)gx), dim3(256), 0, st, p, g, m, v, n,
                       lr_over_bc1, inv_sqrt_bc2, beta1, beta2, eps, grad_scale, cnt);
    MARL_LAUNCH_CHECK();
    return MARL_OK;
}

__global__ void counters_kernel(Counters* c, uint64_t rng_offset, int64_t step, float lr, float beta1,
                                float beta2, int tick) {
    if (blockIdx.x != 0 || threadIdx.x != 0) return;
    uint64_t off = rng_offset, st = (uint64_t)step;
    if (tick) {
        off = c->rng_offset + 1;
        st = c->step + 1;
    }
    c->rng_offset = off;
    c->step = st;
    const double bc1 = 1.0 - pow((double)beta1, (double)st);
    const double bc2 = 1.0 - pow((double)beta2, (double)st);
    c->lr_over_bc1 = (float)((double)lr / bc1);
    c->inv_sqrt_bc2 = (float)(1.0 / sqrt(bc2));
}

int launch_counters_set(Counters* c, uint64_t rng_offset, int64_t step, float lr, float beta1,
                        float beta2, int tick, hipStream_t st) {
    hipLaunchKernelGGL(counters_kernel, dim3(1), dim3(64), 0, st, c, rng_offset, step, lr, beta1, beta2, tick);
    MARL_LAUNCH_CHECK();
    return MARL_OK;
}

__global__ void fill_kernel(float* p, int64_t n, float v) {
    for (int64_t i = (int64_t)blockIdx.x * blockDim.x + threadIdx.x; i < n;
         i += (int64_t)gridDim.x * blockDim.x)
        p[i] = v;
}
int launch_fill(float* p, int64_t n, float v, hipStream_t st) {
    if (n <= 0) return MARL_OK;
    int64_t gx = cdiv(n, 256);
    if (gx > 8192) gx = 8192;
    hipLaunchKernelGGL(fill_kernel, dim3((unsigned)gx), dim3(256), 0, st, p, n, v);
    MARL_LAUNCH_CHECK();
    return MARL_OK;
}

__global__ void copy2d_kernel(const float* __restrict__ src, int64_t lds, float* __restrict__ dst,
                              int64_t ldd, int64_t rows, int cols) {
    const int64_t tot = rows * cols;
    for (int64_t i = (int64_t)blockIdx.x * blockDim.x + threadIdx.x; i < tot;
         i += (int64_t)gridDim.x * blockDim.x) {
        const int64_t r = i / cols;
        const int c = (int)(i % cols);
        dst[r * ldd + c] = src[r * lds + c];
    }
}
__global__ void add2d_kernel(const float* __restrict__ a, int64_t lda, const float* __restrict__ b,
                             int64_t ldb, float* __restrict__ out, int64_t ldo, int64_t rows, int cols) {
    const int64_t idx = (int64_t)blockIdx.x * blockDim.x + threadIdx.x;
    if (idx >= rows * cols) return;
    const int64_t r = idx / cols;
    const int c = (int)(idx % cols);
    out[r * ldo + c] = a[r * lda + c] + b[r * ldb + c];
}
int launch_add2d(const float* a, int64_t lda, const float* b, int64_t ldb, float* out, int64_t ldo,
                 int64_t rows, int cols, hipStream_t st) {
    if (rows <= 0 || cols <= 0) return MARL_OK;
    hipLaunchKernelGGL(add2d_kernel, dim3((unsigned)cdiv(rows * cols, 256)), dim3(256), 0, st, a, lda, b,
                       ldb, out, ldo, rows, cols);
    MARL_LAUNCH_CHECK();
    return MARL_OK;
}

int launch_copy2d(const float* src, int64_t lds, float* dst, int64_t ldd, int64_t rows, int cols,
                  hipStream_t st) {
    if (rows <= 0 || cols <= 0) return MARL_OK;
    int64_t gx = cdiv(rows * cols, 256);
    if (gx > 8192) gx = 8192;
    hipLaunchKernelGGL(copy2d_kernel, dim3((unsigned)gx), dim3(256), 0, st, src, lds, dst, ldd, rows,
                       cols);
    MARL_LAUNCH_CHECK();
    return MARL_OK;
}

__global__ void i64_to_i32_kernel(const int64_t* __restrict__ s, int32_t* __restrict__ d,
                                  int64_t n) {
    const int64_t i = (int64_t)blockIdx.x * blockDim.x + threadIdx.x;
    if (i < n) d[i] = (int32_t)s[i];
}
int launch_i64_to_i32(const int64_t* src, int32_t* dst, int64_t n, hipStream_t st) {
    if (n <= 0) return MARL_OK;
    hipLaunchKernelGGL(i64_to_i32_kernel, dim3((unsigned)cdiv(n, 256)), dim3(256), 0, st, src, dst,
                       n);
    MARL_LAUNCH_CHECK();
    return MARL_OK;
}

__global__ void policy_dlogits_kernel(const float* __restrict__ dlogp,
                                      const float* __restrict__ probs,
                                      const int32_t* __restrict__ actions, float* __restrict__ out,
                                      int ld, int64_t rows, int nA) {
    const int64_t idx = (int64_t)blockIdx.x * blockDim.x + threadIdx.x;
    if (idx >= rows * nA) return;
    const int64_t r = idx / nA;
    const int j = (int)(idx % nA);
    const float g = dlogp ? dlogp[r] : 0.f;
    out[r * ld + j] = g * ((j == actions[r] ? 1.0f : 0.0f) - probs[r * nA + j]);
}
int launch_policy_dlogits(const float* dlogp, const float* probs, const int32_t* actions,
                          float* out, int ld, int64_t rows, int nA, hipStream_t st) {
    hipLaunchKernelGGL(policy_dlogits_kernel, dim3((unsigned)cdiv(rows * nA, 256)), dim3(256), 0,
                       st, dlogp, probs, actions, out, ld, rows, nA);
    MARL_LAUNCH_CHECK();
    return MARL_OK;
}

__global__ void policy_dlogits_probs_kernel(const float* __restrict__ dlogp,
                                            const float* __restrict__ dprobs,
                                            const float* __restrict__ probs,
                                            const int32_t* __restrict__ actions,
                                            float* __restrict__ out, int ld, int64_t rows, int nA) {
    const int64_t r = (int64_t)blockIdx.x * blockDim.x + threadIdx.x;
    if (r >= rows) return;
    const float* p = probs + r * nA;
    const float* g = dprobs + r * nA;
    float s = 0.f;
    for (int j = 0; j < nA; ++j) s = fmaf(p[j], g[j], s);
    const float gl = dlogp ? dlogp[r] : 0.f;
    const int a = dlogp ? actions[r] : -1;
    for (int j = 0; j < nA; ++j)
// ... 199 lines not shown
```

Measured before the change: 9.360 million agent-env-steps/s.

## Fuse weight packing, episode-start copies, and write grads directly to flat buffers

Replaces the chain of permute/copy launches that pack parameters into the weight workspace with a single tiled pack kernel driven by a cached table. It also merges the episode-start state copies, image conversions and position cast into one kernel. Weight gradients for matrix and conv params are now written straight into the caller's gradient buffers, with the conv index permutation applied inside the slab reduce, and the duplicate bhh bias gradient is written in the same reduce. Together these remove several launches and a gradient copy pass per iteration, at the cost of more complex indexing and an env-var fallback path.

New measurement: 9.411 million agent-env-steps/s (median of 6 runs). Within noise of the previous version (+0.5%).

```diff
diff --git a/marlclassification_amd/csrc/common.h b/marlclassification_amd/csrc/common.h
--- a/marlclassification_amd/csrc/common.h
+++ b/marlclassification_amd/csrc/common.h
@@ -18,6 +18,7 @@
 
 int tune_get(const char* key, int dflt);
 int tune_set(const char* key, int value);
+int tune_epoch();
 
 __device__ __forceinline__ float rcp_fast(float x) { return __builtin_amdgcn_rcpf(x); }
 __device__ __forceinline__ float sigmoid_acc(float x) { return rcp_fast(1.0f + __expf(-x)); }
@@ -283,6 +284,7 @@
     float* out1;
     int accumulate;
     int folds, per;
+    int ci;
 };
 constexpr int kMaxRed = 40;
 struct RedBatch {
@@ -299,7 +301,7 @@
     void reset(float* s, size_t floats, hipStream_t stream);
     float* take(size_t floats, bool may_flush = true);
     void push(const float* part, int64_t stride, int count, int n, float* out0, int split, int nj,
-              int ldc, float* out1, int accumulate);
+              int ldc, float* out1, int accumulate, int ci = 0);
     int launch_pending();
     int flush();
 };
@@ -454,6 +456,51 @@
     int count;
 };
 int launch_permute(const PermBatch& b, hipStream_t st);
+
+struct PackMat {
+    uint32_t wp, wt, wp3, wt3, wp3k, wt3k, wpf, wtf, wf;
+    int n, k;
+    int ldp, ldt;
+    int gpf, gtf;
+    int ci;
+    int param;
+    int tile0;
+};
+struct PackVec {
+    uint32_t dst;
+    int n;
+    short a, b;
+};
+constexpr int kMaxPackMat = MARL_MAX_CNN_LAYERS + 16;
+constexpr int kMaxPackVec = MARL_NPARAMS + 2;
+struct PackTable {
+    PackMat m[kMaxPackMat];
+    PackVec v[kMaxPackVec];
+    int nm, nv, tiles;
+};
+struct PackParams {
+    const float* p[MARL_NPARAMS];
+};
+int launch_pack_weights(const PackTable& t, const PackParams& p, float* W, hipStream_t st);
+
+struct StartCopy {
+    const float* src;
+    float* dst;
+    int64_t rows;
+    int cols, lds, ldd;
+};
+struct StartDesc {
+    StartCopy c[5];
+    const float* img_src[2];
+    char* img_dst[2];
+    int img_k[2];
+    int nimg;
+    int64_t rows;
+    const int64_t* pos;
+    int32_t* pos_dst;
+    int64_t npos;
+};
+int launch_episode_start(const StartDesc& s, hipStream_t st);
 
 __host__ __device__ inline int panel_frag_groups(int K) { return (K + 15) >> 4; }
 __host__ __device__ inline size_t panel_frag_floats(int n, int K) {
@@ -814,7 +861,8 @@
 };
 CnnWgradPlanInfo cnn_wgrad_launch_plan(const CnnWgradArgs& a);
 int launch_slab_reduce(const float* part, int64_t stride, int splits, float* c, int ldc, int ni,
-                       int nj, const float* bpart, float* bias, hipStream_t st);
+                       int nj, const float* bpart, float* bias, hipStream_t st, int conv_ci = 0,
+                       float* bias2 = nullptr);
 
 int launch_gather_im2col(const void* img, int img_u8, const int32_t* pos, float* cols, int ldk,
                          int na, int nb, int c_img, int cin, int H, int W, int f, hipStream_t st);
diff --git a/marlclassification_amd/csrc/episode.hip b/marlclassification_amd/csrc/episode.hip
--- a/marlclassification_amd/csrc/episode.hip
+++ b/marlclassification_amd/csrc/episode.hip
@@ -621,7 +621,15 @@
     }
     const float* wpf(int i) const { return w.wpf[i] ? W + w.wpf[i] : nullptr; }
     const float* wtf(int i) const { return w.wtf[i] ? W + w.wtf[i] : nullptr; }
-    float* gp(int i) const { return W + w.gp[i]; }
+    float* const* gflat = nullptr;
+    bool g_direct(int i) const {
+        if (!gflat) return false;
+        const ParamKind k = param_meta(d, i).kind;
+        return k == PK_MATRIX || (k == PK_CONV && e.wgrad_ok[i / 4]);
+    }
+    float* gp(int i) const { return g_direct(i) ? gflat[i] : W + w.gp[i]; }
+    int gld(int i) const { return g_direct(i) ? param_meta(d, i).k : w.ldp[i]; }
+    bool bhh_by_reduce() const { return gflat && plan.g3_tn; }
     float* at(size_t off) const { return E + off; }
     float* at(const SBuf& s, int t) const { return E + s.at(train ? t : 0); }
     float* Hs(int t) const { return E + e.H + (size_t)t * d.R * d.ld_nb; }
@@ -1244,9 +1252,33 @@
     return perm(src, dst, (int)rows, cols, (int)ldd, 1, (int)lds, 0, 1, 1, 0);
 }
 
-static int load_state(const Ctx& c, const float* h, const float* cc_, const float* hc,
+static bool edge_fused() {
+    const char* v = getenv("MARL_EDGE_FUSED");
+    return !(v && v[0] == '0');
+}
+
+static int load_state(const Ctx& c, const int64_t* pos0, const float* h, const float* cc_, const float* hc,
                       const float* cca, const float* msg) {
     const Dims& d = c.d;
+    if (edge_fused()) {
+        StartDesc s{};
+        s.c[0] = StartCopy{h, c.Hs(0), d.R, d.n_b, d.n_b, d.ld_nb};
+        s.c[1] = StartCopy{cc_, c.Cs(0), d.R, d.n_b, d.n_b, d.ld_nb};
+        s.c[2] = StartCopy{hc, c.HCs(0), d.R, d.n_a, d.n_a, d.ld_na};
+        s.c[3] = StartCopy{cca, c.CCs(0), d.R, d.n_a, d.n_a, d.ld_na};
+        s.c[4] = StartCopy{msg, c.MSGs(0), d.R, msg ? d.n_m : d.ld_nm, d.n_m, d.ld_nm};
+        s.rows = d.R;
+        if (c.e.g3) {
+            s.nimg = 2;
+            s.img_src[0] = h, s.img_dst[0] = c.img(c.e.H3), s.img_k[0] = d.n_b;
+            s.img_src[1] = hc, s.img_dst[1] = c.img(c.e.HC3), s.img_k[1] = d.n_a;
+        }
+        s.pos = pos0;
+        s.pos_dst = c.POSs(0);
+        s.npos = d.R * 2;
+        return launch_episode_start(s, c.st);
+    }
+    if (pos0) MARL_TRY(launch_i64_to_i32(pos0, c.POSs(0), d.R * 2, c.st));
     PermQueue q(c.st);
     q.push(copy_desc(h, d.n_b, c.Hs(0), d.ld_nb, d.R, d.n_b));
     q.push(copy_desc(cc_, d.n_b, c.Cs(0), d.ld_nb, d.R, d.n_b));
@@ -1265,9 +1297,69 @@
     return MARL_OK;
 }
 
-
-static int pack_weights(const Dims& d, const WLayout& w, const float* const* params, float* W,
-                        hipStream_t st) {
+static void make_pack_table(const Dims& d, const WLayout& w, PackTable& t) {
+    memset(&t, 0, sizeof(t));
+    for (int i = 0; i < MARL_NPARAMS; ++i) {
+        const ParamMeta m = param_meta(d, i);
+        if (m.kind == PK_MATRIX || m.kind == PK_CONV) {
+            PackMat& p = t.m[t.nm++];
+            p.wp = (uint32_t)w.wp[i], p.wt = (uint32_t)w.wt[i];
+            p.wp3 = (uint32_t)w.wp3[i], p.wt3 = (uint32_t)w.wt3[i];
+            p.wp3k = (uint32_t)w.wp3k[i], p.wt3k = (uint32_t)w.wt3k[i];
+            p.wpf = (uint32_t)w.wpf[i], p.wtf = (uint32_t)w.wtf[i], p.wf = (uint32_t)w.wf[i];
+            p.n = m.n, p.k = m.k, p.ldp = w.ldp[i], p.ldt = w.ldt[i], p.gpf = w.gpf[i], p.gtf = w.gtf[i];
+            p.ci = m.kind == PK_CONV ? m.k / 9 : 0;
+            p.param = i;
+            p.tile0 = t.tiles;
+            t.tiles += ((m.n + 31) / 32) * ((m.k + 31) / 32);
+        } else if (m.kind == PK_VEC) {
+            t.v[t.nv++] = PackVec{(uint32_t)w.wp[i], m.n, (short)i, (short)-1};
+        }
+    }
+    t.v[t.nv++] = PackVec{(uint32_t)w.bsum_b, 4 * d.n_b, (short)MARL_P_LB_BIH, (short)MARL_P_LB_BHH};
+    t.v[t.nv++] = PackVec{(uint32_t)w.bsum_a, 4 * d.n_a, (short)MARL_P_LA_BIH, (short)MARL_P_LA_BHH};
+}
+static const PackTable& pack_table(const Dims& d, const WLayout& w) {
+    struct Cached {
+        Dims d;
+        int epoch;
+        size_t total;
+        PackTable t;
+    };
+    static thread_local Cached c;
+    static thread_local bool valid = false;
+    const int epoch = tune_epoch();
+    if (!valid || c.epoch != epoch || c.total != w.total || memcmp(&c.d, &d, sizeof(Dims)) != 0) {
+        make_pack_table(d, w, c.t);
+        memcpy(&c.d, &d, sizeof(Dims));
+        c.epoch = epoch;
+        c.total = w.total;
+        valid = true;
+    }
+    return c.t;
+}
+
+static int pack_weights_chain(const Dims& d, const WLayout& w, const float* const* params, float* W, hipStream_t st);
+static int pack_weights(const Dims& d, const WLayout& w, const float* const* params, float* W, hipStream_t st) {
+    if (!edge_fused()) return pack_weights_chain(d, w, params, W, st);
+    if (w.total >> 32) {
+        set_error("pack_weights: weights workspace beyond 2^32 floats");
+        return MARL_ELIMIT;
+    }
+    PackParams p{};
+    for (int i = 0; i < MARL_NPARAMS; ++i) {
+        if (param_meta(d, i).kind == PK_NONE) continue;
+        if (!params[i]) {
+            set_error("parameter %d is null", i);
+            return MARL_EINVAL;
+        }
+        p.p[i] = params[i];
+    }
+    return launch_pack_weights(pack_table(d, w), p, W, st);
+}
+
+static int pack_weights_chain(const Dims& d, const WLayout& w, const float* const* params, float* W,
+                              hipStream_t st) {
     PermQueue q(st);
     for (int i = 0; i < MARL_NPARAMS; ++i) {
         const ParamMeta m = param_meta(d, i);
@@ -1346,6 +1438,7 @@
         const bool head = i >= MARL_P_POL_W0 && i <= MARL_P_PRE_B1;
         if ((which == 1 && !head) || (which == 2 && head)) continue;
         const ParamMeta m = param_meta(c.d, i);
+        if (c.g_direct(i)) continue;
         if (m.kind == PK_MATRIX) {
             q.push(perm(c.gp(i), grads[i], m.n, m.k, m.k, 1, c.w.ldp[i], 0, 1, 1, 0));
         } else if (m.kind == PK_CONV) {
@@ -1353,7 +1446,7 @@
             q.push(perm(c.gp(i), grads[i], m.n, m.k, m.k, 1, c.w.ldp[i], 0, 9, 1, ci));
         }
     }
-    if (which != 1) {
+    if (which != 1 && !c.bhh_by_reduce()) {
         q.push(perm(grads[MARL_P_LB_BIH], grads[MARL_P_LB_BHH], 1, 4 * c.d.n_b, 4 * c.d.n_b, 1, 0, 0, 1, 1, 0));
         q.push(perm(grads[MARL_P_LA_BIH], grads[MARL_P_LA_BHH], 1, 4 * c.d.n_a, 4 * c.d.n_a, 1, 0, 0, 1, 1, 0));
     }
@@ -1364,10 +1457,11 @@
 static int tn(const Ctx& c, const float* a, int lda, const float* b, int ldb, int pidx, int ni,
               int nj, int64_t rows, float* bias = nullptr) {
     RedQueue* q = c.defer_this(gemm_tn_scratch_bytes(ni, nj, rows)) ? c.rq : nullptr;
-    return launch_gemm_tn(a, lda, b, ldb, c.gp(pidx), c.w.ldp[pidx], ni, nj, rows, c.at(c.e.TNS),
+    return launch_gemm_tn(a, lda, b, ldb, c.gp(pidx), c.gld(pidx), ni, nj, rows, c.at(c.e.TNS),
                           c.e.tns_bytes, c.st, bias, q, q ? c.tq : nullptr);
 }
-static int tn3(const Ctx& c, const char* a3, int ni, const char* b3, int nj, int pidx, int64_t rows, float* bias) {
+static int tn3(const Ctx& c, const char* a3, int ni, const char* b3, int nj, int pidx, int64_t rows, float* bias,
+               float* bias2 = nullptr) {
     const G3TnPlan plan = g3_tn_plan(ni, nj, rows);
     if (g3_tn_scratch_bytes(ni, nj, rows) > c.e.tns_bytes) {
         set_error("tn3: scratch too small");
@@ -1387,10 +1481,11 @@
     a.rows = rows;
     a.csum = bias ? scratch + (size_t)plan.splits * ni * nj : nullptr;
     MARL_TRY(launch_gemm_tn3(a, plan, c.st));
-    return launch_slab_reduce(scratch, (int64_t)ni * nj, plan.splits, c.gp(pidx), c.w.ldp[pidx], ni, nj, a.csum, bias, c.st);
+    return launch_slab_reduce(scratch, (int64_t)ni * nj, plan.splits, c.gp(pidx), c.gld(pidx), ni, nj, a.csum, bias, c.st, 0,
+                              bias2);
 }
 static int tn3_cell(const Ctx& c, const char* g3, int ni, const char* u3, int nin, int p_ih, const char* h3, int nh,
-                    int p_hh, int64_t rows, float* bias) {
+                    int p_hh, int64_t rows, float* bias, float* bias2) {
     const G3TnPlan plan = g3_tn_cell_plan(ni, nin, nh, rows);
     if (g3_tn_cell_scratch_bytes(ni, nin, nh, rows) > c.e.tns_bytes) {
         set_error("tn3_cell: scratch too small");
@@ -1416,8 +1511,8 @@
     hh.out = s_hh;
     hh.out_split_stride = (int64_t)ni * nh;
     MARL_TRY(launch_gemm_tn3_cell(ih, hh, plan, c.st));
-    MARL_TRY(launch_slab_reduce(s_ih, (int64_t)ni * nin, plan.splits, c.gp(p_ih), c.w.ldp[p_ih], ni, nin, nullptr, nullptr, c.st));
-    return launch_slab_reduce(s_hh, (int64_t)ni * nh, plan.splits, c.gp(p_hh), c.w.ldp[p_hh], ni, nh, ih.csum, bias, c.st);
+    MARL_TRY(launch_slab_reduce(s_ih, (int64_t)ni * nin, plan.splits, c.gp(p_ih), c.gld(p_ih), ni, nin, nullptr, nullptr, c.st));
+    return launch_slab_reduce(s_hh, (int64_t)ni * nh, plan.splits, c.gp(p_hh), c.gld(p_hh), ni, nh, ih.csum, bias, c.st, 0, bias2);
 }
 static float* part_scratch(const Ctx& c, int64_t blocks, int n, int acc, RedQueue*& q) {
     q = acc ? nullptr : c.rq;
@@ -1512,12 +1607,13 @@
     return c.at(c.e.TNS);
 }
 static int slab_reduce(const Ctx& c, float* part_w, float* part_b, int blocks, int co, int k, int pidx, float* bias) {
+    const int ci = c.g_direct(pidx) ? k / 9 : 0;
     if (c.rq && part_w != c.at(c.e.TNS)) {
-        c.rq->push(part_w, (int64_t)co * k, blocks, co * k, c.gp(pidx), co * k, k, c.w.ldp[pidx], nullptr, 0);
+        c.rq->push(part_w, (int64_t)co * k, blocks, co * k, c.gp(pidx), co * k, k, c.gld(pidx), nullptr, 0, ci);
         c.rq->push(part_b, co, blocks, co, bias, co, co, co, nullptr, 0);
         return MARL_OK;
     }
-    return launch_slab_reduce(part_w, (int64_t)co * k, blocks, c.gp(pidx), c.w.ldp[pidx], co, k, part_b, bias, c.st);
+    return launch_slab_reduce(part_w, (int64_t)co * k, blocks, c.gp(pidx), c.gld(pidx), co, k, part_b, bias, c.st, ci);
 }
 
 struct BwdState {
@@ -1848,21 +1944,22 @@
         const int enc[] = {MARL_P_ENC_B0, MARL_P_ENC_LN0W, MARL_P_ENC_LN0B, MARL_P_ENC_B1,
                            MARL_P_ENC_LN1W, MARL_P_ENC_LN1B};
         for (int i : enc) MARL_TRY(launch_fill(grads[i], param_meta(d, i).n, 0.f, c.st));
-        MARL_TRY(launch_fill(c.gp(MARL_P_ENC_W0), (int64_t)d.nm2 * c.w.ldp[MARL_P_ENC_W0], 0.f, c.st));
-        MARL_TRY(launch_fill(c.gp(MARL_P_ENC_W1), (int64_t)d.n_m * c.w.ldp[MARL_P_ENC_W1], 0.f, c.st));
+        MARL_TRY(launch_fill(c.gp(MARL_P_ENC_W0), (int64_t)d.nm2 * c.gld(MARL_P_ENC_W0), 0.f, c.st));
+        MARL_TRY(launch_fill(c.gp(MARL_P_ENC_W1), (int64_t)d.n_m * c.gld(MARL_P_ENC_W1), 0.f, c.st));
     }
     for (int which = 0; which < 2; ++which) {
         const int n = which ? d.n_a : d.n_b;
         const int p_ih = which ? MARL_P_LA_WIH : MARL_P_LB_WIH, p_hh = which ? MARL_P_LA_WHH : MARL_P_LB_WHH;
         float* bias = grads[which ? MARL_P_LA_BIH : MARL_P_LB_BIH];
+        float* bias2 = c.bhh_by_reduce() ? grads[which ? MARL_P_LA_BHH : MARL_P_LB_BHH] : nullptr;
         if (c.plan.g3_tn) {
             const char* g3 = c.img(which ? c.e.GA3 : c.e.GB3);
             const char* h3 = c.img(which ? c.e.HC3 : c.e.H3);
             if (g3_tn_cell_ok(4 * n, d.nin, n, NR)) {
-                MARL_TRY(tn3_cell(c, g3, 4 * n, c.img(c.e.U3), d.nin, p_ih, h3, n, p_hh, NR, bias));
+                MARL_TRY(tn3_cell(c, g3, 4 * n, c.img(c.e.U3), d.nin, p_ih, h3, n, p_hh, NR, bias, bias2));
             } else {
                 MARL_TRY(tn3(c, g3, 4 * n, c.img(c.e.U3), d.nin, p_ih, NR, nullptr));
-                MARL_TRY(tn3(c, g3, 4 * n, h3, n, p_hh, NR, bias));
+                MARL_TRY(tn3(c, g3, 4 * n, h3, n, p_hh, NR, bias, bias2));
             }
         } else {
             const float* g = c.at(which ? c.e.GA : c.e.GB, 0);
@@ -2028,6 +2125,7 @@
     s.sb = sb;
     s.enc_last = sb && sb->g_msg;
     Ctx& c = s.c;
+    if (edge_fused()) c.gflat = grads;
     s.rq.reset(c.at(c.e.RED), c.e.red_floats, c.st);
     const int defer = tune_get("red_defer", 3);
     if (defer) c.rq = &s.rq;
@@ -2165,8 +2263,7 @@
         return MARL_ELIMIT;
     }
     const Dims& d = c.d;
-    MARL_TRY(launch_i64_to_i32(pos0, c.POSs(0), d.R * 2, c.st));
-    MARL_TRY(load_state(c, h0, c0, hc0, cc0, nullptr));
+    MARL_TRY(load_state(c, pos0, h0, c0, hc0, cc0, nullptr));
     StepIn in;
     in.img = img;
     in.img_u8 = cfg->img_u8 != 0;
@@ -2644,7 +2741,7 @@
         return MARL_EINVAL;
     }
     const Dims& d = c.d;
-    MARL_TRY(load_state(c, h, cc_, hc, cca, msg));
+    MARL_TRY(load_state(c, nullptr, h, cc_, hc, cca, msg));
     StepIn in;
     in.obs = obs;
     in.npos = norm_pos;
diff --git a/marlclassification_amd/csrc/gemm.hip b/marlclassification_amd/csrc/gemm.hip
--- a/marlclassification_amd/csrc/gemm.hip
+++ b/marlclassification_amd/csrc/gemm.hip
@@ -536,7 +536,8 @@
 
 __global__ __launch_bounds__(1024) void slab_reduce_kernel(
     const float* __restrict__ part, int64_t stride, int splits, float* __restrict__ c, int ldc,
-    int NI, int NJ, const float* __restrict__ bpart, float* __restrict__ bias, int main_blocks) {
+    int NI, int NJ, const float* __restrict__ bpart, float* __restrict__ bias, int main_blocks, int ci,
+    float* __restrict__ bias2) {
     __shared__ float sh[16][64];
     const int el = threadIdx.x & 63, g = threadIdx.x >> 6;
     const bool is_bias = (int)blockIdx.x >= main_blocks;
@@ -563,16 +564,21 @@
         for (int q = 1; q < 16; ++q) t += sh[q][el];
         if (is_bias) {
             bias[e] = t;
+            if (bias2) bias2[e] = t;
         } else {
-            const int i = (int)(e / NJ), j = (int)(e - (int64_t)i * NJ);
+            const int i = (int)(e / NJ);
+            int j = (int)(e - (int64_t)i * NJ);
+            if (ci > 0) j = (j % ci) * 9 + j / ci;
             c[(size_t)i * ldc + j] = t;
         }
     }
 }
 
+template <bool CONV>
 __global__ __launch_bounds__(1024) void slab_reduce4_kernel(
     const float* __restrict__ part, int64_t stride, int splits, float* __restrict__ c, int ldc,
-    int NI, int NJ, const float* __restrict__ bpart, float* __restrict__ bias, int main_blocks) {
+    int NI, int NJ, const float* __restrict__ bpart, float* __restrict__ bias, int main_blocks, int ci,
+    float* __restrict__ bias2) {
     __shared__ float4 sh[16][64];
     const int el = threadIdx.x & 63, g = threadIdx.x >> 6;
     if ((int)blockIdx.x >= main_blocks) {
@@ -596,6 +602,7 @@
 #pragma unroll
             for (int q = 1; q < 16; ++q) t += shf[q * 64 + el];
             bias[e] = t;
+            if (bias2) bias2[e] = t;
         }
         return;
     }
@@ -636,25 +643,37 @@
             t.w += u.w;
         }
         const int i = (int)(e / NJ), j = (int)(e - (int64_t)i * NJ);
-        *reinterpret_cast<float4*>(c + (size_t)i * ldc + j) = t;
+        if (CONV) {
+            float* o = c + (size_t)i * ldc + (j % ci) * 9 + j / ci;
+            o[0] = t.x;
+            o[9] = t.y;
+            o[18] = t.z;
+            o[27] = t.w;
+        } else {
+            *reinterpret_cast<float4*>(c + (size_t)i * ldc + j) = t;
+        }
     }
 }
 
 int launch_slab_reduce(const float* part, int64_t stride, int splits, float* c, int ldc, int ni,
-                       int nj, const float* bpart, float* bias, hipStream_t st) {
+                       int nj, const float* bpart, float* bias, hipStream_t st, int conv_ci, float* bias2) {
     if ((nj & 3) == 0 && (stride & 3) == 0 && (ldc & 3) == 0 && ((reinterpret_cast<uintptr_t>(part) |
                                                                   reinterpret_cast<uintptr_t>(c)) & 15) == 0) {
         const int main_blocks = (int)cdiv((int64_t)ni * nj, 256);
         const int extra = (bpart && bias) ? (int)cdiv(ni, 64) : 0;
-        hipLaunchKernelGGL(slab_reduce4_kernel, dim3((unsigned)(main_blocks + extra)), dim3(1024), 0, st, part,
-                           stride, splits, c, ldc, ni, nj, bpart, bias, main_blocks);
+        if (conv_ci > 0)
+            hipLaunchKernelGGL(slab_reduce4_kernel<true>, dim3((unsigned)(main_blocks + extra)), dim3(1024), 0, st, part,
+                               stride, splits, c, ldc, ni, nj, bpart, bias, main_blocks, conv_ci, bias2);
+        else
+            hipLaunchKernelGGL(slab_reduce4_kernel<false>, dim3((unsigned)(main_blocks + extra)), dim3(1024), 0, st, part,
+                               stride, splits, c, ldc, ni, nj, bpart, bias, main_blocks, conv_ci, bias2);
         MARL_LAUNCH_CHECK();
         return MARL_OK;
     }
     const int main_blocks = (int)cdiv((int64_t)ni * nj, 64);
     const int extra = (bpart && bias) ? (int)cdiv(ni, 64) : 0;
     hipLaunchKernelGGL(slab_reduce_kernel, dim3((unsigned)(main_blocks + extra)), dim3(1024), 0, st,
-                       part, stride, splits, c, ldc, ni, nj, bpart, bias, main_blocks);
+                       part, stride, splits, c, ldc, ni, nj, bpart, bias, main_blocks, conv_ci, bias2);
     MARL_LAUNCH_CHECK();
     return MARL_OK;
 }
@@ -698,7 +717,9 @@
         if (D.folds > 1) {
             o = D.out0 + (size_t)f * D.n + e;
         } else if (e < D.split) {
-            const int i = e / D.nj, j = e - i * D.nj;
+            const int i = e / D.nj;
+            int j = e - i * D.nj;
+            if (D.ci > 0) j = (j % D.ci) * 9 + j / D.ci;
             o = D.out0 + (size_t)i * D.ldc + j;
         } else {
             o = D.out1 + (e - D.split);
@@ -748,11 +769,11 @@
 }
 
 void RedQueue::push(const float* part, int64_t stride, int count, int n, float* out0, int split, int nj,
-                    int ldc, float* out1, int accumulate) {
+                    int ldc, float* out1, int accumulate, int ci) {
     if (rc != MARL_OK || n <= 0 || count <= 0) return;
     int folds = count > 1024 ? 64 : (count > 256 ? 16 : 1);
     if (stage2.count + 1 > kMaxRed || stage1.count + (folds > 1) > kMaxRed) (void)launch_pending();
-    RedDesc d{part, stride, count, n, out0, split, nj, ldc, out1, accumulate, 1, count};
+    RedDesc d{part, stride, count, n, out0, split, nj, ldc, out1, accumulate, 1, count, ci};
     if (folds > 1) {
         const int per = (int)cdiv(count, folds);
         folds = (int)cdiv(count, per);
diff --git a/marlclassification_amd/csrc/rowops.hip b/marlclassification_amd/csrc/rowops.hip
--- a/marlclassification_amd/csrc/rowops.hip
+++ b/marlclassification_amd/csrc/rowops.hip
@@ -28,6 +28,7 @@
 constexpr int kMaxKnobs = 128;
 Knob g_knobs[kMaxKnobs];
 int g_nknobs = 0;
+int g_knob_epoch = 0;
 Knob* knob(const char* key, bool create) {
     for (int i = 0; i < g_nknobs; ++i)
         if (!strcmp(g_knobs[i].key, key)) return &g_knobs[i];
@@ -61,8 +62,10 @@
     }
     k->value = value;
     k->set = true;
-    return MARL_OK;
-}
+    ++g_knob_epoch;
+    return MARL_OK;
+}
+int tune_epoch() { return g_knob_epoch; }
 
 int tune_get(const char* key, int dflt) {
     Knob* k = knob(key, true);
@@ -1644,6 +1647,178 @@
     return MARL_OK;
 }
 
+__global__ __launch_bounds__(256) void pack_weights_kernel(const PackTable T, const PackParams P, float* __restrict__ W) {
+    __shared__ float t[32][33];
+    const int tid = threadIdx.x;
+    const int blk = (int)blockIdx.x;
+    if (blk >= T.tiles) {
+        const PackVec& v = T.v[blk - T.tiles];
+        const float* a = P.p[v.a];
+        const float* b = v.b >= 0 ? P.p[v.b] : nullptr;
+        for (int i = tid; i < v.n; i += 256) {
+            float x = a[i];
+            if (b) x += b[i];
+            W[(size_t)v.dst + i] = x;
+        }
+        return;
+    }
+    int mi = 0;
+    while (mi + 1 < T.nm && T.m[mi + 1].tile0 <= blk) ++mi;
+    const PackMat& m = T.m[mi];
+    const int n = m.n, k = m.k;
+    const int tk = (k + 31) >> 5, lt = blk - m.tile0;
+    const int r0 = (lt / tk) * 32, c0 = (lt % tk) * 32;
+    const float* __restrict__ src = P.p[m.param];
+    const int lo = tid & 31, hi = tid >> 5;
+    {
+        const int C = c0 + lo;
+        const int sc = m.ci > 0 ? (C % m.ci) * 9 + C / m.ci : C;
+#pragma unroll
+        for (int i = 0; i < 4; ++i) {
+            const int r = hi + 8 * i, R = r0 + r;
+            t[r][lo] = (R < n && C < k) ? src[(size_t)R * k + sc] : 0.f;
+        }
+    }
+    __syncthreads();
+    {
+        const int C = c0 + lo;
+#pragma unroll
+        for (int i = 0; i < 4; ++i) {
+            const int r = hi + 8 * i, R = r0 + r;
+            if (R >= n || C >= k) continue;
+            const float v = t[r][lo];
+            W[m.wp + (size_t)R * m.ldp + C] = v;
+            if (m.wpf) W[m.wpf + panel_frag_index(R, C, m.gpf)] = v;
+            if (m.wf)
+                W[m.wf + ((size_t)((R >> 4) * (k >> 4) + (C >> 4)) * 4 + ((C >> 2) & 3)) * 64 + (R & 15) * 4 + (C & 3)] = v;
+        }
+    }
+    {
+        const int R = r0 + lo;
+#pragma unroll
+        for (int i = 0; i < 4; ++i) {
+            const int c = hi + 8 * i, C = c0 + c;
+            if (R >= n || C >= k) continue;
+            const float v = t[lo][c];
+            W[m.wt + (size_t)C * m.ldt + R] = v;
+            if (m.wtf) W[m.wtf + panel_frag_index(C, R, m.gtf)] = v;
+        }
+    }
+    if (m.wp3) {
+        uint32_t* o3 = reinterpret_cast<uint32_t*>(W + m.wp3);
+        uint32_t* t3 = reinterpret_cast<uint32_t*>(W + m.wt3);
+        const int ktp = tk, ktt = (n + 31) >> 5;
+#pragma unroll
+        for (int i = 0; i < 2; ++i) {
+            const int p = tid + 256 * i, pr = p & 15, q = p >> 4;
+            uint32_t p0, p1, p2;
+            if (r0 + q < n) {
+                split_pair(t[q][2 * pr], t[q][2 * pr + 1], p0, p1, p2);
+                uint32_t* o = o3 + ((size_t)(r0 + q) * ktp + (c0 >> 5)) * 48 + pr;
+                o[0] = p0;
+                o[16] = p1;
+                o[32] = p2;
+            }
+            if (c0 + q < k) {
+                split_pair(t[2 * pr][q], t[2 * pr + 1][q], p0, p1, p2);
+                uint32_t* o = t3 + ((size_t)(c0 + q) * ktt + (r0 >> 5)) * 48 + pr;
+                o[0] = p0;
+                o[16] = p1;
+                o[32] = p2;
+            }
+        }
+    }
+    if (m.wp3k) {
+        float v[8];
+        if (tid < 128) {
+            const int r = tid >> 2, seg = tid & 3, k0 = c0 + seg * 8, steps = (k + 15) >> 4;
+            if (k0 < steps * 16) {
+#pragma unroll
+                for (int q = 0; q < 8; ++q) v[q] = t[r][seg * 8 + q];
+                img_store8(reinterpret_cast<char*>(W + m.wp3k) + img_off(r0 + r, k0 >> 4, steps), k0, v);
+            }
+        } else {
+            const int c = tid & 31, seg = (tid - 128) >> 5, n0 = r0 + seg * 8, steps = (n + 15) >> 4;
+            if (n0 < steps * 16) {
+#pragma unroll
+                for (int q = 0; q < 8; ++q) v[q] = t[seg * 8 + q][c];
+                img_store8(reinterpret_cast<char*>(W + m.wt3k) + img_off(c0 + c, n0 >> 4, steps), n0, v);
+            }
+        }
+    }
+}
+
+int launch_pack_weights(const PackTable& t, const PackParams& p, float* W, hipStream_t st) {
+    const int blocks = t.tiles + t.nv;
+    if (blocks <= 0) return MARL_OK;
+    hipLaunchKernelGGL(pack_weights_kernel, dim3((unsigned)blocks), dim3(256), 0, st, t, p, W);
+    MARL_LAUNCH_CHECK();
+    return MARL_OK;
+}
+
+__global__ __launch_bounds__(256) void episode_start_kernel(const StartDesc S) {
+    const int part = (int)blockIdx.y;
+    const int64_t i0 = (int64_t)blockIdx.x * blockDim.x + threadIdx.x, stride = (int64_t)gridDim.x * blockDim.x;
+    if (part < 5) {
+        const StartCopy& c = S.c[part];
+        if (!((c.cols | c.lds | c.ldd) & 3) &&
+            !((reinterpret_cast<uintptr_t>(c.src) | reinterpret_cast<uintptr_t>(c.dst)) & 15)) {
+            const int c4 = c.cols >> 2;
+            const int64_t tot4 = c.rows * c4;
+            for (int64_t idx = i0; idx < tot4; idx += stride) {
+                const int64_t r = idx / c4;
+                const int col = (int)(idx - r * c4) * 4;
+                *reinterpret_cast<float4*>(c.dst + r * c.ldd + col) =
+                    c.src ? *reinterpret_cast<const float4*>(c.src + r * c.lds + col) : make_float4(0.f, 0.f, 0.f, 0.f);
+            }
+            return;
+        }
+        const int64_t tot = c.rows * c.cols;
+        for (int64_t idx = i0; idx < tot; idx += stride) {
+            const int64_t r = idx / c.cols;
+            const int col = (int)(idx - r * c.cols);
+            c.dst[r * c.ldd + col] = c.src ? c.src[r * c.lds + col] : 0.f;
+        }
+    } else if (part < 7) {
+        const int j = part - 5;
+        if (j >= S.nimg) return;
+        const int k = S.img_k[j], steps = (k + 15) >> 4;
+        const float* src = S.img_src[j];
+        const int64_t rows32 = (S.rows + 31) & ~(int64_t)31;
+        const int64_t tot = rows32 * steps * 2;
+        for (int64_t idx = i0; idx < tot; idx += stride) {
+            const int64_t r = idx / (steps * 2);
+            const int k0 = (int)(idx - r * steps * 2) * 8;
+            float v[8];
+            if (r < S.rows && k0 + 8 <= k && (k & 3) == 0 && (reinterpret_cast<uintptr_t>(src) & 15) == 0) {
+                const float4 a = *reinterpret_cast<const float4*>(src + r * k + k0);
+                const float4 b = *reinterpret_cast<const float4*>(src + r * k + k0 + 4);
+                v[0] = a.x, v[1] = a.y, v[2] = a.z, v[3] = a.w, v[4] = b.x, v[5] = b.y, v[6] = b.z, v[7] = b.w;
+            } else {
+#pragma unroll
+                for (int q = 0; q < 8; ++q) v[q] = (r < S.rows && k0 + q < k) ? src[r * k + k0 + q] : 0.f;
+            }
+            img_store8(S.img_dst[j] + img_off(r, k0 >> 4, steps), k0, v);
+        }
+    } else if (S.pos) {
+        for (int64_t idx = i0; idx < S.npos; idx += stride) S.pos_dst[idx] = (int32_t)S.pos[idx];
+    }
+}
+
+int launch_episode_start(const StartDesc& s, hipStream_t st) {
+    int64_t mx = s.pos ? s.npos : 0;
+    for (int i = 0; i < 5; ++i) mx = s.c[i].rows * s.c[i].cols > mx ? s.c[i].rows * s.c[i].cols : mx;
+    for (int j = 0; j < s.nimg; ++j) {
+        const int64_t t = ((s.rows + 31) & ~(int64_t)31) * img_steps(s.img_k[j]) * 2;
+        mx = t > mx ? t : mx;
+    }
+    int64_t gx = cdiv(mx, 256);
+    gx = gx > 1024 ? 1024 : (gx < 1 ? 1 : gx);
+    hipLaunchKernelGGL(episode_start_kernel, dim3((unsigned)gx, 8), dim3(256), 0, st, s);
+    MARL_LAUNCH_CHECK();
+    return MARL_OK;
+}
+
 __global__ void adam_kernel(float* __restrict__ p, const float* __restrict__ g,
                             float* __restrict__ m, float* __restrict__ v, int64_t n,
                             float step_size, float inv_sqrt_bc2, float beta1, float beta2,
```
